# geobacter-rs/rav1e

Hardware: AMD Instinct MI355X
Metric: encoded frames/sec + Mpixels/sec, 4K 8-bit speed=10, 1/2/4/8 GPU vs host CPU (higher is better)
Workload: dtype u8

## Files before the change

include/rav1e_hip.h:

```cpp
#ifndef RAV1E_HIP_H
#define RAV1E_HIP_H

#include <stddef.h>
#include <stdint.h>

#ifdef __cplusplus
extern "C" {
#endif

#define RV_OK 0
#define RV_EINVAL (-1)
#define RV_EHIP (-2)
#define RV_ENOTSUP (-3)

typedef enum rv_cpu_feature_level {
  RV_CPU_NATIVE = 0,
  RV_CPU_SSE2 = 1,
  RV_CPU_SSSE3 = 2,
  RV_CPU_AVX2 = 3,
  RV_CPU_HIP = 4,
  RV_CPU_LEVELS = 5
} rv_cpu_feature_level;

int rv_cpu_feature_level_default(void);
// ... 248 lines not shown
                        uint32_t *d_offsets, uint32_t *d_tokens, uint32_t token_cap,
                        uint32_t *d_status, void *stream);
int rv_ec_cand_rates(const rv_ec_cand *d_cands, int n, const rv_ec_mode_job *d_mode_jobs,
                     int n_mode_jobs, const rv_ec_job *d_tx_jobs, int n_tx_jobs,
                     rv_ec_mode_params params, int n_tiles, const int32_t *d_tile_dims, int xdec,
                     int ydec, int map_w4, int map_h4, const uint8_t *d_coef_map, int map_w8,
                     int map_h8, const uint32_t *d_mode_map, void *d_scratch, uint32_t *d_offsets,
                     uint32_t *d_tokens, uint32_t token_cap, const uint16_t *d_cdfs_all, int n_cdfs,
                     const int32_t *d_group_cdf, const uint32_t *d_init, uint32_t *d_rate,
                     uint32_t *d_status, void *stream);

int rv_q_lookup(int ac, int qindex, int bit_depth);

typedef struct rv_mv {
  int16_t row, col;
} rv_mv;
typedef struct rv_fs_job {
  int32_t po_x, po_y;
  int32_t x_lo, x_hi, y_lo, y_hi;
  rv_mv pmv[2];
  uint32_t lambda;
  int32_t reserved;
} rv_fs_job;
typedef struct rv_fs_result {
  rv_mv best_mv;
  uint32_t reserved;
  uint64_t cost;
} rv_fs_result;

typedef struct rv_mv_blk {
  int8_t ref[2];
  uint8_t n4_w, n4_h, newmv, pad[3];
  rv_mv mv[2];
} rv_mv_blk;
typedef struct rv_mv_cand {
  rv_mv this_mv, comp_mv;
  uint32_t weight;
} rv_mv_cand;
typedef struct rv_mvref_tile {
  int32_t cols, rows, mi_x, mi_y;
} rv_mvref_tile;
typedef struct rv_mvref_geom {
  int32_t n_tiles, grid_w, grid_h, frame_cols, frame_rows;
  uint32_t sign_bias;
} rv_mvref_geom;
typedef struct rv_mvref_query {
  int32_t tile, bx, by, bw4, bh4, ref[2], reserved;
} rv_mvref_query;
typedef struct rv_mvref_result {
  int32_t mode_context, n;
  rv_mv_cand stack[9];
} rv_mvref_result;
size_t rv_mvref_paint_scratch_bytes(rv_mvref_geom geom);
int rv_mvref_grid_paint(const rv_ec_mode_job *d_jobs, int n, rv_mvref_geom geom,
                        const rv_mvref_tile *d_tiles, rv_mv_blk *d_grid, void *d_scratch,
                        uint32_t *d_status, void *stream);
int rv_find_mvrefs_batch(const rv_mvref_query *d_queries, int n, rv_mvref_geom geom,
                         const rv_mvref_tile *d_tiles, const rv_mv_blk *d_grid,
                         rv_mvref_result *d_results, uint32_t *d_status, void *stream);
int rv_ec_mode_fill_stacks(rv_ec_mode_job *d_jobs, int n, rv_mvref_geom geom,
                           const rv_mvref_tile *d_tiles, const rv_mv_blk *d_grid,
                           rv_mvref_result *d_stacks, uint32_t *d_status, void *stream);

size_t rv_propagate_importances_scratch(int w_imp, int h_imp);
int rv_propagate_importances(const rv_plane *org, const rv_plane *ref, const rv_mv *d_mvs,
                             const uint32_t *d_intra_costs, const float *d_importances,
                             int n_unique, float *d_ref_importances, void *d_scratch,
                             size_t scratch_bytes, void *stream);
int rv_full_search_batch(const rv_plane *org, const rv_plane *ref,
                         const rv_fs_job *d_jobs, int n, int blk_w,
                         int blk_h, int step, int allow_hp,
                         rv_fs_result *d_out, void *stream);

int rv_plane_box_sums(const rv_plane *p, uint32_t *d_box, void *stream);

int rv_full_search_sea_batch(const rv_plane *org, const rv_plane *ref,
                             const uint32_t *d_ref_box, const rv_fs_job *d_jobs,
                             int n, int allow_hp, rv_fs_result *d_out,
                             void *stream);

#define RV_DS_MAX_PRED 17
#define RV_MAX_REFS 8
typedef struct rv_ds_job {
  int32_t po_x, po_y;
  int32_t mvx_min, mvx_max;
  int32_t mvy_min, mvy_max;
  rv_mv pmv[2];
  uint32_t lambda;
  int32_t n_pred;
  rv_mv pred[RV_DS_MAX_PRED];
} rv_ds_job;
int rv_diamond_search_batch(const rv_plane *org, const rv_plane *ref,
                            const rv_ds_job *d_jobs, int n, int blk_w,
                            int blk_h, int subpixel, int use_satd,
                            int allow_hp, int bit_depth,
                            rv_fs_result *d_out, void *stream);

int rv_telescopic_subpel_batch(const rv_plane *org, const rv_plane *ref,
                               const rv_ds_job *d_jobs,
                               const rv_fs_result *d_start, int n, int blk_w,
                               int blk_h, int use_satd, int allow_hp,
                               int bit_depth, rv_fs_result *d_out,
                               void *stream);

typedef struct rv_replay_cfg {
  int32_t width, height;
  int32_t xdec, ydec;
  int32_t bit_depth;
  int32_t tile_x0, tile_y0;
  int32_t tile_w, tile_h;
  int32_t n_refs;
  int32_t tile_w_sb, tile_h_sb;
  int32_t n_inputs;
  int32_t flags;
} rv_replay_cfg;
#define RV_REPLAY_EXHAUSTIVE_FS 4
#define RV_REPLAY_SPEED6 8
#define RV_REPLAY_DEBLOCK 16
#define RV_REPLAY_CDEF 32
#define RV_REPLAY_NO_INTRA 64
#define RV_REPLAY_ENTROPY 128
#define RV_REPLAY_MVREF_STANDIN 256
#define RV_REPLAY_LRF 512
typedef struct rv_replay_frame_info {
  int32_t display;
  int32_t me_range_scale;
  int32_t level;
  int32_t is_key;
  int32_t ref_display[2];
  int32_t compound;
} rv_replay_frame_info;
typedef struct rv_replay_level_params {
  int32_t base_q_idx;
  int32_t dc_delta_q[3];
  int32_t ac_delta_q[3];
  int32_t cdef_strengths;
  double lambda, me_lambda;
  double dist_scale[3];
} rv_replay_level_params;
typedef struct rv_replay rv_replay;
rv_replay *rv_replay_create(const rv_replay_cfg *cfg, void *stream);
void rv_replay_destroy(rv_replay *r);
rv_replay *rv_replay_create_twin(rv_replay *primary, void *stream);
int rv_replay_seek(rv_replay *r, long n);
void *rv_replay_stream(rv_replay *r);
int rv_replay_set_level_params(rv_replay *r, int level, const rv_replay_level_params *p);
int rv_replay_synth_inputs(rv_replay *r, int t0);
int rv_replay_set_input(rv_replay *r, int idx, const void *host_yuv);
int rv_replay_get_input(rv_replay *r, int idx, void *host_yuv);
int rv_replay_get_recon(rv_replay *r, int display, void *host_yuv);
int rv_replay_set_importances(rv_replay *r, const float *host, int n);
int rv_replay_set_imp_window(rv_replay *r, int window, long limit);
int rv_replay_set_inputs_ready(rv_replay *r, long displays);
typedef struct rv_la_hub rv_la_hub;
rv_la_hub *rv_la_hub_create(int n_groups);
void rv_la_hub_destroy(rv_la_hub *hub);
int rv_replay_set_la_exchange(rv_replay *r, void *comm, rv_la_hub *hub);
int rv_replay_get_importances(rv_replay *r, float *host, int n);
int rv_replay_frame(rv_replay *r, rv_replay_frame_info *info);
int rv_replay_set_groups(rv_replay *r, int n_groups, const int32_t *rects, int my_group,
                         void *comm);
int rv_replay_exchange_buffers(rv_replay *r, void **send, void **recv, size_t *bytes_per_group);
int rv_replay_import(rv_replay *r);
int rv_comm_unique_id(uint8_t *out, int cap);
void *rv_comm_create(const uint8_t *id, int nranks, int rank);
void rv_comm_destroy(void *comm);
int rv_replay_results(rv_replay *r, uint64_t *host_out, int cap);
int rv_replay_entropy_stats(rv_replay *r, uint64_t *out, int cap);
int rv_replay_set_timing(rv_replay *r, int stride, int block);
int rv_replay_stage_times(rv_replay *r, float *ms_out, int cap);
int rv_replay_stage_times_sum(rv_replay *r, int last_frames, float *ms_out,
                              int cap);
int rv_replay_set_kernel_probe(rv_replay *r, int on);
int rv_round_ring_slots(uint32_t q, int32_t *out, int cap);
int rv_replay_lrf_units(rv_replay *r, int plane, int8_t *out, int cap);
int rv_replay_la_refs(long m, int R, int32_t *out);
int rv_replay_kernel_probe(rv_replay *r, double *out, int cap);
int rv_ds_phase_dump(void);
int rv_rdo_phase_dump(void);
int rv_replay_counters(rv_replay *r, uint64_t *out, int cap);

int rv_replay_dpb_slots(void);


void rv_shims_release(void);
void rv_shims_shutdown(void);

#define RV_DIST_SIZES(X) \
  X(4, 4) X(4, 8) X(8, 4) X(8, 8) X(8, 16) X(16, 8) X(16, 16) X(16, 32) \
  X(32, 16) X(32, 32) X(32, 64) X(64, 32) X(64, 64) X(64, 128) X(128, 64) \
  X(128, 128) X(4, 16) X(16, 4) X(8, 32) X(32, 8) X(16, 64) X(64, 16)

#define RV_DECL_DIST(W, H)                                                   \
  uint32_t rav1e_sad##W##x##H##_hip(const uint8_t *src, ptrdiff_t src_stride, \
                                    const uint8_t *dst, ptrdiff_t dst_stride); \
  uint32_t rav1e_sad##W##x##H##_hbd_hip(const uint16_t *src,                  \
                                        ptrdiff_t src_stride,                 \
                                        const uint16_t *dst,                  \
                                        ptrdiff_t dst_stride);                \
  uint32_t rav1e_satd_##W##x##H##_hip(const uint8_t *src,                     \
                                      ptrdiff_t src_stride,                   \
                                      const uint8_t *dst,                     \
                                      ptrdiff_t dst_stride);                  \
  uint32_t rav1e_satd_##W##x##H##_hbd_hip(const uint16_t *src,                \
                                          ptrdiff_t src_stride,               \
                                          const uint16_t *dst,                \
                                          ptrdiff_t dst_stride);
RV_DIST_SIZES(RV_DECL_DIST)
#undef RV_DECL_DIST

#define RV_FILTER_PAIRS(X)                                                  \
  X(regular, regular, 0, 0) X(smooth, regular, 1, 0)                       \
  X(sharp, regular, 2, 0) X(bilinear, regular, 3, 0)                       \
  X(regular, smooth, 0, 1) X(smooth, smooth, 1, 1) X(sharp, smooth, 2, 1)  \
  X(bilinear, smooth, 3, 1) X(regular, sharp, 0, 2) X(smooth, sharp, 1, 2) \
  X(sharp, sharp, 2, 2) X(bilinear, sharp, 3, 2)                           \
  X(regular, bilinear, 0, 3) X(smooth, bilinear, 1, 3)                     \
  X(sharp, bilinear, 2, 3) X(bilinear, bilinear, 3, 3)

#define RV_DECL_MC(NX, NY, MX, MY)                                            \
  void rav1e_put_8tap_##NX##_##NY##_hip(                                      \
      uint8_t *dst, ptrdiff_t dst_stride, const uint8_t *src,                 \
      ptrdiff_t src_stride, int32_t w, int32_t h, int32_t mx, int32_t my);    \
  void rav1e_put_8tap_##NX##_##NY##_16bpc_hip(                                \
      uint16_t *dst, ptrdiff_t dst_stride, const uint16_t *src,               \
      ptrdiff_t src_stride, int32_t w, int32_t h, int32_t mx, int32_t my,     \
      int32_t bit_depth);                                                     \
  void rav1e_prep_8tap_##NX##_##NY##_hip(int16_t *tmp, const uint8_t *src,    \
                                         ptrdiff_t src_stride, int32_t w,     \
                                         int32_t h, int32_t mx, int32_t my);  \
  void rav1e_prep_8tap_##NX##_##NY##_16bpc_hip(                               \
      int16_t *tmp, const uint16_t *src, ptrdiff_t src_stride, int32_t w,     \
      int32_t h, int32_t mx, int32_t my, int32_t bit_depth);
RV_FILTER_PAIRS(RV_DECL_MC)
#undef RV_DECL_MC

void rav1e_avg_hip(uint8_t *dst, ptrdiff_t dst_stride, const int16_t *tmp1,
                   const int16_t *tmp2, int32_t w, int32_t h);
void rav1e_avg_16bpc_hip(uint16_t *dst, ptrdiff_t dst_stride,
                         const int16_t *tmp1, const int16_t *tmp2, int32_t w,
                         int32_t h, int32_t bit_depth);

int rav1e_fwd_txfm_hip(const int16_t *residual, int32_t *coeffs,
                       int32_t tx_size, int32_t tx_type, int32_t bit_depth);
int rav1e_inv_txfm_add_hip(const int32_t *coeffs, void *dst,
                           ptrdiff_t dst_stride, int32_t tx_size,
                           int32_t tx_type, int32_t bit_depth);

typedef uint32_t (*rv_dist_fn)(const void *src, ptrdiff_t src_stride,
                               const void *dst, ptrdiff_t dst_stride);
rv_dist_fn rv_sad_fn(int cpu_level, int bsize, int hbd);
rv_dist_fn rv_satd_fn(int cpu_level, int bsize, int hbd);
typedef void (*rv_put_fn)(void *dst, ptrdiff_t dst_stride, const void *src,
                          ptrdiff_t src_stride, int32_t w, int32_t h,
                          int32_t mx, int32_t my);
rv_put_fn rv_put_fn_get(int cpu_level, int mode_x, int mode_y);

#ifdef __cplusplus
}
#endif
#endif
```

rav1e_amd/__init__.py:

```python
from __future__ import annotations

import ctypes as C
import enum
import os

import numpy as np

_ROOT = os.path.dirname(os.path.abspath(__file__))
LIB_PATH = os.environ.get("RAV1E_HIP_LIB") or os.path.join(_ROOT, "lib", "librav1e_hip.so")
HEADER_PATH = os.path.join(os.path.dirname(_ROOT), "include", "rav1e_hip.h")

RV_OK, RV_EINVAL, RV_EHIP, RV_ENOTSUP = 0, -1, -2, -3


class Rav1eHipError(RuntimeError):
    pass


class RvPlane(C.Structure):
    _fields_ = [("data", C.c_void_p), ("stride", C.c_int32),
                ("alloc_height", C.c_int32), ("width", C.c_int32),
                ("height", C.c_int32), ("xorigin", C.c_int32),
                ("yorigin", C.c_int32), ("xdec", C.c_int32),
                ("ydec", C.c_int32), ("hbd", C.c_int32),
# ... 113 lines not shown
    TX_64X64 = 4
    TX_4X8 = 5
    TX_8X4 = 6
    TX_8X16 = 7
    TX_16X8 = 8
    TX_16X32 = 9
    TX_32X16 = 10
    TX_32X64 = 11
    TX_64X32 = 12
    TX_4X16 = 13
    TX_16X4 = 14
    TX_8X32 = 15
    TX_32X8 = 16
    TX_16X64 = 17
    TX_64X16 = 18

    def width(self) -> int:
        return int(self.name.split("_")[1].split("X")[0])

    def height(self) -> int:
        return int(self.name.split("X")[-1])


class TxType(enum.IntEnum):
    DCT_DCT = 0
    ADST_DCT = 1
    DCT_ADST = 2
    ADST_ADST = 3
    FLIPADST_DCT = 4
    DCT_FLIPADST = 5
    FLIPADST_FLIPADST = 6
    ADST_FLIPADST = 7
    FLIPADST_ADST = 8
    IDTX = 9
    V_DCT = 10
    H_DCT = 11
    V_ADST = 12
    H_ADST = 13
    V_FLIPADST = 14
    H_FLIPADST = 15


class FilterMode(enum.IntEnum):
    REGULAR = 0
    SMOOTH = 1
    SHARP = 2
    BILINEAR = 3


_lib = None


class RvEcModeParams(C.Structure):
    _fields_ = [(n, C.c_int32) for n in ("frame_type", "reference_mode", "force_integer_mv",
                                         "allow_high_precision_mv", "seg_enabled",
                                         "last_active_segid")]


class RvMvrefGeom(C.Structure):
    _fields_ = [(n, C.c_int32) for n in ("n_tiles", "grid_w", "grid_h", "frame_cols",
                                         "frame_rows")] + [("sign_bias", C.c_uint32)]


def _declare(L):
    vp, i32, sz = C.c_void_p, C.c_int, C.c_size_t
    P = C.POINTER(RvPlane)
    sig = {
        "rv_cpu_feature_level_default": (i32, []),
        "rv_cpu_feature_level_index": (i32, [i32]),
        "rv_device_count": (i32, []),
        "rv_set_device": (i32, [i32]),
        "rv_last_error": (C.c_char_p, []),
        "rv_version": (C.c_char_p, []),
        "rv_malloc": (vp, [sz]),
        "rv_free": (None, [vp]),
        "rv_host_alloc": (vp, [sz]),
        "rv_host_free": (None, [vp]),
        "rv_memcpy_h2d": (i32, [vp, vp, sz, vp]),
        "rv_memcpy_d2h": (i32, [vp, vp, sz, vp]),
        "rv_memcpy_d2d": (i32, [vp, vp, sz, vp]),
        "rv_memset": (i32, [vp, i32, sz, vp]),
        "rv_stream_create": (vp, []),
        "rv_stream_create_priority": (vp, [i32]),
        "rv_stream_destroy": (i32, [vp]),
        "rv_stream_sync": (i32, [vp]),
        "rv_device_sync": (i32, []),
        "rv_trace_marker": (i32, [vp]),
        "rv_event_create": (vp, []),
        "rv_event_destroy": (i32, [vp]),
        "rv_event_record": (i32, [vp, vp]),
        "rv_event_sync": (i32, [vp]),
        "rv_stream_wait_event": (i32, [vp, vp]),
        "rv_event_elapsed_ms": (C.c_float, [vp, vp]),
        "rv_plane_geometry": (sz, [P, i32, i32, i32, i32, i32, i32, i32]),
        "rv_plane_pad": (i32, [P, vp]),
        "rv_plane_downsample": (i32, [P, P, vp]),
        "rv_sad_batch": (i32, [P, P, vp, i32, i32, i32, vp, vp]),
        "rv_satd_batch": (i32, [P, P, vp, i32, i32, i32, vp, vp]),
        "rv_sse_batch": (i32, [P, P, vp, i32, i32, i32, vp, vp]),
        "rv_lookahead_intra_costs": (i32, [P, i32, vp, vp]),
        "rv_propagate_importances_scratch": (sz, [i32, i32]),
        "rv_propagate_importances": (i32, [P, P, vp, vp, vp, i32, vp, vp, sz, vp]),
        "rv_cdef_moments_batch": (i32, [P, P, vp, i32, i32, i32, vp, vp]),
        "rv_put_8tap_batch": (i32, [P, P, vp, i32, i32, i32, i32, i32, i32, vp]),
        "rv_predict_intra_batch": (i32, [P, vp, vp, i32, i32, i32, vp]),
        "rv_cfl_luma_ac_batch": (i32, [P, vp, i32, i32, i32, i32, vp, vp]),
        "rv_predict_cfl_batch": (i32, [P, vp, vp, vp, vp, i32, i32, i32, vp]),
        "rv_cfl_alpha_search_batch": (i32, [P, P, vp, i32, i32, i32, vp, vp, vp]),
        "rv_frame_delta_batch": (i32, [P, i32, i32, vp, i32, vp, vp]),
        "rv_deblock_plane": (i32, [P, i32, i32, i32, vp, vp, i32, vp, i32, vp]),
        "rv_deblock_fast_level": (i32, [i32, i32, i32]),
        "rv_deblock_sse": (i32, [P, P, i32, i32, vp, vp, i32, vp, vp, i32, vp]),
        "rv_deblock_frame": (i32, [P, i32, i32, vp, vp, i32, vp, i32, vp]),
        "rv_cdef_find_dirs": (i32, [P, i32, i32, vp, i32, vp, vp, i32, vp]),
        "rv_lrf_stripe_filter": (i32, [P, P] + [i32] * 10 + [vp, vp]),
        "rv_y4m_parse_header": (i32, [C.c_char_p, vp]),
        "rv_y4m_open": (vp, [C.c_char_p]),
        "rv_y4m_get_info": (i32, [vp, vp]),
        "rv_y4m_frame_bytes": (sz, [vp]),
        "rv_y4m_read_frame": (i32, [vp, vp]),
        "rv_y4m_close": (None, [vp]),
        "rv_ivf_create": (vp, [C.c_char_p, i32, i32, i32, i32]),
        "rv_ivf_write_frame": (i32, [vp, C.c_uint64, vp, sz]),
        "rv_ivf_close": (i32, [vp]),
        "rv_cdef_filter_plane": (i32, [P, P, i32, i32, i32, vp, i32, vp, vp, vp, vp, vp, i32, i32,
                                       vp]),
        "rv_prep_8tap_batch": (i32, [vp, P, vp, i32, i32, i32, i32, i32, i32, vp]),
        "rv_mc_avg_batch": (i32, [P, vp, vp, vp, i32, i32, i32, i32, vp]),
        "rv_mc_dist_batch": (i32, [P, P, vp, i32, i32, i32, i32, i32, i32, i32, vp, vp]),
        "rv_fwd_txfm_batch": (i32, [vp, vp, i32, i32, i32, i32, vp]),
        "rv_diff_fwd_txfm_batch": (i32, [P, P, vp, i32, i32, i32, i32, vp, vp]),
        "rv_inv_txfm_add_batch": (i32, [vp, P, vp, i32, i32, i32, i32, vp]),
        "rv_quantize_batch": (i32, [vp, i32, i32, i32, i32, i32, i32, i32, i32, i32, vp, vp, vp,
                                    vp]),
        "rv_dequantize_batch": (i32, [vp, i32, i32, i32, i32, i32, i32, vp, vp]),
        "rv_estimate_rate_batch": (i32, [vp, i32, i32, i32, vp, vp]),
        "rv_full_search_batch": (i32, [P, P, vp, i32, i32, i32, i32, i32, vp, vp]),
        "rv_full_search_sea_batch": (i32, [P, P, vp, vp, i32, i32, vp, vp]),
        "rv_plane_box_sums": (i32, [P, vp, vp]),
        "rv_replay_create": (vp, [C.POINTER(RvReplayCfg), vp]),
        "rv_replay_create_twin": (vp, [vp, vp]),
        "rv_replay_seek": (i32, [vp, C.c_long]),
        "rv_replay_stream": (vp, [vp]),
        "rv_replay_destroy": (None, [vp]),
        "rv_q_lookup": (i32, [i32, i32, i32]),
        "rv_replay_synth_inputs": (i32, [vp, i32]),
        "rv_replay_set_level_params": (i32, [vp, i32, C.POINTER(RvReplayLevelParams)]),
        "rv_replay_set_input": (i32, [vp, i32, vp]),
        "rv_replay_get_input": (i32, [vp, i32, vp]),
        "rv_replay_get_recon": (i32, [vp, i32, vp]),
        "rv_replay_set_importances": (i32, [vp, vp, i32]),
        "rv_replay_set_imp_window": (i32, [vp, i32, C.c_long]),
        "rv_replay_set_inputs_ready": (i32, [vp, C.c_long]),
        "rv_replay_get_importances": (i32, [vp, vp, i32]),
        "rv_replay_frame": (i32, [vp, C.POINTER(RvReplayFrameInfo)]),
        "rv_replay_set_groups": (i32, [vp, i32, vp, i32, vp]),
        "rv_replay_exchange_buffers": (i32, [vp, C.POINTER(C.c_void_p), C.POINTER(C.c_void_p),
                                             C.POINTER(C.c_size_t)]),
        "rv_replay_import": (i32, [vp]),
        "rv_comm_unique_id": (i32, [vp, i32]),
        "rv_comm_create": (vp, [vp, i32, i32]),
        "rv_comm_destroy": (None, [vp]),
        "rv_replay_results": (i32, [vp, vp, i32]),
        "rv_replay_entropy_stats": (i32, [vp, vp, i32]),
        "rv_replay_stage_times": (i32, [vp, vp, i32]),
        "rv_replay_stage_times_sum": (i32, [vp, i32, vp, i32]),
        "rv_replay_counters": (i32, [vp, vp, i32]),
        "rv_replay_dpb_slots": (i32, []),
        "rv_replay_set_kernel_probe": (i32, [vp, i32]),
        "rv_replay_kernel_probe": (i32, [vp, vp, i32]),
        "rv_round_ring_slots": (i32, [C.c_uint32, vp, i32]),
        "rv_replay_lrf_units": (i32, [vp, i32, vp, i32]),
        "rv_replay_la_refs": (i32, [C.c_long, i32, vp]),
        "rv_la_hub_create": (vp, [i32]),
        "rv_la_hub_destroy": (None, [vp]),
        "rv_replay_set_la_exchange": (i32, [vp, vp, vp]),
        "rv_replay_set_timing": (i32, [vp, i32, i32]),
        "rv_diamond_search_batch": (i32, [P, P, vp, i32, i32, i32, i32, i32, i32, i32, vp, vp]),
        "rv_telescopic_subpel_batch": (i32, [P, P, vp, vp, i32, i32, i32, i32, i32, i32, vp, vp]),
        "rv_tx_dist_batch": (i32, [vp, i32, vp, i32, i32, vp, vp]),
        "rav1e_fwd_txfm_hip": (i32, [vp, vp, i32, i32, i32]),
        "rav1e_inv_txfm_add_hip": (i32, [vp, vp, C.c_ssize_t, i32, i32, i32]),
        "rv_ec_scratch_bytes": (C.c_size_t, [i32]),
        "rv_ec_tokenize": (i32, [vp, i32, i32, i32, i32, i32, i32, vp, vp, vp, vp, C.c_uint32, vp,
                                 vp]),
        "rv_ec_code_tokens": (C.c_long, [vp, C.c_size_t, vp, vp, C.c_size_t]),
        "rv_ec_count_tokens": (C.c_long, [vp, C.c_size_t, vp, vp]),
        "rv_ec_rate_batch": (i32, [vp, vp, vp, i32, vp, i32, vp, vp, vp, vp, vp]),
        "rv_ec_cdf_total": (i32, []),
        "rv_ec_default_cdf": (i32, [i32, vp]),
        "rv_ec_reset_counts": (None, [vp]),
        "rv_ec_mode_scratch_bytes": (C.c_size_t, [i32]),
        "rv_ec_mode_tokenize": (i32, [vp, i32, RvEcModeParams, i32, vp, i32, i32, vp, vp, vp, vp,
                                      C.c_uint32, vp, vp]),
        "rv_ec_code_stream": (C.c_long, [vp, C.c_size_t, vp, vp, C.c_size_t]),
        "rv_ec_count_stream": (C.c_long, [vp, C.c_size_t, vp, vp]),
        "rv_ec_cdf_total_all": (i32, []),
        "rv_ec_default_cdf_all": (i32, [i32, vp]),
        "rv_ec_reset_counts_all": (None, [vp]),
        "rv_ec_partition_gather": (i32, [vp, i32]),
        "rv_ec_rate_stream_batch": (i32, [vp, vp, vp, i32, vp, i32, vp, vp, vp, vp, vp]),
        "rv_ec_rate_stream_batch_waves": (i32, [vp, vp, vp, i32, vp, i32, vp, vp, vp, vp, i32, vp]),
        "rv_ec_cand_scratch_bytes": (C.c_size_t, [i32, i32]),
        "rv_ec_cand_tokenize": (i32, [vp, i32, vp, i32, vp, i32, RvEcModeParams, i32, vp, i32, i32,
                                      i32, i32, vp, i32, i32, vp, vp, vp, vp, C.c_uint32, vp, vp]),
        "rv_ec_cand_rates": (i32, [vp, i32, vp, i32, vp, i32, RvEcModeParams, i32, vp, i32, i32,
                                   i32, i32, vp, i32, i32, vp, vp, vp, vp, C.c_uint32, vp, i32, vp,
                                   vp, vp, vp, vp]),
        "rv_mvref_paint_scratch_bytes": (C.c_size_t, [RvMvrefGeom]),
        "rv_mvref_grid_paint": (i32, [vp, i32, RvMvrefGeom, vp, vp, vp, vp, vp]),
        "rv_find_mvrefs_batch": (i32, [vp, i32, RvMvrefGeom, vp, vp, vp, vp, vp]),
        "rv_ec_mode_fill_stacks": (i32, [vp, i32, RvMvrefGeom, vp, vp, vp, vp, vp]),
        "rv_sad_fn": (vp, [i32, i32, i32]),
        "rv_satd_fn": (vp, [i32, i32, i32]),
        "rv_put_fn_get": (vp, [i32, i32, i32]),
    }
    for name, (res, args) in sig.items():
        f = getattr(L, name)
        f.restype = res
        f.argtypes = args


def lib():
    global _lib
    if _lib is None:
        if not os.path.exists(LIB_PATH):
            raise Rav1eHipError(
                f"{LIB_PATH} missing: run `python -c 'import __graft_entry__ as g; g.build()'`")
        L = C.CDLL(LIB_PATH, mode=C.RTLD_GLOBAL)
        _declare(L)
        _lib = L
    return _lib


def _check(rc, what):
    if rc != RV_OK:
        raise Rav1eHipError(f"{what} failed ({rc}): {lib().rv_last_error().decode()}")


def require_device(device: int = 0):
    L = lib()
    if L.rv_device_count() <= device:
        raise Rav1eHipError("no HIP device visible: the HIP level needs a gfx950 GPU")
    _check(L.rv_set_device(device), "rv_set_device")


class DeviceBuffer:

    def __init__(self, nbytes: int):
        self.nbytes = int(nbytes)
        self.ptr = lib().rv_malloc(max(1, self.nbytes))
        if not self.ptr:
            raise Rav1eHipError(f"rv_malloc({nbytes}): {lib().rv_last_error().decode()}")

    @classmethod
    def from_array(cls, a: np.ndarray) -> "DeviceBuffer":
        a = np.ascontiguousarray(a)
        b = cls(a.nbytes)
        b.upload(a)
        return b

    def upload(self, a: np.ndarray, stream=None):
        a = np.ascontiguousarray(a)
        assert a.nbytes <= self.nbytes
        if a.nbytes:
            _check(lib().rv_memcpy_h2d(self.ptr, a.ctypes.data, a.nbytes, stream), "rv_memcpy_h2d")

    def download(self, dtype, count=None, stream=None) -> np.ndarray:
        dt = np.dtype(dtype)
        n = self.nbytes // dt.itemsize if count is None else int(count)
        out = np.empty(n, dtype=dt)
        if out.nbytes:
            _check(lib().rv_memcpy_d2h(out.ctypes.data, self.ptr, out.nbytes, stream),
                   "rv_memcpy_d2h")
        return out

    def zero(self, stream=None):
        _check(lib().rv_memset(self.ptr, 0, self.nbytes, stream), "rv_memset")
        _check(lib().rv_stream_sync(stream), "rv_stream_sync")

    def free(self):
        if self.ptr:
            lib().rv_free(self.ptr)
            self.ptr = None

    def __del__(self):
        try:
            self.free()
        except Exception:
            pass


class DevicePlane:

    def __init__(self, width, height, xdec=0, ydec=0, xpad=0, ypad=0, hbd=False,
                 bit_depth=None):
        self.desc = RvPlane()
        nbytes = lib().rv_plane_geometry(C.byref(self.desc), width, height, xdec, ydec,
                                         xpad, ypad, 1 if hbd else 0)
        if bit_depth is not None:
            self.desc.bit_depth = int(bit_depth)
        self.buf = DeviceBuffer(nbytes)
        self.desc.data = self.buf.ptr
        self.dtype = np.uint16 if hbd else np.uint8

    @classmethod
# ... 1737 lines not shown
```

rav1e_amd/csrc/rv_epzs.h:

```cpp
#pragma once

#include "rv_chain.h"

namespace rv {

struct EpzsGeo {
  int tx0, ty0, tw, th, tws, ths, W, H, w_in_b, h_in_b;
};

__device__ inline void epzs_tile(const EpzsGeo &g, int fx, int fy, int &t0x, int &t0y, int &mi_w,
                                 int &mi_h) {
  t0x = fx - fx % g.tws;
  t0y = fy - fy % g.ths;
  const int vw = g.W - t0x * 64 < g.tws * 64 ? g.W - t0x * 64 : g.tws * 64;
  const int vh = g.H - t0y * 64 < g.ths * 64 ? g.H - t0y * 64 : g.ths * 64;
  mi_w = vw >> 2;
  mi_h = vh >> 2;
}

__device__ inline void epzs_adjust_bo(int mi_w, int mi_h, int &bx, int &by, int bw, int bh) {
  const int x = bx < mi_w - bw / 4 ? bx : mi_w - bw / 4;
  const int y = by < mi_h - bh / 4 ? by : mi_h - bh / 4;
  bx = x > 0 ? x : 0;
  by = y > 0 ? y : 0;
}

__device__ inline rv_mv epzs_qfull(rv_mv m) {
  return rv_mv{(int16_t)((m.row / 8) * 8), (int16_t)((m.col / 8) * 8)};
}
__device__ inline bool epzs_zero(rv_mv m) { return m.row == 0 && m.col == 0; }

template <int NCM, typename Rd>
__device__ inline bool epzs_update(rv_ds_job *j, int shr, const EpzsGeo &g, int tx4, int ty4,
                                   int mi_w, int bx, int by, const rv_mv (&cm)[NCM], int ncm,
                                   Rd rd, const rv_mv *prev, int pr) {
  static_assert(NCM >= 1 && 1 + NCM + 4 + 5 <= RV_DS_MAX_PRED, "slots");
  constexpr int NS = 1 + NCM + 4 + 5;
  const bool hl = bx > 0, ht = by > 0, htr = ht && bx < mi_w - 1;
  const rv_mv z{0, 0};
  const rv_mv l = hl ? rd(tx4 + bx - 1, ty4 + by) : z;
  const rv_mv t = ht ? rd(tx4 + bx, ty4 + by - 1) : z;
  const rv_mv tr = htr ? rd(tx4 + bx + 1, ty4 + by - 1) : z;
  rv_mv c[NS];
  uint32_t valid = 1;
  c[0] = z;
#pragma unroll
  for (int i = 0; i < NCM; i++) {
    c[1 + i] = epzs_qfull(cm[i]);
    valid |= (uint32_t)(i < ncm) << (1 + i);
  }
  c[NCM + 1] = l;
  c[NCM + 2] = t;
  c[NCM + 3] = tr;
  valid |= (uint32_t)(hl && !epzs_zero(l)) << (NCM + 1);
  valid |= (uint32_t)(ht && !epzs_zero(t)) << (NCM + 2);
  valid |= (uint32_t)(htr && !epzs_zero(tr)) << (NCM + 3);
  const int nm = (int)hl + (int)ht + (int)htr;
  {
    const int16_t sr = (int16_t)((int16_t)(l.row + t.row) + tr.row);
    const int16_t sc = (int16_t)((int16_t)(l.col + t.col) + tr.col);
    const int d = nm ? nm : 1;
    c[NCM + 4] = epzs_qfull(rv_mv{(int16_t)(sr / d), (int16_t)(sc / d)});
    valid |= (uint32_t)(nm && !epzs_zero(c[NCM + 4])) << (NCM + 4);
  }
  if (prev) {
    const int fx = tx4 + bx, fy = ty4 + by, w8 = g.w_in_b >> 1;
    auto pv = [&](int x, int y) { return prev[((y >> 1) * w8 + (x >> 1)) * pr]; };
    c[NCM + 5] = fx > 0 ? pv(fx - 1, fy) : z;
    c[NCM + 6] = fy > 0 ? pv(fx, fy - 1) : z;
    c[NCM + 7] = fx < g.w_in_b - 1 ? pv(fx + 1, fy) : z;
    c[NCM + 8] = fy < g.h_in_b - 1 ? pv(fx, fy + 1) : z;
    c[NCM + 9] = pv(fx, fy);
#pragma unroll
    for (int i = NCM + 5; i < NS; i++) valid |= (uint32_t)!epzs_zero(c[i]) << i;
  } else {
#pragma unroll
    for (int i = NCM + 5; i < NS; i++) c[i] = z;
  }
  auto tf = [&](rv_mv m) { return shr ? rv_mv{(int16_t)(m.row >> 1), (int16_t)(m.col >> 1)} : m; };
  rv_mv nw[NS];
#pragma unroll
  for (int p = 0; p < NS; p++) nw[p] = z;
#pragma unroll
  for (int i = 0; i < NS; i++) {
    const bool v = (valid >> i) & 1;
    const int pos = __popc(valid & ((1u << i) - 1));
    const rv_mv ti = tf(c[i]);
#pragma unroll
    for (int p = 0; p <= i; p++)
      if (v && pos == p) nw[p] = ti;
  }
  const int n = __popc(valid);
  rv_mv old[NS];
#pragma unroll
  for (int p = 0; p < NS; p++) old[p] = j->pred[p];
  const int old_n = j->n_pred;
  bool same = old_n == n;
#pragma unroll
  for (int p = 0; p < NS; p++) same &= (p >= n) | mv_eq(old[p], nw[p]);
  if (same) return false;
#pragma unroll
  for (int p = 0; p < NS; p++)
    if (p < n) j->pred[p] = nw[p];
  j->n_pred = n;
  return true;
}

struct RoundPub {
  int32_t *cnt, *next;
  uint32_t *ticket;
  unsigned long long *host;
  uint32_t seq;
};
__device__ inline void round_publish(const RoundPub &p) {
  if (!p.host) return;
  __syncthreads();
  if (threadIdx.x != 0) return;
  __threadfence();
  const uint32_t t = atomicAdd(p.ticket, 1u);
  if (t != gridDim.x - 1) return;
  __threadfence();
  const int c = atomicAdd(p.cnt, 0) + atomicAdd(p.cnt + 1, 0);
  p.next[0] = p.next[1] = 0;
  *p.ticket = 0;
  __threadfence();
  __hip_atomic_store(p.host, ((unsigned long long)p.seq << 32) | (uint32_t)c, __ATOMIC_RELAXED,
                     __HIP_MEMORY_SCOPE_SYSTEM);
}

}
```

rav1e_amd/csrc/rv_me.h:

```cpp
#pragma once
#include "rv_chain.h"
#include "rv_device.h"

int rv_full_search_multi(const rv_plane *org, const rv_plane *refs, int n_refs,
                         const rv_fs_job *d_jobs, int n_per_ref, int blk_w, int blk_h,
                         int step, int allow_hp, rv_fs_result *d_out, const rv::ChainNext *next,
                         const uint32_t *const *box, void *stream);
int rv_diamond_search_multi(const rv_plane *org, const rv_plane *refs, int n_refs,
                            const rv_ds_job *d_jobs, int n_per_ref, int blk_w, int blk_h,
                            int subpixel, int use_satd, int allow_hp, int bit_depth,
                            rv_fs_result *d_out, uint32_t *d_evals, const rv::ChainNext *next,
                            void *stream, const uint8_t *active = nullptr,
                            const int32_t *alist = nullptr, const int32_t *acount = nullptr,
                            int lper = 1, const uint8_t *dirty = nullptr, int list_grid = 0,
                            uint32_t *eval_acc = nullptr, unsigned long long *t01 = nullptr);
int rv_diamond_f2_f3(const rv_plane *org_h, const rv_plane *refs_h, const rv_ds_job *jobs_h,
                     rv_fs_result *out_h, const uint8_t *dirty_h, const rv_plane *org,
                     const rv_plane *refs, const rv_ds_job *jobs, rv_fs_result *out,
                     const uint8_t *dirty, const rv::ChainNext *next, int n_refs, int n_per_ref,
                     int bit_depth, const int32_t *alist, const int32_t *acount, int list_grid,
                     void *stream, const rv_ds_job *jobs_sub = nullptr,
                     rv_fs_result *out_sub = nullptr, uint32_t *eval_acc = nullptr,
                     unsigned long long *t01 = nullptr);
```

rav1e_amd/csrc/rv_me_diamond.hip:

```cpp
#include <algorithm>
#include <stdio.h>
#include <stdlib.h>
#include <string.h>

#include "rv_chain.h"
#include "rv_device.h"
#include "rv_me.h"

namespace rv {

constexpr int kDsThreads = 256;
constexpr int kDsWaves = kDsThreads / 64;

__constant__ int8_t kReg[2][16][8] = {
    {{0, 0, 0, 127, 0, 0, 0, 0}, {0, 2, -6, 126, 8, -2, 0, 0},
     {0, 2, -10, 122, 18, -4, 0, 0}, {0, 2, -12, 116, 28, -8, 2, 0},
     {0, 2, -14, 110, 38, -10, 2, 0}, {0, 2, -14, 102, 48, -12, 2, 0},
     {0, 2, -16, 94, 58, -12, 2, 0}, {0, 2, -14, 84, 66, -12, 2, 0},
     {0, 2, -14, 76, 76, -14, 2, 0}, {0, 2, -12, 66, 84, -14, 2, 0},
     {0, 2, -12, 58, 94, -16, 2, 0}, {0, 2, -12, 48, 102, -14, 2, 0},
     {0, 2, -10, 38, 110, -14, 2, 0}, {0, 2, -8, 28, 116, -12, 2, 0},
     {0, 0, -4, 18, 122, -10, 2, 0}, {0, 0, -2, 8, 126, -6, 2, 0}},
    {{0, 0, 0, 127, 0, 0, 0, 0}, {0, 0, -4, 126, 8, -2, 0, 0},
     {0, 0, -8, 122, 18, -4, 0, 0}, {0, 0, -10, 116, 28, -6, 0, 0},
     {0, 0, -12, 110, 38, -8, 0, 0}, {0, 0, -12, 102, 48, -10, 0, 0},
     {0, 0, -14, 94, 58, -10, 0, 0}, {0, 0, -12, 84, 66, -10, 0, 0},
     {0, 0, -12, 76, 76, -12, 0, 0}, {0, 0, -10, 66, 84, -12, 0, 0},
     {0, 0, -10, 58, 94, -14, 0, 0}, {0, 0, -10, 48, 102, -12, 0, 0},
     {0, 0, -8, 38, 110, -12, 0, 0}, {0, 0, -6, 28, 116, -10, 0, 0},
     {0, 0, -4, 18, 122, -8, 0, 0}, {0, 0, -2, 8, 126, -4, 0, 0}}};

__device__ __forceinline__ uint32_t ds_diff_to_rate(int16_t diff, int hp) {
  int16_t d = hp ? diff : (int16_t)(diff >> 1);
  if (d == 0) return 0;
  uint32_t a = (uint16_t)(d < 0 ? -d : d);
  return 2u * (16u - (uint32_t)(__builtin_clz(a) - 16));
}

__device__ __forceinline__ uint64_t ds_cost(uint32_t dist, rv_mv mv, const rv_ds_job &jb,
                                            int hp) {
  const uint32_t r1 = ds_diff_to_rate((int16_t)(mv.row - jb.pmv[0].row), hp) +
                      ds_diff_to_rate((int16_t)(mv.col - jb.pmv[0].col), hp);
  const uint32_t r2 = ds_diff_to_rate((int16_t)(mv.row - jb.pmv[1].row), hp) +
                      ds_diff_to_rate((int16_t)(mv.col - jb.pmv[1].col), hp);
  const uint32_t rate = r1 < r2 + 1 ? r1 : r2 + 1;
  return 256ull * dist + (uint64_t)rate * jb.lambda;
}

__device__ __forceinline__ bool ds_in_range(rv_mv mv, const rv_ds_job &jb) {
  return !(mv.col < jb.mvx_min || mv.col > jb.mvx_max || mv.row < jb.mvy_min ||
           mv.row > jb.mvy_max);
}

__device__ __forceinline__ int xcd_job(int n) {
  const int per = (int)gridDim.x >> 3;
  return ((int)blockIdx.x & 7) * per + ((int)blockIdx.x >> 3);
}

struct DsArgs {
  rv_plane org;
  rv_plane ref[RV_MAX_REFS];
  const rv_ds_job *jobs;
  rv_fs_result *out;
  int n, n_per_ref, w, h, subpel, satd, hp, bd;
  uint32_t *evals;
  uint32_t *eval_acc;
  unsigned long long *t0, *t1;
  ChainNext next;
  int tele;
  const rv_fs_result *start;
  const uint8_t *active;
  const int32_t *alist;
  const int32_t *acount;
  int lper;
  const uint8_t *dirty;
  int list_grid;
  int ph;
};

__device__ unsigned long long g_ds_ph[16];

__device__ __forceinline__ int ds_list_total(const DsArgs &a) {
  const int cnt = __builtin_amdgcn_readfirstlane(*a.acount);
  return a.lper ? cnt * a.lper * (a.n / a.n_per_ref) : cnt;
}
__device__ __forceinline__ int ds_list_job(const DsArgs &a, int ord) {
  if (!a.lper) return a.alist[ord];
  const int cnt = *a.acount, per = cnt * a.lper;
  const int r = ord / per, rem = ord - r * per, i = rem / a.lper;
  return r * a.n_per_ref + a.alist[i] * a.lper + (rem - i * a.lper);
}

constexpr int kDsListGrid = 512;

__device__ __forceinline__ void ds_write(const DsArgs &a, int job, rv_mv center,
                                         uint64_t cost) {
  rv_fs_result r;
  r.best_mv = center;
  r.reserved = 0;
  r.cost = cost;
  a.out[job] = r;
}

__device__ __forceinline__ uint4 ld16(const void *p) {
  uint4 v;
  __builtin_memcpy(&v, p, 16);
  return v;
}
template <typename Px>
__device__ __forceinline__ uint32_t sad16(uint4 a, uint4 b, uint32_t acc) {
  if constexpr (sizeof(Px) == 1) {
    acc = __builtin_amdgcn_sad_u8(a.x, b.x, acc);
    acc = __builtin_amdgcn_sad_u8(a.y, b.y, acc);
    acc = __builtin_amdgcn_sad_u8(a.z, b.z, acc);
    return __builtin_amdgcn_sad_u8(a.w, b.w, acc);
  } else {
    acc = __builtin_amdgcn_sad_u16(a.x, b.x, acc);
    acc = __builtin_amdgcn_sad_u16(a.y, b.y, acc);
    acc = __builtin_amdgcn_sad_u16(a.z, b.z, acc);
    return __builtin_amdgcn_sad_u16(a.w, b.w, acc);
  }
}

__device__ __forceinline__ uint32_t wave_sum(uint32_t v) { return group_sum<64>(v); }

template <typename Px, int W, int H>
struct FullGeo {
  static constexpr int K = W * (int)sizeof(Px) / 16;
  static constexpr int R = 64 / K;
  static constexpr int I = (H + R - 1) / R;
  static constexpr bool kPartial = (R * I != H);
};

template <typename Px, int W, int H>
struct SubGeo {
  static constexpr int G = 64 / W;
  static constexpr int RG = H / G;
  static constexpr int P = sizeof(Px) == 1 ? ((W + 8 + 15) / 16) * 16
                                           : ((2 * (W + 8) + 15) / 16) * 16;
  static constexpr int kWinDwords = (H + 7) * P / 4;
  static constexpr int kOrgDwords = RG * (int)sizeof(Px) / 4;
  static constexpr int D = 8;
  static constexpr int UP = (((W + 7 + D + 4) * (int)sizeof(Px)) + 15) / 16 * 16;
  static constexpr int kUnionDwords = (H + 7 + D) * UP / 4;
};

template <typename Px, int W, int RG, int UP, bool HF, bool VF>
__device__ __forceinline__ uint32_t sub_sad_rows(const uint32_t *win, const Px *ocol, int cx,
                                                 int grp, const int8_t *xf, const int8_t *yf,
                                                 int ib, int maxv) {
  constexpr int B = (int)sizeof(Px);
  constexpr int PD = UP / 4;
  uint32_t xp[4] = {0, 0, 0, 0};
  int xsum = 0;
  if constexpr (HF) {
    if constexpr (B == 1) {
#pragma unroll
      for (int h = 0; h < 2; h++)
        xp[h] = (uint32_t)(uint8_t)xf[4 * h] | ((uint32_t)(uint8_t)xf[4 * h + 1] << 8) |
                ((uint32_t)(uint8_t)xf[4 * h + 2] << 16) | ((uint32_t)(uint8_t)xf[4 * h + 3] << 24);
#pragma unroll
      for (int k = 0; k < 8; k++) xsum += xf[k];
    } else {
#pragma unroll
      for (int h = 0; h < 3; h++)
        xp[h] = (uint32_t)(uint16_t)(int16_t)xf[2 * h + 1] |
                ((uint32_t)(uint16_t)(int16_t)xf[2 * h + 2] << 16);
    }
  }
  uint32_t tp[3] = {0, 0, 0};
  if constexpr (VF) {
#pragma unroll
    for (int h = 0; h < 3; h++)
      tp[h] = (uint32_t)(uint16_t)(int16_t)yf[2 * h + 1] |
              ((uint32_t)(uint16_t)(int16_t)yf[2 * h + 2] << 16);
  }
  const int hbias = 128 * xsum;
  const int hround = (1 << (7 - ib)) >> 1, hsh = 7 - ib;
  const uint32_t *base = win + grp * RG * PD;
  auto hval = [&](int t) __attribute__((always_inline)) -> int32_t {
    const uint32_t *row = base + t * PD;
    if constexpr (B == 1) {
      if constexpr (!HF) {
        return (int32_t)(reinterpret_cast<const uint8_t *>(row)[cx + 3] ^ 0x80u);
      } else {
        const int d0 = cx >> 2, sh = cx & 3;
        const uint32_t w0 = row[d0], w1 = row[d0 + 1], w2 = row[d0 + 2];
        int32_t s = dot4_i8(__builtin_amdgcn_alignbyte(w1, w0, sh), xp[0], hbias + hround);
        s = dot4_i8(__builtin_amdgcn_alignbyte(w2, w1, sh), xp[1], s);
        return s >> hsh;
      }
    } else {
      if constexpr (!HF) {
        return (int32_t)reinterpret_cast<const uint16_t *>(row)[cx + 3];
      } else {
        const int c1 = cx + 1, d0 = c1 >> 1, sh = (c1 & 1) * 2;
        uint32_t w[4];
#pragma unroll
        for (int k = 0; k < 4; k++) w[k] = row[d0 + k];
        int32_t s = hround;
#pragma unroll
        for (int k = 0; k < 3; k++) s = dot2_i16(__builtin_amdgcn_alignbyte(w[k + 1], w[k], sh), xp[k], s);
        return s >> hsh;
      }
    }
  };
  auto absdiff_acc = [](uint32_t a, uint32_t b, uint32_t acc) __attribute__((always_inline)) {
    return (a > b ? a - b : b - a) + acc;
  };
  uint32_t acc = 0;
  if constexpr (!VF) {
#pragma unroll 8
    for (int r = 0; r < RG; r++) {
      int32_t v = hval(r + 3);
      if constexpr (HF) v = clamp_med3(round_shift(v, ib), 0, maxv);
      acc = absdiff_acc((uint32_t)ocol[r * W], (uint32_t)v, acc);
    }
  } else {
    const int vshift = HF ? 7 + ib : 7;
    const int vround = (1 << vshift) >> 1;
    auto pack = [](int32_t lo, int32_t hi) __attribute__((always_inline)) {
      return __builtin_amdgcn_perm((uint32_t)hi, (uint32_t)lo, 0x05040100u);
    };
    uint32_t pr[8];
    int32_t prev = hval(1);
#pragma unroll
    for (int t = 2; t < 6; t++) {
      const int32_t m = hval(t);
      pr[t - 1] = pack(prev, m);
      prev = m;
// ... 609 lines not shown
      if (center_cost <= best) {
        if (radius == radius_end) break;
        radius /= 2;
      } else {
        center = best_mv;
        center_cost = best;
      }
    }
  }
  if (threadIdx.x == 0) {
    if (a.evals) a.evals[job] = evals;
    ds_write(a, job, center, center_cost);
    chain_emit(a.next, job, a.n_per_ref, a.n / a.n_per_ref, center);
  }
}

template <typename Px, int W, int H>
__global__ __launch_bounds__(64) void ds_wave_kernel(DsArgs a) {
  using F = FullGeo<Px, W, H>;
  constexpr int B = (int)sizeof(Px);
  const int job = xcd_job(a.n);
  if (job >= a.n) return;
  if (a.active && !a.active[job % a.n_per_ref]) return;
  const int lane = threadIdx.x;
  const rv_ds_job *jp = a.jobs + job;
  const rv_ds_job jb = *jp;
  const rv_plane &ref = a.ref[job / a.n_per_ref];
  const int frow = lane / F::K, fchunk = lane % F::K;
  uint32_t org[4 * F::I];
  {
    const uint8_t *o = (const uint8_t *)plane_ptr<Px>(a.org, jb.po_x, jb.po_y);
    const int64_t os = (int64_t)a.org.stride * B;
#pragma unroll
    for (int i = 0; i < F::I; i++) {
      const int r = i * F::R + frow;
      uint4 v = make_uint4(0, 0, 0, 0);
      if (!F::kPartial || r < H) v = ld16(o + r * os + fchunk * 16);
      org[4 * i + 0] = v.x;
      org[4 * i + 1] = v.y;
      org[4 * i + 2] = v.z;
      org[4 * i + 3] = v.w;
    }
  }
  const int64_t rs = (int64_t)ref.stride * B;
  uint32_t evals = 0;
  auto round4 = [&](const rv_mv *cands, int n, int skip, uint64_t *cost)
      __attribute__((always_inline)) {
    bool ok[kDsWaves];
    const uint8_t *rp[kDsWaves];
#pragma unroll
    for (int k = 0; k < kDsWaves; k++) {
      ok[k] = k < n && k != skip && ds_in_range(cands[k], jb);
      rp[k] = (const uint8_t *)plane_ptr<Px>(ref, jb.po_x + (ok[k] ? cands[k].col / 8 : 0),
                                             jb.po_y + (ok[k] ? cands[k].row / 8 : 0));
      evals += ok[k];
    }
    uint32_t acc[kDsWaves] = {0, 0, 0, 0};
#pragma unroll
    for (int i = 0; i < F::I; i++) {
      const int rr = i * F::R + frow;
      if (!F::kPartial || rr < H) {
        uint4 v[kDsWaves];
#pragma unroll
        for (int k = 0; k < kDsWaves; k++)
          v[k] = ok[k] ? ld16(rp[k] + rr * rs + fchunk * 16) : make_uint4(0, 0, 0, 0);
        const uint4 o = make_uint4(org[4 * i], org[4 * i + 1], org[4 * i + 2], org[4 * i + 3]);
#pragma unroll
        for (int k = 0; k < kDsWaves; k++) acc[k] = sad16<Px>(o, v[k], acc[k]);
      }
    }
#pragma unroll
    for (int k = 0; k < kDsWaves; k++)
      cost[k] = ok[k] ? ds_cost(wave_sum(acc[k]), cands[k], jb, a.hp) : ~0ull;
  };

  rv_mv center{0, 0};
  uint64_t center_cost = ~0ull;
  const int np = jb.n_pred < RV_DS_MAX_PRED ? jb.n_pred : RV_DS_MAX_PRED;
  int16_t radius = 16;
  const int16_t radius_end = 8;
  int p0 = 0;
  int back = -1;
  for (int iter = 0; iter < 4096 + RV_DS_MAX_PRED; iter++) {
    const bool pred_phase = p0 < np;
    rv_mv c4[kDsWaves];
    int n;
    if (pred_phase) {
      n = np - p0 < kDsWaves ? np - p0 : kDsWaves;
#pragma unroll
      for (int k = 0; k < kDsWaves; k++) c4[k] = jp->pred[p0 + (k < n ? k : 0)];
    } else {
      n = kDsWaves;
      c4[0] = rv_mv{(int16_t)(center.row + radius), center.col};
      c4[1] = rv_mv{center.row, (int16_t)(center.col + radius)};
      c4[2] = rv_mv{(int16_t)(center.row - radius), center.col};
      c4[3] = rv_mv{center.row, (int16_t)(center.col - radius)};
    }
    uint64_t c[kDsWaves];
    round4(c4, n, pred_phase ? -1 : back, c);
    uint64_t best = ~0ull;
    int bp = 0;
#pragma unroll
    for (int k = 0; k < kDsWaves; k++)
      if (k < n && c[k] < best) {
        best = c[k];
        bp = k;
      }
    rv_mv bmv = c4[0];
#pragma unroll
    for (int k = 1; k < kDsWaves; k++)
      if (bp == k) bmv = c4[k];
    if (pred_phase) {
      if (best < center_cost) {
        center = bmv;
        center_cost = best;
      }
      p0 += kDsWaves;
    } else if (center_cost <= best) {
      if (radius == radius_end) break;
      radius /= 2;
      back = -1;
    } else {
      back = center_cost != ~0ull ? (bp + 2) & 3 : -1;
      center = bmv;
      center_cost = best;
    }
  }
  if (lane == 0) {
    if (a.evals) a.evals[job] = evals;
    ds_write(a, job, center, center_cost);
    chain_emit(a.next, job, a.n_per_ref, a.n / a.n_per_ref, center);
  }
}

typedef short rv_s16x2 __attribute__((ext_vector_type(2)));
__device__ __forceinline__ int32_t sdot2(uint32_t a, uint32_t b, int32_t c) {
  return __builtin_amdgcn_sdot2(__builtin_bit_cast(rv_s16x2, a), __builtin_bit_cast(rv_s16x2, b),
                                c, false);
}
__device__ __forceinline__ uint32_t pk16(int lo, int hi) {
  return (uint32_t)(uint16_t)lo | ((uint32_t)(uint16_t)hi << 16);
}

template <int N, bool SADONLY>
struct GrpGeo {
  static constexpr int C = N == 8 || (SADONLY && N == 16) ? 4 : 16;
  static constexpr int L = 4 * C;
  static constexpr int RPL = N == 8 ? 2 : (N == 16 && C == 16) ? 2 : 8;
  static constexpr int LPC = 8 / RPL;
  static constexpr int NC = N / 8;
  static constexpr int CPL = NC * NC * LPC / C;
};

template <typename Px, int N, bool SUB, bool SATD>
__device__ __forceinline__ void ds_grp_body(const DsArgs &a, const int ord, const int nord) {
  using G = GrpGeo<N, !SUB && !SATD>;
  static_assert(G::CPL >= 1 && G::C % G::LPC == 0, "lane layout");
  const int lane = threadIdx.x & 63;
  const int gl = lane % G::L, k = gl / G::C, c = gl % G::C;
  const int gbase = lane - gl;
  const int oid = ord < nord ? ord : nord - 1;
  const int job = a.alist ? ds_list_job(a, oid) : oid;
  const bool live = ord < nord && !(a.dirty && !a.dirty[job]);
  if (__ballot(live) == 0) return;
  const int jid = job;
  const rv_ds_job *jp = a.jobs + jid;
  const rv_ds_job jb = *jp;
  const rv_plane &ref = a.ref[jid / a.n_per_ref];
  const int ib = a.bd == 12 ? 2 : 4, maxv = (1 << a.bd) - 1;
  const int lic = c % G::LPC;

  auto dist = [&](rv_mv mv, bool ok) -> uint32_t {
    int cf = 0, rf = 0, sx = 0, sy = 0;
    if (SUB) {
      const int xs = 3 + ref.xdec, ys = 3 + ref.ydec;
      const int roff = (int)mv.row >> ys, coff = (int)mv.col >> xs;
      rf = ((int)mv.row - (roff << ys)) << (4 - ys);
      cf = ((int)mv.col - (coff << xs)) << (4 - xs);
      sx = clampi(jb.po_x + coff - 3, -ref.xorigin, ref.width);
      sy = clampi(jb.po_y + roff - 3, -ref.yorigin, ref.height);
    } else {
      sx = jb.po_x + (ok ? mv.col / 8 : 0);
      sy = jb.po_y + (ok ? mv.row / 8 : 0);
    }
    uint32_t xp[7];
    int32_t fy[8];
    if (SUB) {
      int32_t fx[8];
      const int8_t *xf = kReg[0][cf];
      const int8_t *yf = kReg[0][rf];
#pragma unroll
      for (int u = 0; u < 8; u++) {
        fx[u] = cf ? (int32_t)xf[u] : (u == 3 ? 128 : 0);
        fy[u] = rf ? (int32_t)yf[u] : (u == 3 ? 128 : 0);
      }
      xp[0] = pk16(fx[1], fx[2]);
      xp[1] = pk16(fx[3], fx[4]);
      xp[2] = pk16(fx[5], fx[6]);
      xp[3] = pk16(fx[0], fx[1]);
      xp[4] = pk16(fx[2], fx[3]);
      xp[5] = pk16(fx[4], fx[5]);
      xp[6] = pk16(fx[6], fx[7]);
    }
    const int32_t hround = (1 << (7 - ib)) >> 1, vround = (1 << (7 + ib)) >> 1;
    uint32_t acc = 0;
#pragma unroll 1
    for (int j = 0; j < G::CPL; j++) {
      const int q = c / G::LPC + j * (G::C / G::LPC);
      const int x0 = (q % G::NC) * 8, y0 = (q / G::NC) * 8 + lic * G::RPL;
      int32_t d[G::RPL][8];
      if (SUB) {
        int32_t v[G::RPL][8];
#pragma unroll
        for (int i = 0; i < G::RPL; i++)
#pragma unroll
          for (int t = 0; t < 8; t++) v[i][t] = vround;
#pragma unroll
        for (int m = 1; m < G::RPL + 6; m++) {
          const Px *w = plane_ptr<Px>(ref, sx + x0, sy + y0 + m);
          uint32_t pp[7];
          if constexpr (sizeof(Px) == 1) {
            const uint4 lv = ld16(w);
            const uint32_t wd[4] = {lv.x, lv.y, lv.z, lv.w};
#pragma unroll
            for (int jj = 0; jj < 7; jj++)
              pp[jj] = __builtin_amdgcn_perm(0u, wd[jj >> 1], jj & 1 ? 0x0c030c02u : 0x0c010c00u);
          } else {
            const uint4 v0 = ld16(w), v1 = ld16(w + 8);
            const uint32_t wd[7] = {v0.x, v0.y, v0.z, v0.w, v1.x, v1.y, v1.z};
#pragma unroll
            for (int jj = 0; jj < 7; jj++) pp[jj] = wd[jj];
          }
          int32_t mid[8];
#pragma unroll
          for (int t = 0; t < 8; t++) {
            int32_t hs = hround;
            if (t & 1) {
#pragma unroll
              for (int u = 0; u < 3; u++) hs = sdot2(pp[(t + 1) / 2 + u], xp[u], hs);
            } else {
#pragma unroll
              for (int u = 0; u < 4; u++) hs = sdot2(pp[t / 2 + u], xp[3 + u], hs);
            }
            mid[t] = hs >> (7 - ib);
          }
#pragma unroll
          for (int i = 0; i < G::RPL; i++) {
            const int kk = m - i;
            if (kk >= 1 && kk < 7) {
#pragma unroll
              for (int t = 0; t < 8; t++) v[i][t] += __mul24(fy[kk], mid[t]);
            }
          }
        }
#pragma unroll
        for (int i = 0; i < G::RPL; i++) {
          const Px *o = plane_ptr<Px>(a.org, jb.po_x + x0, jb.po_y + y0 + i);
#pragma unroll
          for (int t = 0; t < 8; t++)
            d[i][t] = (int32_t)o[t] - clampi(v[i][t] >> (7 + ib), 0, maxv);
        }
      } else if (ok) {
        if (!SATD) {
#pragma unroll
          for (int i = 0; i < G::RPL; i++) {
            const Px *o = plane_ptr<Px>(a.org, jb.po_x + x0, jb.po_y + y0 + i);
            const Px *r = plane_ptr<Px>(ref, sx + x0, sy + y0 + i);
            if constexpr (sizeof(Px) == 1) {
              uint2 ov, rv;
              __builtin_memcpy(&ov, o, 8);
              __builtin_memcpy(&rv, r, 8);
              acc = __builtin_amdgcn_sad_u8(ov.x, rv.x, acc);
              acc = __builtin_amdgcn_sad_u8(ov.y, rv.y, acc);
            } else {
              acc = sad16<Px>(ld16(o), ld16(r), acc);
            }
#pragma unroll
            for (int t = 0; t < 8; t++) d[i][t] = 0;
          }
        } else {
#pragma unroll
          for (int i = 0; i < G::RPL; i++) {
            const Px *o = plane_ptr<Px>(a.org, jb.po_x + x0, jb.po_y + y0 + i);
            const Px *r = plane_ptr<Px>(ref, sx + x0, sy + y0 + i);
#pragma unroll
            for (int t = 0; t < 8; t++) d[i][t] = (int32_t)o[t] - (int32_t)r[t];
          }
        }
      } else {
#pragma unroll
        for (int i = 0; i < G::RPL; i++)
#pragma unroll
          for (int t = 0; t < 8; t++) d[i][t] = 0;
      }
      if (SATD) {
#pragma unroll
        for (int i = 0; i < G::RPL; i++) ds_had<8>(&d[i][0], 1);
#pragma unroll
        for (int b = 1; b < G::RPL; b <<= 1)
#pragma unroll
          for (int i = 0; i < G::RPL; i++)
            if (!(i & b))
#pragma unroll
              for (int t = 0; t < 8; t++) {
                const int32_t x = d[i][t], y = d[i + b][t];
                d[i][t] = x + y;
                d[i + b][t] = x - y;
              }
#pragma unroll
        for (int b = 1; b < G::LPC; b <<= 1) {
          const bool up = (lic & b) != 0;
#pragma unroll
          for (int i = 0; i < G::RPL; i++)
#pragma unroll
            for (int t = 0; t < 8; t++) {
              const int32_t p = __shfl_xor(d[i][t], b, 64);
              d[i][t] = up ? p - d[i][t] : d[i][t] + p;
            }
        }
      }
#pragma unroll
      for (int i = 0; i < G::RPL; i++)
#pragma unroll
        for (int t = 0; t < 8; t++) acc += (uint32_t)(d[i][t] < 0 ? -d[i][t] : d[i][t]);
    }
#pragma unroll
    for (int m = G::C / 2; m; m >>= 1) acc += __shfl_xor(acc, m, 64);
    return SATD ? (acc + 4) >> 3 : acc;
  };

  uint32_t evals = 0;
  auto round4 = [&](const rv_mv *cands, int n, int skip, uint64_t *cost)
      __attribute__((always_inline)) {
    bool ok[4];
#pragma unroll
    for (int kk = 0; kk < 4; kk++) {
      ok[kk] = kk < n && kk != skip && ds_in_range(cands[kk], jb);
      evals += ok[kk];
    }
    rv_mv mine = cands[0];
    bool okm = ok[0];
#pragma unroll
    for (int kk = 1; kk < 4; kk++)
      if (k == kk) {
        mine = cands[kk];
        okm = ok[kk];
      }
    const uint32_t dv = dist(mine, okm);
    const uint64_t cm = okm ? ds_cost(dv, mine, jb, a.hp) : ~0ull;
    const uint32_t lo = (uint32_t)cm, hi = (uint32_t)(cm >> 32);
#pragma unroll
    for (int kk = 0; kk < 4; kk++) {
      const uint32_t l = __shfl(lo, gbase + kk * G::C, 64), h = __shfl(hi, gbase + kk * G::C, 64);
      cost[kk] = ((uint64_t)h << 32) | l;
    }
  };

  rv_mv center{0, 0};
  uint64_t center_cost = ~0ull;
  const int np = jb.n_pred < RV_DS_MAX_PRED ? jb.n_pred : RV_DS_MAX_PRED;
  int16_t radius = SUB ? 4 : 16;
  const int16_t radius_end = SUB ? (a.hp ? 1 : 2) : 8;
  int p0 = 0, back = -1;
  for (int iter = 0; iter < 4096 + RV_DS_MAX_PRED; iter++) {
    const bool pred_phase = p0 < np;
    rv_mv c4[4];
    int n;
    if (pred_phase) {
      n = np - p0 < 4 ? np - p0 : 4;
#pragma unroll
      for (int kk = 0; kk < 4; kk++) c4[kk] = jp->pred[p0 + (kk < n ? kk : 0)];
    } else {
      n = 4;
      c4[0] = rv_mv{(int16_t)(center.row + radius), center.col};
      c4[1] = rv_mv{center.row, (int16_t)(center.col + radius)};
      c4[2] = rv_mv{(int16_t)(center.row - radius), center.col};
      c4[3] = rv_mv{center.row, (int16_t)(center.col - radius)};
    }
    uint64_t cst[4];
    round4(c4, n, pred_phase ? -1 : back, cst);
    uint64_t best = ~0ull;
    int bp = 0;
#pragma unroll
    for (int kk = 0; kk < 4; kk++)
      if (kk < n && cst[kk] < best) {
        best = cst[kk];
        bp = kk;
      }
    rv_mv bmv = c4[0];
#pragma unroll
    for (int kk = 1; kk < 4; kk++)
      if (bp == kk) bmv = c4[kk];
    if (pred_phase) {
      if (best < center_cost) {
        center = bmv;
        center_cost = best;
      }
      p0 += 4;
    } else if (center_cost <= best) {
      if (radius == radius_end) break;
      radius /= 2;
      back = -1;
    } else {
      back = center_cost != ~0ull ? (bp + 2) & 3 : -1;
      center = bmv;
      center_cost = best;
    }
  }
  if (gl == 0 && live) {
    if (a.evals) a.evals[job] = evals;
    ds_write(a, job, center, center_cost);
    chain_emit(a.next, job, a.n_per_ref, a.n / a.n_per_ref, center);
  }
}

template <typename Px, int N, bool SUB, bool SATD>
__global__ __launch_bounds__(256) void ds_grp_kernel(DsArgs a) {
  using G = GrpGeo<N, !SUB && !SATD>;
  constexpr int JPW = 64 / G::L;
  const int lane = threadIdx.x & 63;
  const int w0 = ((int)blockIdx.x * 4 + (int)(threadIdx.x >> 6)) * JPW;
  const int nord = a.alist ? ds_list_total(a) : a.n;
  const int step = (int)gridDim.x * 4 * JPW;
  for (int o = w0; o < nord; o += step) {
    ds_grp_body<Px, N, SUB, SATD>(a, o + lane / G::L, nord);
    if (!a.alist) break;
  }
}
template <typename Px>
__device__ __forceinline__ void ds_grp16_pool(DsArgs a, int b, int gsz) {
  using G = GrpGeo<16, true>;
  constexpr int JPW = 64 / G::L;
  const int lane = threadIdx.x & 63;
  const int nord = ds_list_total(a);
  for (int o = (b * 4 + (int)(threadIdx.x >> 6)) * JPW; o < nord; o += gsz * 4 * JPW)
    ds_grp_body<Px, 16, false, false>(a, o + lane / G::L, nord);
}
template <typename Px>
__device__ __forceinline__ void ds_fast64_pool(DsArgs a, DsArgs sa, bool fuse, int b, int gsz) {
  const int total = ds_list_total(a);
  for (int i = b; i < total; i += gsz) {
    const int job = __builtin_amdgcn_readfirstlane(ds_list_job(a, i));
    if (a.dirty && !a.dirty[job]) continue;
    const rv_mv best = ds_fast_body<Px, 64, 64, false>(a, job);
    __syncthreads();
    if (fuse) {
      ds_fast_body<Px, 64, 64, true>(sa, job, true, best);
      __syncthreads();
    }
  }
}
template <typename Px>
__global__ __launch_bounds__(256) void ds_f2_f3_kernel(
    DsArgs f2, DsArgs f3, DsArgs f3s, int g2, int fuse, unsigned long long *t01) {
  if (t01 && threadIdx.x == 0) atomicMin(t01, (unsigned long long)wall_clock64());
  if ((int)blockIdx.x < g2)
    ds_grp16_pool<Px>(f2, blockIdx.x, g2);
  else
    ds_fast64_pool<Px>(f3, f3s, fuse != 0, (int)blockIdx.x - g2, (int)gridDim.x - g2);
  if (t01) {
    __syncthreads();
    if (threadIdx.x == 0) atomicMax(t01 + 1, (unsigned long long)wall_clock64());
  }
}

template <typename Px>
bool try_grp(const DsArgs &a, hipStream_t s) {
  if (a.tele || a.w != a.h || a.active) return false;
  const int n = a.w;
  const bool small = n == 8 || n == 16;
  if (!(small || (a.satd && (n == 32 || n == 64)))) return false;
  const int jpw = 64 / (n == 8 || (n == 16 && !a.subpel && !a.satd) ? 16 : 64);
  unsigned grid = (unsigned)((a.n + 4 * jpw - 1) / (4 * jpw));
  if (a.alist && grid > (unsigned)(a.list_grid ? a.list_grid : kDsListGrid))
    grid = (unsigned)(a.list_grid ? a.list_grid : kDsListGrid);
#define RV_GRP(N)                                                                     \
  if (n == N) {                                                                       \
    if (a.subpel) {                                                                   \
      if (a.satd) ds_grp_kernel<Px, N, true, true><<<grid, 256, 0, s>>>(a);           \
      else ds_grp_kernel<Px, N, true, false><<<grid, 256, 0, s>>>(a);                 \
    } else {                                                                          \
      if (a.satd) ds_grp_kernel<Px, N, false, true><<<grid, 256, 0, s>>>(a);          \
      else ds_grp_kernel<Px, N, false, false><<<grid, 256, 0, s>>>(a);                \
    }                                                                                 \
    return true;                                                                      \
  }
  RV_GRP(8)
  RV_GRP(16)
  RV_GRP(32)
  RV_GRP(64)
#undef RV_GRP
  return false;
}

template <typename Px, int W, int H, bool SUB>
void launch_fast(DsArgs a, hipStream_t s) {
  static const bool phases = getenv("RAV1E_HIP_DS_PHASES") && getenv("RAV1E_HIP_DS_PHASES")[0] == '1';
  a.ph = phases && SUB && a.alist ? 1 : 0;
  const unsigned grid = a.alist ? (unsigned)std::min(a.n, a.list_grid ? a.list_grid : kDsListGrid)
                                 : (unsigned)((a.n + 7) / 8 * 8);
  if (!SUB && !a.tele && W * H <= 32 * 32 && !a.alist)
    ds_wave_kernel<Px, W, H><<<grid, 64, 0, s>>>(a);
  else
    ds_fast_kernel<Px, W, H, SUB><<<grid, kDsThreads, 0, s>>>(a);
}

template <typename Px>
bool try_fast(const DsArgs &a, hipStream_t s) {
  if (a.satd) return false;
#define RV_DS_CASE(W, H)                                        \
  if (a.w == W && a.h == H) {                                   \
    if (a.subpel)                                               \
      launch_fast<Px, W, H, true>(a, s);                        \
    else                                                        \
      launch_fast<Px, W, H, false>(a, s);                       \
    return true;                                                \
  }
  RV_DS_CASE(64, 64)
  RV_DS_CASE(32, 32)
  RV_DS_CASE(64, 32)
  RV_DS_CASE(32, 64)
  RV_DS_CASE(16, 32)
  RV_DS_CASE(16, 64)
#undef RV_DS_CASE
  return false;
}

}

using namespace rv;

extern "C" int rv_ds_phase_dump(void) {
  unsigned long long h[16];
  if (hipDeviceSynchronize() != hipSuccess || hipMemcpyFromSymbol(h, HIP_SYMBOL(g_ds_ph), sizeof(h)) != hipSuccess)
    return rv_set_error(RV_EHIP, "rv_ds_phase_dump");
  const double us = 0.01;
  const double j = h[5] ? (double)h[5] : 1.0, w = h[8] ? (double)h[8] : 1.0;
  fprintf(stderr,
          "[ds phases] jobs %llu: setup %.2f us, stage+filter+SAD %.2f us, exchange %.2f us, "
          "job %.2f us per job; %.2f iterations, %.2f stagings per job; workgroups %llu: %.2f us each\n",
          h[5], h[0] * us / j, h[1] * us / j, h[2] * us / j, h[3] * us / j, h[4] / j, h[6] / j, h[8],
          h[7] * us / w);
  memset(h, 0, sizeof(h));
  return hipMemcpyToSymbol(HIP_SYMBOL(g_ds_ph), h, sizeof(h)) == hipSuccess ? RV_OK : rv_set_error(RV_EHIP, "rv_ds_phase_dump");
}

static int ds_dispatch(DsArgs &a, void *stream);

int rv_diamond_search_multi(const rv_plane *org, const rv_plane *refs, int n_refs,
                            const rv_ds_job *d_jobs, int n_per_ref, int blk_w, int blk_h,
                            int subpixel, int use_satd, int allow_hp, int bit_depth,
                            rv_fs_result *d_out, uint32_t *d_evals, const ChainNext *next,
                            void *stream, const uint8_t *active, const int32_t *alist,
                            const int32_t *acount, int lper, const uint8_t *dirty,
                            int list_grid, uint32_t *eval_acc, unsigned long long *t01) {
  auto p2 = [](int v) { return v >= 4 && v <= 128 && (v & (v - 1)) == 0; };
  if (!org || !refs || n_refs < 1 || n_refs > RV_MAX_REFS || n_per_ref < 0 || !p2(blk_w) ||
      !p2(blk_h) || (bit_depth != 8 && bit_depth != 10 && bit_depth != 12) ||
      (!org->hbd && bit_depth != 8))
    return rv_set_error(RV_EINVAL, "rv_diamond_search_batch: bad arguments");
  for (int k = 0; k < n_refs; k++)
    if (refs[k].hbd != org->hbd)
      return rv_set_error(RV_EINVAL, "rv_diamond_search_batch: pixel type mismatch");
  const int n = n_refs * n_per_ref;
  if (n == 0) return RV_OK;
  DsArgs a;
  memset(&a, 0, sizeof(a));
  a.org = *org;
  for (int k = 0; k < n_refs; k++) a.ref[k] = refs[k];
  a.jobs = d_jobs;
  a.out = d_out;
  a.n = n;
  a.n_per_ref = n_per_ref;
  a.w = blk_w;
  a.h = blk_h;
  a.subpel = subpixel ? 1 : 0;
  a.satd = use_satd ? 1 : 0;
  a.hp = allow_hp ? 1 : 0;
  a.bd = bit_depth;
  a.evals = d_evals;
  a.active = active;
  a.alist = alist;
  a.acount = acount;
  a.lper = lper;
  a.dirty = alist ? dirty : nullptr;
  a.list_grid = list_grid;
  a.eval_acc = eval_acc;
  if (t01) {
    a.t0 = t01;
    a.t1 = t01 + 1;
  }
  if (alist && (!acount || lper < 0 || use_satd ||
                !((blk_w == 64 && blk_h == 64) || (blk_w == 16 && blk_h == 16 && !subpixel))))
    return rv_set_error(RV_EINVAL,
                        "rv_diamond_search_multi: list-driven launches: 64x64, or 16x16 full-pel SAD");
  if (next) a.next = *next;
  return ds_dispatch(a, stream);
}

static void ds_fill(DsArgs &a, const rv_plane *org, const rv_plane *refs, int n_refs,
                    const rv_ds_job *d_jobs, int n_per_ref, int blk, rv_fs_result *d_out,
                    int bit_depth, const int32_t *alist, const int32_t *acount, int lper,
                    const uint8_t *dirty) {
  memset(&a, 0, sizeof(a));
  a.org = *org;
  for (int k = 0; k < n_refs; k++) a.ref[k] = refs[k];
  a.jobs = d_jobs;
  a.out = d_out;
  a.n = n_refs * n_per_ref;
  a.n_per_ref = n_per_ref;
  a.w = a.h = blk;
  a.bd = bit_depth;
  a.alist = alist;
  a.acount = acount;
  a.lper = lper;
  a.dirty = dirty;
}

int rv_diamond_f2_f3(const rv_plane *org_h, const rv_plane *refs_h, const rv_ds_job *jobs_h,
                     rv_fs_result *out_h, const uint8_t *dirty_h, const rv_plane *org,
                     const rv_plane *refs, const rv_ds_job *jobs, rv_fs_result *out,
                     const uint8_t *dirty, const ChainNext *next, int n_refs, int n_per_ref,
                     int bit_depth, const int32_t *alist, const int32_t *acount, int list_grid,
                     void *stream, const rv_ds_job *jobs_sub, rv_fs_result *out_sub,
                     uint32_t *eval_acc, unsigned long long *t01) {
  if (!org_h || !refs_h || !org || !refs || n_refs < 1 || n_refs > RV_MAX_REFS || n_per_ref <= 0 ||
      !alist || !acount || org->hbd != org_h->hbd)
    return rv_set_error(RV_EINVAL, "rv_diamond_f2_f3: bad arguments");
  DsArgs f2, f3;
  ds_fill(f2, org_h, refs_h, n_refs, jobs_h, n_per_ref * 4, 16, out_h, bit_depth, alist, acount, 4,
          dirty_h);
  ds_fill(f3, org, refs, n_refs, jobs, n_per_ref, 64, out, bit_depth, alist, acount, 1, dirty);
  if (next) f3.next = *next;
  DsArgs f3s;
  ds_fill(f3s, org, refs, n_refs, jobs_sub ? jobs_sub : jobs, n_per_ref, 64, out_sub ? out_sub : out,
          bit_depth, alist, acount, 1, dirty);
  f3s.subpel = 1;
  static const bool phases = getenv("RAV1E_HIP_DS_PHASES") && getenv("RAV1E_HIP_DS_PHASES")[0] == '1';
  f3s.ph = phases ? 1 : 0;
  const int fuse = jobs_sub && out_sub ? 1 : 0;
  if (fuse) f3s.eval_acc = eval_acc;
  unsigned long long *ts = fuse ? t01 : nullptr;
  const int pool = list_grid ? list_grid : kDsListGrid;
  const int g2 = std::min(pool, (f2.n + 15) / 16), g3 = std::min(f3.n, pool);
  hipStream_t s = rv_resolve_stream(stream);
  if (org->hbd)
    ds_f2_f3_kernel<uint16_t><<<g2 + g3, 256, 0, s>>>(f2, f3, f3s, g2, fuse, ts);
  else
    ds_f2_f3_kernel<uint8_t><<<g2 + g3, 256, 0, s>>>(f2, f3, f3s, g2, fuse, ts);
  RV_HIP_CHECK_LAUNCH();
  return RV_OK;
}

static int ds_dispatch(DsArgs &a, void *stream) {
  const int n = a.n, blk_w = a.w, blk_h = a.h, subpixel = a.subpel;
  const rv_plane *org = &a.org;
  hipStream_t s = rv_resolve_stream(stream);
  const bool fast = (org->hbd ? try_grp<uint16_t>(a, s) : try_grp<uint8_t>(a, s)) ||
                    (org->hbd ? try_fast<uint16_t>(a, s) : try_fast<uint8_t>(a, s));
  if (!fast) {
    const size_t lds = subpixel ? (size_t)((blk_w + 7) * (blk_h + 7) + (blk_h + 7) * blk_w +
                                           blk_w * blk_h) * sizeof(int16_t)
                                : 0;
    if (org->hbd)
      diamond_kernel<uint16_t><<<n, kDsThreads, lds, s>>>(a);
    else
      diamond_kernel<uint8_t><<<n, kDsThreads, lds, s>>>(a);
  }
  RV_HIP_CHECK_LAUNCH();
  return RV_OK;
}

extern "C" int rv_diamond_search_batch(const rv_plane *org, const rv_plane *ref,
                                       const rv_ds_job *d_jobs, int n, int blk_w,
                                       int blk_h, int subpixel, int use_satd,
                                       int allow_hp, int bit_depth,
                                       rv_fs_result *d_out, void *stream) {
  if (!ref) return rv_set_error(RV_EINVAL, "rv_diamond_search_batch: null ref");
  return rv_diamond_search_multi(org, ref, 1, d_jobs, n, blk_w, blk_h, subpixel, use_satd,
                                 allow_hp, bit_depth, d_out, nullptr, nullptr, stream, nullptr,
                                 nullptr, nullptr, 0, nullptr, 0, nullptr, nullptr);
}

extern "C" int rv_telescopic_subpel_batch(const rv_plane *org, const rv_plane *ref,
                                          const rv_ds_job *d_jobs, const rv_fs_result *d_start,
                                          int n, int blk_w, int blk_h, int use_satd,
                                          int allow_hp, int bit_depth, rv_fs_result *d_out,
                                          void *stream) {
  auto p2 = [](int v) { return v >= 4 && v <= 128 && (v & (v - 1)) == 0; };
  if (!org || !ref || !d_start || n < 0 || !p2(blk_w) || !p2(blk_h) || ref->hbd != org->hbd ||
      (bit_depth != 8 && bit_depth != 10 && bit_depth != 12) || (!org->hbd && bit_depth != 8))
    return rv_set_error(RV_EINVAL, "rv_telescopic_subpel_batch: bad arguments");
  if (n == 0) return RV_OK;
  DsArgs a;
  memset(&a, 0, sizeof(a));
  a.org = *org;
  a.ref[0] = *ref;
  a.jobs = d_jobs;
  a.out = d_out;
  a.n = n;
  a.n_per_ref = n;
  a.w = blk_w;
  a.h = blk_h;
  a.subpel = 1;
  a.satd = use_satd ? 1 : 0;
  a.hp = allow_hp ? 1 : 0;
  a.bd = bit_depth;
  a.tele = 1;
  a.start = d_start;
  return ds_dispatch(a, stream);
}
```

rav1e_amd/csrc/rv_replay.h:

```cpp
#pragma once
#include <string.h>

#include <chrono>
#include <condition_variable>
#include <algorithm>
#include <deque>
#include <mutex>
#include <thread>
#include <vector>

#include "rv_cdef.h"
#include "rv_chain.h"
#include "rv_deblock.h"
#include "rv_device.h"
#include "rv_ec.h"
#include "rv_frame.h"
#include "rv_intra.h"
#include "rv_intra_pass.h"
#include "rv_me.h"
#include "rv_mvref.h"
#include "rv_owned.h"
#include "rv_impwin.h"
#include "rv_lrf.h"
#include "rv_rdo.h"
#include <string>

#if __has_include(<rccl/rccl.h>)
#include <rccl/rccl.h>
#define RV_HAVE_RCCL 1
#else
#define RV_HAVE_RCCL 0
#endif

#define RV_R(expr)                  \
  do {                              \
    int e_ = (expr);                \
    if (e_ != RV_OK) return e_;     \
  } while (0)
#define RV_H(expr)                                            \
  do {                                                        \
    hipError_t e_ = (expr);                                   \
    if (e_ != hipSuccess) return rv_set_hip_error(e_, #expr); \
  } while (0)

namespace rv {

constexpr int kSb = 64;
constexpr int kSlots = 24;
constexpr int kWordsPerRef = 2 + 8 + 2 + 2 + 32 + 8;
constexpr int kRoundGrid = 256;
constexpr int kMaxGroups = 8;

struct Geo {
  int W, H, xdec, ydec, bd, hbd;
  int w_in_b, h_in_b;
  int tx0, ty0, tw, th;
  int tws, ths;
  int nsb, R, M, C;
  int cw, ch;
  int w_imp, h_imp;
  int vis_w, vis_h;
};

__host__ __device__ inline int div_trunc8(int v) { return v / 8; }

__host__ __device__ inline void mv_range(const Geo &g, int bx, int by, int bw, int bh, int r[4]) {
  const int border_w = 128 + bw * 8, border_h = 128 + bh * 8;
  r[0] = -bx * 32 - border_w;
  r[1] = (g.w_in_b - bx - bw / 4) * 32 + border_w;
  r[2] = -by * 32 - border_h;
  r[3] = (g.h_in_b - by - bh / 4) * 32 + border_h;
}
__host__ __device__ inline void sb_tile(const Geo &g, int sx, int sy, int &t0x, int &t0y,
                                        int &mi_w, int &mi_h) {
  const int fx = g.tx0 + sx, fy = g.ty0 + sy;
  t0x = fx - fx % g.tws;
  t0y = fy - fy % g.ths;
  const int vw = g.W - t0x * kSb < g.tws * kSb ? g.W - t0x * kSb : g.tws * kSb;
  const int vh = g.H - t0y * kSb < g.ths * kSb ? g.H - t0y * kSb : g.ths * kSb;
  mi_w = vw >> 2;
  mi_h = vh >> 2;
}
__host__ __device__ inline void adjust_bo(int mi_w, int mi_h, int &bx, int &by, int bw, int bh) {
  int x = bx < mi_w - bw / 4 ? bx : mi_w - bw / 4;
  int y = by < mi_h - bh / 4 ? by : mi_h - bh / 4;
  bx = x > 0 ? x : 0;
  by = y > 0 ? y : 0;
}
__host__ __device__ inline uint32_t pack_mv(rv_mv m) {
  return ((uint32_t)(uint16_t)m.row << 16) | (uint16_t)m.col;
}
__device__ inline void block_atomic_add(uint64_t s, unsigned long long *out) {
  __shared__ uint64_t red[4];
  s = group_sum<64>(s);
  if ((threadIdx.x & 63) == 0) red[threadIdx.x >> 6] = s;
  __syncthreads();
  if (threadIdx.x == 0) {
    uint64_t t = 0;
    for (int i = 0; i < (int)(blockDim.x >> 6); i++) t += red[i];
    if (t) atomicAdd(out, (unsigned long long)t);
  }
}

constexpr int kLevels = 4;

struct CandKey {
  uint32_t tag, mv0, mv1;
};

struct XRect {
  int64_t off;
  int plane, x0, y0, w, h;
};

enum StageEv {
  kEvStart = 0,
  kEvF0,
  kEvF1,
  kEvF2,
  kEvFL,
  kEvF3Full,
  kEvF3Sub,
  kEvF4Single,
  kEvF4Comp,
  kEvArgmin,
  kEvCommit,
  kEvIntra,
  kEvF5,
  kEvF7,
  kEvLaBegin,
  kEvLaEnd,
  kEvEdgeBegin,
  kEvEdgeEnd,
  kEvF8Begin,
  kEvF8End,
  kEvCount
};

}

using namespace rv;

struct RvSlot {
  rv_plane y, u, v;
  rv_mv *fmv = nullptr;
};
struct RvInput {
  rv_plane y, u, v;
  rv_plane hres, qres;
  uint32_t *qres_box = nullptr;
};

struct EcHost {
  std::thread th;
  std::mutex mu;
  std::condition_variable cv;
  struct Item {
    int slot, level, qctx;
  };
  std::deque<Item> q;
  bool stop = false;
  long queued = 0, done = 0;
  int ntiles = 1;
  uint32_t *tok_h[2] = {nullptr, nullptr}, *stat_h[2] = {nullptr, nullptr};
  hipEvent_t ev[2] = {nullptr, nullptr};
  bool busy[2] = {false, false};
  std::vector<uint16_t> chain[3];
  uint64_t stat[5] = {0, 0, 0, 0, 0};
  int err = 0;

  void code(const Item &it);
  void run();
  void drain();
};

struct RoundRing {
  static constexpr int kCnt = 64, kPub = 64;
  int32_t *cnt = nullptr;
  uint32_t *ticket = nullptr;
  unsigned long long *h_pub = nullptr, *d_pub = nullptr;
  uint32_t seq = 0;
  int last_count = -1;
  int32_t *slot(uint32_t q) const { return cnt + 2 * (q % kCnt); }
  RoundPub pub(uint32_t q, bool publish = true) const {
    return RoundPub{slot(q), slot(q + 1), ticket, publish ? d_pub + q % kPub : nullptr, q};
  }
};

struct LaRefs {
  int n, disp[kImpMaxRefs], order[kImpMaxRefs];
};

struct LaOut {
  rv_fs_result *coarse = nullptr, *half_l = nullptr, *look = nullptr;
};

constexpr int kEngineWaitS = 60;

struct rv_la_hub {
  static constexpr int kRing = 4;
  int n = 0;
  std::mutex mu;
  std::condition_variable cv;
  std::vector<long> posted;
  std::vector<uint8_t *> buf[kRing];
  std::vector<hipEvent_t> ev[kRing];
};

struct RvLaEngine {
  static constexpr int kLaSlack = 28;
  int W = 0, RW = 0, dev = 0;
  long limit = 0;
  Owned own;
  hipStream_t las = nullptr;
  RoundRing rr;
  int32_t *la_list = nullptr;
  void *scratch = nullptr;
  size_t scratch_bytes = 0;
  struct Entry {
    LaOut o;
    ImpFrame f;
    long m = -1;
    long used_by = -1;
    rv_replay_frame_info fi{};
    LaRefs lr{};
    hipEvent_t ev_imp = nullptr, ev_used = nullptr;
    hipEvent_t ev_data = nullptr, ev_xchg = nullptr;
  };
  std::vector<Entry> ring;
  std::vector<long> pyr_display;
  std::thread th;
  std::mutex mu;
  std::condition_variable cv;
  long requested = 0;
  long inputs_ready = 0;
  long imp_ready = 0;
  long imp_next = 1;
  bool stop = false;
  int err = 0;
  std::string msg;
  long la_round_sum = 0, la_reeval = 0, la_frames = 0;
  void *comm = nullptr;
  uint8_t *psend = nullptr, *precv = nullptr;
  size_t pbytes = 0;
  long data_ready = 0, xchg_done = 0, xchg_next = 1;
  rv_la_hub *hub = nullptr;
  int hub_k = -1;
  Entry &at(long m) { return ring[(size_t)(m % RW)]; }
};

struct rv_replay {
  rv_replay_cfg cfg{};
  Geo g{};
  int RA = 1;
  CandGeo cg{};
  Owned own;
  hipStream_t stream = nullptr;
  template <class T>
  T *dev(size_t n, Fill fill = Fill::None) { return own.dev<T>(n, fill, stream); }
  hipEvent_t ev_ielig = nullptr;
  bool overlap = false;
  bool own_stream = false;
  bool sea = false;
  struct Level {
    bool set = false;
    int qidx = 0;
    QCtx ql{}, qu{}, qv{};
    QCtx qil{}, qiu{}, qiv{};
    QCtx qs[kLevels][3] = {};
    double lambda = 0.0, me_lambda = 0.0, ds[3] = {0.0, 0.0, 0.0};
  } lv[3] = {};
  struct PLevel {
    int B = 0, n = 0, gw = 0, gh = 0, bc = 0, bch = 0, txl = 0, txc = 0;
    CandGeo cg{};
    rv_ds_job *jobs_full[3] = {nullptr, nullptr, nullptr}, *jobs_sub[3] = {nullptr, nullptr, nullptr};
    rv_fs_result *full = nullptr, *sub = nullptr;
    uint64_t *l_out = nullptr, *c_out = nullptr;
    RdoWinner *win = nullptr;
    int32_t *cand_list = nullptr, *cand_count = nullptr;
    int32_t *l_lev = nullptr, *c_lev = nullptr;
    int32_t *leaf = nullptr;
    size_t woff = 0;
  } pl[kLevels] = {};
  bool s6 = false;
  bool lvl = false;
  int ex0 = 0, ey0 = 0, ew = 0, eh = 0;
  bool lv_used[kLevels] = {false, false, false, false};
  bool lv_me[kLevels] = {false, false, false, false};
  hipStream_t edge[kLevels] = {nullptr, nullptr, nullptr, nullptr};
  hipEvent_t ev_efork = nullptr, ev_l1me = nullptr, ev_epart = nullptr;
  hipEvent_t ev_ejoin[kLevels] = {nullptr, nullptr, nullptr, nullptr};
  hipEvent_t ev_ecommit[kLevels] = {nullptr, nullptr, nullptr, nullptr};
  bool deblock = false;
  uint8_t *mi_lg = nullptr, *mi_skip = nullptr;
  int mi_stride = 0, mi_cols = 0, mi_rows = 0;
  uint8_t db_level[3] = {0, 0, 0};
  int64_t *db_tally = nullptr;
  uint8_t *db_dlev = nullptr;
  bool cdef = false;
  bool lrf = false;
  uint64_t *lrf_err = nullptr;
  int8_t *lrf_xqd = nullptr, *lrf_units = nullptr;
  int lrf_fix_passes = 1 << 30;
  RvInput lrf_out{};
  RvInput cdef_pre{};
  uint8_t *cdef_dir = nullptr, *cdef_idx = nullptr;
  int32_t *cdef_var = nullptr;
  uint8_t cdef_str[3][2] = {};
  int32_t *leaf_count = nullptr;
  bool entropy = false;
  EcFrameBufs ecb{};
  EcHost *ech = nullptr;
  long ec_frames = 0;
  bool intra = false;
  uint8_t *i_elig = nullptr, *i_was = nullptr, *i_win = nullptr, *i_modes = nullptr;
  int32_t *i_mark = nullptr, *i_list[2] = {nullptr, nullptr}, *i_commit = nullptr,
          *i_revert = nullptr;
  int32_t *i_cnt = nullptr;
  int32_t *h_cnt = nullptr;
  void *i_edges = nullptr;
  uint64_t *i_lout = nullptr, *i_cout = nullptr;
  uint32_t *i_stats = nullptr;
  bool exact = false;
  MvStack *stk = nullptr;
  BlkDec *dec_lv[3] = {nullptr, nullptr, nullptr};
  uint8_t *mv_active = nullptr;
  static constexpr int kRoundsAhead = 2;
  RoundRing rr;
  int32_t *mv_list = nullptr;
  bool edge_tr = false;
  long mv_round_sum = 0, mv_reeval = 0, mv_run_sum = 0;
  long mv_frames = 0;
  size_t nwords = 0, wpart = 0;
  bool jobs_built = false;
  std::mutex jobs_mu;
  std::vector<RvSlot> slots;
  std::vector<RvInput> inputs;
  rv_fs_job *fs_jobs[3] = {nullptr, nullptr, nullptr};
  rv_fs_result *coarse = nullptr, *half = nullptr, *full = nullptr, *sub = nullptr, *look = nullptr;
  rv_fs_result *half_l = nullptr;
  rv_ds_job *jobs_half[3] = {}, *jobs_full[3] = {}, *jobs_sub[3] = {}, *jobs_look[3] = {};
  rv_ds_job *jobs_half_l[3] = {nullptr, nullptr, nullptr};
  int32_t *la_list = nullptr;
  long la_round_sum = 0, la_reeval = 0;
  long la_frames = 0;
  RvLaEngine *eng = nullptr;
  bool eng_owned = false;
  const float *imp_last = nullptr;
  int32_t *src_half = nullptr, *src_full = nullptr, *src_look = nullptr;
  uint64_t *l_out = nullptr, *c_out = nullptr;
  RdoWinner *win = nullptr;
  int32_t *cand_list = nullptr, *cand_count = nullptr;
  RdoArgs *f4_args = nullptr;
  CandKey *cand_key = nullptr;
  uint8_t *f3dirty = nullptr;
  uint8_t *f2dirty = nullptr;
  uint32_t *cand_evals = nullptr;
  int32_t *l_lev = nullptr, *c_lev = nullptr;
  uint64_t *words = nullptr;
  unsigned long long *tail = nullptr;
  float *imp = nullptr;
  int n_imp = 0, imp_bx = 0, imp_by = 0, ntx_c = 0;
  long coded = 0;
  rv_replay_frame_info last{};
  int n_groups = 1, my_group = 0;
  int32_t grects[4 * kMaxGroups] = {};
  size_t xbytes = 0;
  uint8_t *xsend = nullptr, *xrecv = nullptr;
  void *comm = nullptr;
  static constexpr int kRing = 64;
  hipEvent_t evs[kRing][kEvCount] = {};
  int timing_stride = 1, timing_block = 1;
  long timed = 0;
  uint32_t *ds_evals = nullptr;
  static constexpr int kProbes = 2, kKpCnt = 4;
  bool kprobe = false;
  static constexpr int kKp = 512;
  std::vector<hipEvent_t> kp_ev[kProbes];
  long kp_n[kProbes] = {0, 0}, kp_done[kProbes] = {0, 0}, kp_base[kProbes] = {0, 0};
  long kp_init[kProbes] = {0, 0};
  static constexpr int kKpInit = 256;
  double kp_ms[kProbes] = {0.0, 0.0}, kp_dev_ms[kProbes] = {0.0, 0.0};
  uint32_t *kp_cnt[kProbes] = {nullptr, nullptr};
  unsigned long long *kp_ts[kProbes] = {nullptr, nullptr};
  double kp_tick_ms = 0.0;
};

template <typename Check, typename Eval>
int run_rounds(RoundRing &rr, hipStream_t xs, int budget, Check &&check, Eval &&eval,
               long *nrounds, long *nre, bool *changed, const char *what, long frame, int level) {
  static const bool mv_trace = getenv("RAV1E_HIP_MV_TRACE") != nullptr;
  if (changed) *changed = false;
  rr.last_count = -1;
  const uint32_t first = rr.seq++;
  RV_R(check(first));
  int queued = 0;
  for (int seen = 0;; seen++) {
    while (queued < budget && queued < seen + rv_replay::kRoundsAhead) {
      RV_R(eval(first + (uint32_t)queued));
      RV_R(check(rr.seq++));
      queued++;
    }
    const uint32_t q = first + (uint32_t)seen;
    volatile unsigned long long *pub = rr.h_pub + q % RoundRing::kPub;
    const auto t0 = std::chrono::steady_clock::now();
    unsigned long long v;
    for (long spin = 0;; spin++) {
      v = *pub;
      if ((uint32_t)(v >> 32) == q) break;
      if ((spin & 1023) == 1023) {
        const hipError_t he = hipStreamQuery(xs);
        if (he != hipSuccess && he != hipErrorNotReady)
          return rv_set_error(RV_EHIP, "rv_replay_frame: a round failed");
        if (std::chrono::steady_clock::now() - t0 > std::chrono::seconds(30))
          return rv_set_error(RV_EHIP, "rv_replay_frame: a round's count never arrived");
        std::this_thread::yield();
      }
    }
    const int c = (int)(uint32_t)v;
    rr.last_count = c;
    if (mv_trace) fprintf(stderr, "%s frame %ld level %d check %d: %d\n", what, frame, level, seen, c);
    if (c == 0) return RV_OK;
    if (seen >= budget)
      return rv_set_error(RV_EHIP, "rv_replay_frame: rounds beyond the chain's dependency "
                                   "depth (internal error)");
    *nre += c;
    (*nrounds)++;
    if (changed) *changed = true;
  }
}

namespace rv {

inline bool groups_active(const rv_replay *r) { return r->n_groups >= 2 || r->comm; }

hipError_t kp_harvest(rv_replay *r, int p, long upto);
size_t plane_bytes(const rv_plane &p);
void round_ring_alloc(Owned &dev, Owned &host, RoundRing &q, hipStream_t st);
int ensure_jobs(rv_replay *r);
int group_rects(const rv_replay *r, int k, XRect out[9], int *n);
int xcopy(rv_replay *r, const RvSlot &s, const XRect *rects, int n, int to_plane, uint8_t *buf);
int lrf_decide_slot(rv_replay *r, const RvSlot &s, const RvInput &in, int lv, const LrfGeo &lg,
                    const int32_t *rect);
int filter_slot(rv_replay *r, const RvSlot &s, const RvInput &in, int lv);
void frame_info(long n, int R, rv_replay_frame_info *f);
LaRefs la_refs_of(long m, int R);

int lookahead_frame(rv_replay *r, RoundRing &rr, hipStream_t xs, const rv_replay_frame_info &fi,
                    const LaRefs &lr, long frame, const LaOut &o, int32_t *la_list, bool pyramid,
                    long *nrounds, long *nre, hipEvent_t *e);
void la_engine_destroy(rv_replay *r);
int la_encode_exchange(rv_replay *r, long n, hipStream_t st);
int la_engine_take(rv_replay *r, long n, hipStream_t st, const float **imp);
int la_engine_release(rv_replay *r, long n, hipStream_t st);

}
```

rav1e_amd/csrc/rv_replay.hip:

```cpp
#include "rv_replay.h"

namespace rv {

__global__ void coeff_checksum(const int32_t *packed, int64_t total, int per_block,
                               unsigned long long *out) {
  uint64_t s = 0;
  for (int64_t i = (int64_t)blockIdx.x * blockDim.x + threadIdx.x; i < total;
       i += (int64_t)gridDim.x * blockDim.x)
    s += (uint64_t)(int64_t)packed[i] * (uint64_t)(i % per_block + 1);
  block_atomic_add(s, out);
}

template <typename Px>
__global__ void sum_rect(rv_plane p, int x0, int y0, int w, int h, unsigned long long *out) {
  uint64_t s = 0;
  for (int64_t i = (int64_t)blockIdx.x * blockDim.x + threadIdx.x; i < (int64_t)w * h;
       i += (int64_t)gridDim.x * blockDim.x) {
    const int y = (int)(i / w), x = (int)(i - (int64_t)y * w);
    s += *plane_ptr<Px>(p, x0 + x, y0 + y);
  }
  block_atomic_add(s, out);
}

struct XArgs {
// ... 613 lines not shown
            if (inside && !pin) r->lv_used[l] = true;
          }
      }
    }
    if (x1 >= 0) {
      r->lvl = true;
      r->ex0 = x0;
      r->ey0 = y0;
      r->ew = x1 - x0 + 1;
      r->eh = y1 - y0 + 1;
    }
  }
  if (!r->lvl) return RV_OK;
  r->lv_me[1] = r->lv_used[1] || r->lv_used[2] || r->lv_used[3];
  r->lv_me[2] = r->lv_used[2];
  r->lv_me[3] = r->lv_used[3];
  rv_replay::PLevel &P0 = r->pl[0];
  P0.B = kSb;
  P0.n = g.nsb;
  P0.gw = g.tw;
  P0.gh = g.th;
  for (int l = 1; l < kLevels; l++) {
    rv_replay::PLevel &P = r->pl[l];
    const int k = 1 << l;
    P.B = kSb >> l;
    P.gw = r->ew * k;
    P.gh = r->eh * k;
    P.n = P.gw * P.gh;
    P.bc = P.B >> g.xdec;
    P.bch = P.B >> g.ydec;
    P.txl = 4 - l;
    P.txc = P.bc == 32 ? 3 : P.bc == 16 ? 2 : P.bc == 8 ? 1 : 0;
    P.cg = CandGeo{P.n, P.gw, P.gh, (g.tx0 + r->ex0) * k, (g.ty0 + r->ey0) * k, g.tws * k,
                   g.ths * k, g.R, g.M, 0};
    P.woff = r->nwords;
    r->nwords += (size_t)P.n * (4 * g.R + 4);
  }
  r->wpart = r->nwords;
  r->nwords += (size_t)g.nsb;
  return RV_OK;
}

static int configure_stages(rv_replay *r) {
  const Geo &g = r->g;
  const uint32_t flags = r->cfg.flags;
  r->intra = !r->s6 && !(flags & RV_REPLAY_NO_INTRA) && g.xdec == 1 && g.ydec == 1;
  r->exact = !r->s6 && !(flags & RV_REPLAY_MVREF_STANDIN);
  for (int sb = 0; sb < g.nsb && r->exact && r->lvl; sb++) {
    const int fsx = g.tx0 + sb % g.tw, fsy = g.ty0 + sb / g.tw;
    const int t0x = fsx - fsx % g.tws;
    const int cols = std::min(g.tws * 16, g.w_in_b - t0x * 16);
    if ((fsx + 1) * 64 <= g.W && (fsy + 1) * 64 <= g.H && fsy % g.ths != 0 &&
        (fsx - t0x) * 16 + 16 < cols && (fsx + 2) * 64 > g.W)
      r->edge_tr = true;
  }
  if (flags & RV_REPLAY_CDEF) {
    if (!(flags & RV_REPLAY_DEBLOCK) || (g.W & 7) || (g.H & 7))
      return rv_set_error(RV_EINVAL, "rv_replay_create: RV_REPLAY_CDEF needs RV_REPLAY_DEBLOCK and a "
                                     "frame size that is a multiple of 8");
    r->cdef = true;
  }
  if (flags & RV_REPLAY_LRF) {
    LrfGeo lg;
    if (!r->cdef || g.xdec != g.ydec ||
        lrf_geometry(g.W, g.H, g.xdec, g.ydec, g.bd, 100, g.tws, g.ths, &lg) != RV_OK)
      return rv_set_error(RV_EINVAL, "rv_replay_create: RV_REPLAY_LRF needs RV_REPLAY_CDEF, 4:2:0 or 4:4:4 "
                                     "(rav1e's enable_restoration is off in 4:2:2) and units of one superblock");
    r->lrf = true;
    const char *fe = getenv("RAV1E_LRF_FIX"), *fp = getenv("RAV1E_LRF_FIX_PASSES");
    r->lrf_fix_passes = (fe && fe[0] == '0') ? 0 : fp ? std::max(atoi(fp), 1) : 1 << 30;
  }
  r->entropy = (flags & RV_REPLAY_ENTROPY) != 0;
  if (r->entropy && g.xdec != g.ydec)
    return rv_set_error(RV_EINVAL, "rv_replay_create: RV_REPLAY_ENTROPY needs xdec == ydec");
  r->deblock = (flags & RV_REPLAY_DEBLOCK) != 0;
  if (r->deblock || r->entropy) {
    r->mi_cols = (g.W + 3) / 4;
    r->mi_rows = (g.H + 3) / 4;
    r->mi_stride = (r->mi_cols + 15) / 16 * 16;
  }
  if (r->entropy) {
    EcFrameBufs &b = r->ecb;
    b.ntiles = ((g.tw + g.tws - 1) / g.tws) * ((g.th + g.ths - 1) / g.ths);
    b.max_jobs = ec_max_jobs(g.nsb, b.ntiles);
    b.map_w4 = g.tws * 16;
    b.map_h4 = g.ths * 16;
    b.cap = (uint32_t)((size_t)g.nsb * (1024 + 2 * r->ntx_c * 1024) + (size_t)b.max_jobs * 4);
  }
  const char *e = getenv("RAV1E_HIP_REPLAY_SERIAL");
  r->overlap = !(e && e[0] == '1');
  return RV_OK;
}

static int replay_configure(const rv_replay_cfg *cfg, rv_replay *r) {
  if (!cfg || cfg->width <= 0 || cfg->height <= 0 || (cfg->width & 7) || (cfg->height & 7) ||
      (cfg->bit_depth != 8 && cfg->bit_depth != 10 && cfg->bit_depth != 12) || cfg->xdec < 0 ||
      cfg->xdec > 1 || cfg->ydec < 0 || cfg->ydec > 1 || cfg->n_refs < 1 || cfg->n_refs > 2 ||
      cfg->n_inputs < 1 || cfg->tile_w_sb < 0 || cfg->tile_h_sb < 0)
    return rv_set_error(RV_EINVAL, "rv_replay_create: bad config");
  r->cfg = *cfg;
  Geo &g = r->g;
  g.W = cfg->width;
  g.H = cfg->height;
  g.xdec = cfg->xdec;
  g.ydec = cfg->ydec;
  g.bd = cfg->bit_depth;
  g.hbd = cfg->bit_depth > 8;
  g.w_in_b = 2 * ((g.W + 7) >> 3);
  g.h_in_b = 2 * ((g.H + 7) >> 3);
  const int sbc = (g.W + kSb - 1) / kSb, sbr = (g.H + kSb - 1) / kSb;
  g.tx0 = cfg->tile_x0;
  g.ty0 = cfg->tile_y0;
  g.tw = cfg->tile_w > 0 ? cfg->tile_w : sbc - g.tx0;
  g.th = cfg->tile_h > 0 ? cfg->tile_h : sbr - g.ty0;
  g.tws = cfg->tile_w_sb > 0 ? cfg->tile_w_sb : sbc;
  g.ths = cfg->tile_h_sb > 0 ? cfg->tile_h_sb : sbr;
  if (g.tx0 < 0 || g.ty0 < 0 || g.tw <= 0 || g.th <= 0 || g.tx0 + g.tw > sbc ||
      g.ty0 + g.th > sbr || g.tx0 % g.tws || g.ty0 % g.ths ||
      ((g.tx0 + g.tw) % g.tws && g.tx0 + g.tw != sbc) ||
      ((g.ty0 + g.th) % g.ths && g.ty0 + g.th != sbr))
    return rv_set_error(RV_EINVAL,
                        "rv_replay_create: the tile group is not a rectangle of whole tiles");
  g.vis_w = (g.W - g.tx0 * kSb) < g.tw * kSb ? g.W - g.tx0 * kSb : g.tw * kSb;
  g.vis_h = (g.H - g.ty0 * kSb) < g.th * kSb ? g.H - g.ty0 * kSb : g.th * kSb;
  g.nsb = g.tw * g.th;
  g.R = cfg->n_refs;
  r->RA = g.R == 2 ? kImpMaxRefs : g.R;
  g.M = kCandModes;
  g.C = g.R * g.M + (g.R == 2 ? kCompModes : 0);
  g.cw = kSb >> g.xdec;
  g.ch = kSb >> g.ydec;
  g.w_imp = g.w_in_b / 2;
  g.h_imp = g.h_in_b / 2;
  r->cg = CandGeo{g.nsb, g.tw, g.th, g.tx0, g.ty0, g.tws, g.ths, g.R, g.M, 0};
  r->sea = g.bd <= 10 && (cfg->flags & RV_REPLAY_EXHAUSTIVE_FS) == 0;
  r->ntx_c = (g.cw / 32) * (g.ch / 32);
  r->imp_bx = g.vis_w / 8;
  r->imp_by = g.vis_h / 8;
  r->n_imp = r->imp_bx * r->imp_by;
  const int32_t me[4] = {g.tx0, g.ty0, g.tw, g.th};
  memcpy(r->grects, me, sizeof(me));
  RV_R(configure_levels(r));
  return configure_stages(r);
}

static void alloc_dpb(rv_replay *r, const rv_replay *share) {
  r->slots = share ? share->slots : std::vector<RvSlot>(kSlots);
  r->inputs = share ? share->inputs : std::vector<RvInput>(r->cfg.n_inputs);
  if (share) return;
  for (auto &s : r->slots) alloc_slot(r, s);
  for (auto &in : r->inputs) alloc_input(r, in, true);
}

static void alloc_superblocks(rv_replay *r) {
  const Geo &g = r->g;
  const size_t nsb = (size_t)g.nsb, nr = nsb * g.R, nc = nsb * g.C;
  r->coarse = r->dev<rv_fs_result>(nr);
  r->half = r->dev<rv_fs_result>(nr * 4);
  r->look = r->dev<rv_fs_result>(nr * 16, Fill::Zero);
  r->half_l = r->dev<rv_fs_result>(nr * 4, Fill::Zero);
  r->la_list = r->dev<int32_t>(nr * 20);
  r->full = r->dev<rv_fs_result>(nr);
  r->sub = r->dev<rv_fs_result>(nr);
  r->ds_evals = r->dev<uint32_t>((size_t)rv_replay::kRing * 2 * nr, Fill::Zero);
  r->l_out = r->dev<uint64_t>(nc * 3);
  r->c_out = r->dev<uint64_t>(nc * r->ntx_c * 3 * 2);
  r->win = r->dev<RdoWinner>(nsb);
  r->cand_list = r->dev<int32_t>(nc);
  r->cand_key = r->dev<CandKey>(nsb * (g.R * g.M + kCompModes), Fill::Zero);
  r->f3dirty = r->dev<uint8_t>(nsb * g.R);
  r->f2dirty = r->dev<uint8_t>(nsb * g.R * 4);
  r->cand_count = r->dev<int32_t>(2, Fill::Zero);
  r->f4_args = r->dev<RdoArgs>(4);
  r->cand_evals = r->dev<uint32_t>((size_t)rv_replay::kRing * 2 * kLevels, Fill::Zero);
  r->l_lev = r->dev<int32_t>(nsb * 1024, Fill::Zero);
  r->c_lev = r->dev<int32_t>(nsb * r->ntx_c * 1024 * 2, Fill::Zero);
  r->words = r->dev<uint64_t>(r->nwords, Fill::Zero);
  r->tail = r->dev<unsigned long long>(5, Fill::Zero);
}

static void alloc_levels(rv_replay *r) {
  if (!r->lvl) return;
  size_t nleaf = (size_t)r->g.nsb;
  for (int l = 1; l < kLevels; l++) {
    rv_replay::PLevel &P = r->pl[l];
    const size_t n = (size_t)P.n, nr = n * r->g.R, nc = n * r->g.C;
    P.full = r->dev<rv_fs_result>(nr);
    P.sub = r->dev<rv_fs_result>(nr);
    P.l_out = r->dev<uint64_t>(nc * 3);
    P.c_out = r->dev<uint64_t>(nc * 3 * 2);
    P.win = r->dev<RdoWinner>(n);
    P.cand_list = r->dev<int32_t>(nc);
    P.cand_count = r->dev<int32_t>(2, Fill::Zero);
    P.l_lev = r->dev<int32_t>(n * P.B * P.B, Fill::Zero);
    P.c_lev = r->dev<int32_t>(n * P.bc * P.bch * 2, Fill::Zero);
    nleaf += n;
  }
  int32_t *lf = r->dev<int32_t>(nleaf);
  r->leaf_count = r->dev<int32_t>(kLevels, Fill::Zero);
  for (int l = 0; l < kLevels && lf; l++) {
    r->pl[l].leaf = lf;
    lf += r->pl[l].n;
  }
}

static void alloc_intra(rv_replay *r) {
  r->i_stats = r->dev<uint32_t>((size_t)rv_replay::kRing * 3, Fill::Zero);
  if (!r->intra) return;
  const size_t n = (size_t)r->g.nsb;
  r->i_elig = r->dev<uint8_t>(n);
  r->i_was = r->dev<uint8_t>(n, Fill::Zero);
  r->i_win = r->dev<uint8_t>(2 * n, Fill::Zero);
  r->i_modes = r->dev<uint8_t>(4 * n);
  for (int32_t **list : {&r->i_mark, &r->i_list[0], &r->i_list[1], &r->i_commit, &r->i_revert})
    *list = r->dev<int32_t>(n);
  r->i_cnt = r->dev<int32_t>(4);
  r->i_edges = r->dev<uint8_t>(n * 3 * kIntraEdge * (r->g.hbd ? 2 : 1));
  r->i_lout = r->dev<uint64_t>(n * 3 * 3);
  r->i_cout = r->dev<uint64_t>(n * 6 * 3 * 2);
  r->h_cnt = r->own.pinned<int32_t>(4, hipHostMallocDefault);
  r->ev_ielig = r->own.event(hipEventDisableTiming);
}

static void alloc_mvref(rv_replay *r) {
  round_ring_alloc(r->own, r->own, r->rr, r->stream);
  if (!r->exact) return;
  const size_t n = (size_t)r->g.nsb;
  r->stk = r->dev<MvStack>(n);
  for (int l = 0; l < 3; l++) r->dec_lv[l] = r->dev<BlkDec>(n, Fill::Zero);
  r->mv_active = r->dev<uint8_t>(n);
  r->mv_list = r->dev<int32_t>(2 * n);
}

static void alloc_filters(rv_replay *r) {
  const Geo &g = r->g;
  const size_t n8 = (size_t)(g.W / 8) * (g.H / 8), n64 = (size_t)((g.W + 63) / 64) * ((g.H + 63) / 64);
  if (r->cdef) {
    r->cdef_dir = r->dev<uint8_t>(n8);
    r->cdef_var = r->dev<int32_t>(n8);
    r->cdef_idx = r->dev<uint8_t>(n64, Fill::Zero);
    alloc_input(r, r->cdef_pre, false);
  }
  if (r->lrf) {
    r->lrf_err = r->dev<uint64_t>(3 * n64 * 17);
    r->lrf_xqd = r->dev<int8_t>(3 * n64 * 32);
    r->lrf_units = r->dev<int8_t>(3 * n64 * 3);
    alloc_input(r, r->lrf_out, false);
  }
  if (!r->deblock && !r->entropy) return;
  const size_t mb = (size_t)r->mi_stride * (r->mi_rows + 16);
  r->mi_lg = r->dev<uint8_t>(mb, Byte(4));
  r->mi_skip = r->dev<uint8_t>(mb, Fill::Zero);
  if (r->s6 && r->deblock) {
    r->db_tally = r->dev<int64_t>(3 * 130);
    r->db_dlev = r->dev<uint8_t>(4);
  }
}

static void alloc_sync(rv_replay *r) {
  for (int f = 0; f < rv_replay::kRing; f++)
    for (int i = 0; i < kEvCount; i++) r->evs[f][i] = r->own.event(hipEventDisableSystemFence);
  if (!r->overlap || !r->lvl || r->s6) return;
  for (hipEvent_t *ev : {&r->ev_efork, &r->ev_l1me, &r->ev_epart})
    *ev = r->own.event(hipEventDisableTiming);
  const hipStream_t es = r->own.stream();
  for (int l = 1; l < kLevels; l++) {
    r->edge[l] = es;
    r->ev_ejoin[l] = r->own.event(hipEventDisableTiming);
    r->ev_ecommit[l] = r->own.event(hipEventDisableTiming);
  }
}

static void alloc_entropy(rv_replay *r) {
  if (!r->entropy) return;
  EcFrameBufs &b = r->ecb;
  b.jobs = r->dev<rv_ec_job>((size_t)b.max_jobs);
  b.sb_off = r->dev<uint32_t>((size_t)r->g.nsb + 1);
  b.map = r->dev<uint8_t>((size_t)b.ntiles * 3 * b.map_w4 * b.map_h4);
  b.scratch = r->dev<uint8_t>(rv_ec_scratch_bytes(b.max_jobs));
  b.offsets = r->dev<uint32_t>((size_t)b.max_jobs + 1);
  b.dstat = r->dev<uint32_t>(4);
  EcHost *eh = r->ech = new EcHost();
  eh->ntiles = b.ntiles;
  for (int k = 0; k < 2; k++) {
    eh->tok_h[k] = r->own.pinned<uint32_t>(b.cap, hipHostMallocMapped | hipHostMallocCoherent);
    eh->stat_h[k] = r->own.pinned<uint32_t>((size_t)b.ntiles + 8, hipHostMallocMapped | hipHostMallocCoherent);
    eh->ev[k] = r->own.event(hipEventBlockingSync | hipEventDisableTiming);
  }
  if (!r->own.failed) eh->th = std::thread([eh] { eh->run(); });
}

}

extern "C" {

void rv_replay_destroy(rv_replay *r) {
  if (!r) return;
  la_engine_destroy(r);
  if (r->stream) (void)hipStreamSynchronize(r->stream);
  if (r->ech) {
    {
      std::lock_guard<std::mutex> lk(r->ech->mu);
      r->ech->stop = true;
    }
    r->ech->cv.notify_all();
    if (r->ech->th.joinable()) r->ech->th.join();
    delete r->ech;
  }
  if (r->edge[1]) (void)hipStreamSynchronize(r->edge[1]);
  r->own.release();
  delete r;
}

static rv_replay *create_impl(const rv_replay_cfg *cfg, void *stream, const rv_replay *share) {
// ... 531 lines not shown
```

rav1e_amd/csrc/rv_replay_frame.hip:

```cpp
#include "rv_replay.h"

namespace rv {

struct CandCost {
  double rs, rn;
  uint64_t ds, dn;
  int live;
};
__device__ inline CandCost cand_cost(const CandGeo &cg, double lambda, double ds_u, double ds_v,
                                     const rv_fs_result *sub, const uint64_t *lout,
                                     const uint64_t *uout, const uint64_t *vout, int ntx_c, int sb,
                                     int c) {
  CandCost k{0.0, 0.0, 0, 0, 0};
  const int ns = cg.R * cg.M;
  rv_mv mv;
  if (c < ns ? !cand_live(cg, sub, sb, c, &mv) : !comp_live(cg, sub, sb, c - ns)) return k;
  k.live = 1;
  const int64_t o = (int64_t)c * cg.nsb + sb;
  uint64_t su = 0, sv = 0, nu = 0, nv = 0;
  uint32_t rate = (uint32_t)lout[o * 3 + 2];
  for (int j = 0; j < ntx_c; j++) {
    const int64_t t = (o * ntx_c + j) * 3;
    su += uout[t];
    sv += vout[t];
// ... 533 lines not shown
  ~SideJoin() {
    for (int l = 1; l < kLevels; l++)
      if (armed && r->edge[l]) (void)hipStreamSynchronize(r->edge[l]);
  }
};

struct HostTrace {
  using hclock = std::chrono::steady_clock;
  hclock::time_point h0 = hclock::now(), take = h0, r0 = h0, mv = h0, intra = h0;
  static hclock::time_point now() { return hclock::now(); }
  void report(long frame, int lv) const {
    static const bool host_trace = getenv("RAV1E_HIP_HOST_TRACE") != nullptr;
    if (!host_trace) return;
    auto us = [](hclock::time_point a, hclock::time_point b) {
      return (long)std::chrono::duration_cast<std::chrono::microseconds>(b - a).count();
    };
    static thread_local hclock::time_point prev_end = h0;
    const auto h1 = hclock::now();
    fprintf(stderr, "host frame %ld level %d: since-last-exit %ld take %ld r0 %ld mv %ld intra %ld tail %ld us\n",
            frame, lv, us(prev_end, h0), us(h0, take), us(take, r0), us(r0, mv), us(mv, intra),
            us(intra, h1));
    prev_end = h1;
  }
};

struct KProbe {
  rv_replay *r;
  bool on;
  uint32_t *acc(int p) const { return on ? r->kp_cnt[p] : nullptr; }
  int open(hipStream_t xs, int p = 0) const {
    if (!on) return RV_OK;
    if (r->kp_n[p] >= r->kp_init[p]) {
      constexpr long K = rv_replay::kKp, C = rv_replay::kKpInit;
      static_assert(C <= K, "the initialised slots fit the ring");
      const long need = r->kp_n[p] + C - K;
      if (r->kp_done[p] < need) RV_H(kp_harvest(r, p, need));
      static const std::vector<unsigned long long> init = [] {
        std::vector<unsigned long long> v(2 * (size_t)C, 0ull);
        for (long i = 0; i < C; i++) v[2 * (size_t)i] = ~0ull;
        return v;
      }();
      const long s0 = r->kp_n[p] % K, first = std::min(C, K - s0);
      RV_H(hipMemcpyAsync(r->kp_ts[p] + 2 * s0, init.data(), 2 * sizeof(unsigned long long) * first,
                          hipMemcpyHostToDevice, xs));
      if (C > first)
        RV_H(hipMemcpyAsync(r->kp_ts[p], init.data(), 2 * sizeof(unsigned long long) * (C - first),
                            hipMemcpyHostToDevice, xs));
      r->kp_init[p] = r->kp_n[p] + C;
    }
    RV_H(hipEventRecord(r->kp_ev[p][2 * (size_t)(r->kp_n[p] % rv_replay::kKp)], xs));
    return RV_OK;
  }
  unsigned long long *ts(int p = 0) const {
    return on ? r->kp_ts[p] + 2 * (size_t)(r->kp_n[p] % rv_replay::kKp) : nullptr;
  }
  int close(hipStream_t xs, int p = 0) const {
    if (!on) return RV_OK;
    RV_H(hipEventRecord(r->kp_ev[p][2 * (size_t)(r->kp_n[p] % rv_replay::kKp) + 1], xs));
    r->kp_n[p]++;
    return RV_OK;
  }
};

struct FrameRun {
  rv_replay *const r;
  const Geo &g;
  const rv_replay_frame_info &fi;
  HostTrace &tr;
  const int lv;
  const rv_replay::Level &L;
  hipStream_t const st;
  const RvInput &cur;
  const RvSlot &S;
  CandGeo cg;
  const RvSlot *ref[RV_MAX_REFS];
  rv_plane refs_y[RV_MAX_REFS], refs_h[RV_MAX_REFS], refs_o[RV_MAX_REFS];
  const int nr;
  const long ncoded;
  const int slot;
  uint32_t *ev_full, *ev_sub;
  ChainNext to_sub;
  const EpzsGeo eg;
  const LvPlace place;
  const bool tm;
  hipEvent_t *e;
  const KProbe kp;
  const float *imp = nullptr;
  const uint8_t *const act;
  const int nsingle, ntx_c;
  const int64_t nct;
  const bool f4_list;
  RdoArgs f4h[4], la, ca;
  RdoArgs ll[kLevels], lc6[kLevels];
  MvrefArgs ma;
  uint32_t q_first = 0;
  int mv_runs = 0;
  const int budget;

  static LvPlace placement(const rv_replay *r) {
    if (!r->lvl) return LvPlace::kNone;
    if (!r->s6 && r->edge[1]) return LvPlace::kEdge;
    return r->exact ? LvPlace::kEarly : LvPlace::kRound0;
  }

  FrameRun(rv_replay *r_, const rv_replay_frame_info &fi_, HostTrace &tr_)
      : r(r_), g(r_->g), fi(fi_), tr(tr_), lv(fi_.level), L(r_->lv[fi_.level]), st(r_->stream),
        cur(r_->inputs[fi_.display % r_->inputs.size()]), S(r_->slots[fi_.display % kSlots]),
        cg(r_->cg), nr(r_->g.nsb), ncoded(r_->coded - 1),
        slot((int)((r_->coded - 1) % rv_replay::kRing)),
        to_sub{kChainFullToSub, r_->jobs_sub[fi_.level]},
        eg{g.tx0, g.ty0, g.tw, g.th, g.tws, g.ths, g.W, g.H, g.w_in_b, g.h_in_b},
        place(placement(r_)),
        tm(r_->timing_stride > 0 && (ncoded / r_->timing_block) % r_->timing_stride == 0),
        e(r_->evs[r_->timed % rv_replay::kRing]), kp{r_, tm && r_->kprobe && !r_->s6},
        act(r_->exact ? r_->mv_active : nullptr), nsingle(g.nsb * g.R * g.M), ntx_c(r_->ntx_c),
        nct((int64_t)g.nsb * g.C * r_->ntx_c), f4_list(g.bd != 12),
        budget(g.tws + 2 * g.ths - 2) {
    cg.comp = fi.compound ? kCompModes : 0;
    cg.stk = r->exact ? r->stk : nullptr;
    for (int k = 0; k < g.R; k++) {
      ref[k] = &r->slots[fi.ref_display[k] % kSlots];
      refs_y[k] = ref[k]->y;
      const RvInput &ri = r->inputs[fi.ref_display[k] % r->inputs.size()];
      refs_h[k] = ri.hres;
      refs_o[k] = ri.y;
    }
    ev_full = r->ds_evals + (size_t)slot * 2 * nr * g.R;
    ev_sub = ev_full + (size_t)nr * g.R;
    if (tm) r->timed++;
    memset(&ma, 0, sizeof(ma));
  }

  int ev(StageEv i, hipStream_t xs) const {
    if (tm) RV_H(hipEventRecord(e[i], xs));
    return RV_OK;
  }
  int ev(StageEv i) const { return ev(i, st); }
  Levels searched(int only) const { return Levels{r->lv_me, only}; }
  Levels used(int only = 0) const { return Levels{r->lv_used, only}; }
  int32_t *slot_cnt(uint32_t q) const { return r->rr.slot(q); }
  int32_t *mvl(uint32_t q) const { return r->mv_list + (size_t)(q & 1) * g.nsb; }

  int take_lookahead() {
    imp = r->imp;
    if (r->eng) {
      RV_R(la_encode_exchange(r, r->coded, st));
      RV_R(la_engine_take(r, r->coded, st, &imp));
      for (StageEv i : {kEvF0, kEvF1, kEvF2, kEvLaBegin, kEvLaEnd}) RV_R(ev(i));
    } else {
      LaRefs er;
      memset(&er, 0, sizeof(er));
      er.n = g.R;
      for (int k = 0; k < g.R; k++) er.disp[k] = fi.ref_display[k], er.order[k] = k;
      RV_R(lookahead_frame(r, r->rr, st, fi, er, ncoded, LaOut{r->coarse, r->half_l, r->look}, r->la_list,
                           true, &r->la_round_sum, &r->la_reeval, tm ? e : nullptr));
      r->la_frames++;
    }
    r->imp_last = imp;
    tr.take = HostTrace::now();
    return RV_OK;
  }

  void level_args(int l, RdoArgs a, RdoArgs c) {
    const rv_replay::PLevel &P = r->pl[l];
    CandGeo cgl = P.cg;
    cgl.comp = cg.comp;
    const int ns = P.n * g.R * g.M;
    a.p[0].levels = P.l_lev;
    a.p[0].out = P.l_out;
    a.p[0].q = L.qs[l][0];
    a.g = cgl;
    a.sub = P.sub;
    a.win = P.win;
    a.n_tx = ns;
    a.list = P.cand_list;
    a.count = P.cand_count;
    a.ntx_per_cand = 1;
    a.bsize = P.B;
    a.mb_w = a.mb_h = P.B;
    a.q_tx_index = P.txl * 16;
    a.tx_size = P.txl;
    for (int q = 0; q < 2; q++) {
      c.p[q].levels = P.c_lev + (size_t)q * P.n * P.bc * P.bch;
      c.p[q].out = P.c_out + (size_t)q * P.n * g.C * 3;
      c.p[q].q = L.qs[l][1 + q];
    }
    c.g = cgl;
    c.sub = P.sub;
    c.win = P.win;
    c.n_tx = ns;
    c.list = P.cand_list;
    c.count = P.cand_count;
    c.ntx_per_cand = 1;
    c.bsize = P.B;
    c.mb_w = P.bc;
    c.mb_h = P.bch;
    c.sub_w = (P.bc < 8 ? P.bc : 8) >> g.xdec;
    c.sub_h = (P.bch < 8 ? P.bch : 8) >> g.ydec;
    c.q_tx_index = P.txc * 16;
    c.tx_size = P.txc;
    ll[l] = a;
    lc6[l] = c;
  }

  void build_args() {
    memset(&la, 0, sizeof(la));
    la.p[0].org = cur.y;
    for (int k = 0; k < g.R; k++) la.p[0].ref[k] = ref[k]->y;
    la.p[0].dst = S.y;
    la.p[0].levels = r->l_lev;
    la.p[0].out = r->l_out;
    la.g = cg;
    la.sub = r->sub;
    la.win = r->win;
    la.imp = imp;
    la.w_in_b = g.w_in_b;
    la.h_in_b = g.h_in_b;
    la.w_imp = g.w_imp;
    la.n_tx = nsingle;
    la.list = r->cand_list;
    la.count = r->cand_count;
    la.ntx_per_cand = 1;
    la.bd = g.bd;
    la.bsize = kSb;
    la.mb_w = la.mb_h = kSb;
    la.sub_w = la.sub_h = 8;
    la.p[0].q = L.ql;
    la.q_tx_index = 4 * 16 + 0;
    la.tx_size = 4;
    la.qindex = L.qidx;
    ca = la;
    const rv_plane cur_c[2] = {cur.u, cur.v}, s_c[2] = {S.u, S.v};
    for (int p = 0; p < 2; p++) {
      ca.p[p].org = cur_c[p];
      for (int k = 0; k < g.R; k++) ca.p[p].ref[k] = p ? ref[k]->v : ref[k]->u;
      ca.p[p].dst = s_c[p];
      ca.p[p].levels = r->c_lev + (size_t)p * g.nsb * ntx_c * 1024;
      ca.p[p].out = r->c_out + (size_t)p * nct * 3;
      ca.p[p].q = p ? L.qv : L.qu;
    }
    ca.n_tx = nsingle * ntx_c;
    ca.ntx_per_cand = ntx_c;
    ca.mb_w = g.cw;
    ca.mb_h = g.ch;
    ca.xdec = g.xdec;
    ca.ydec = g.ydec;
    ca.sub_w = (g.cw < 8 ? g.cw : 8) >> g.xdec;
    ca.sub_h = (g.ch < 8 ? g.ch : 8) >> g.ydec;
    ca.q_tx_index = 3 * 16 + 0;
    ca.tx_size = 3;
    f4h[0] = f4h[2] = la;
    f4h[1] = f4h[3] = ca;
    f4h[2].list = f4h[3].list = r->cand_list + nsingle;
    f4h[2].count = f4h[3].count = r->cand_count + 1;
    f4h[2].cand_base = f4h[3].cand_base = 0;
    f4h[2].n_tx = g.nsb * cg.comp;
    f4h[3].n_tx = g.nsb * cg.comp * ntx_c;
    if (place != LvPlace::kNone)
      for (int l : used()) level_args(l, la, ca);
    la.commit = ca.commit = 1;
    la.list = ca.list = r->lvl ? r->pl[0].leaf : nullptr;
    la.count = ca.count = r->lvl ? r->leaf_count : nullptr;
    la.n_tx = g.nsb;
    ca.n_tx = g.nsb * ntx_c;
    la.ntx_per_cand = 1;
  }

  int lv_me(hipStream_t es, int only = 0) {
    for (int l : searched(only)) {
      rv_replay::PLevel &P = r->pl[l];
      if (l == 1)
        seed_level_kernel<<<(P.n * g.R + 255) / 256, 256, 0, es>>>(
            P.jobs_full[lv], P.n, P.gw, g.R, r->half_l, g.nsb, 0, 0, r->ex0, r->ey0, g.tw);
      else
        seed_level_kernel<<<(P.n * g.R + 255) / 256, 256, 0, es>>>(
            P.jobs_full[lv], P.n, P.gw, g.R, r->pl[1].sub, r->pl[1].n, r->pl[1].gw, 1 << (l - 1),
            0, 0, 0);
      ChainNext to_s{kChainFullToSub, P.jobs_sub[lv]};
      RV_R(rv_diamond_search_multi(&cur.y, refs_y, g.R, P.jobs_full[lv], P.n, P.B, P.B, 0, 0, 0,
                                   g.bd, P.full, nullptr, &to_s, es));
      RV_R(rv_diamond_search_multi(&cur.y, refs_y, g.R, P.jobs_sub[lv], P.n, P.B, P.B, 1,
                                   r->s6 ? 1 : 0, 0, g.bd, P.sub, nullptr, nullptr, es));
    }
    return RV_OK;
  }
  void lv_lists(hipStream_t es, bool comp, int only = 0) {
    for (int l : used(only)) {
      rv_replay::PLevel &P = r->pl[l];
      const int ns = P.n * g.R * g.M;
      if (!comp) {
        cand_list_kernel<<<(ns + 255) / 256, 256, 0, es>>>(P.cg, P.sub, ns, P.cand_list,
                                                            P.cand_count);
      } else {
        CandGeo cgl = P.cg;
        cgl.comp = cg.comp;
        comp_list_kernel<<<(P.n * cg.comp + 255) / 256, 256, 0, es>>>(
            cgl, P.sub, ns, P.cand_list + ns, P.cand_count + 1);
      }
    }
  }
  int lv_rdo(hipStream_t es, int only = 0) {
    for (int l : used(only))
      RV_R(rv_rdo_blocks2(ll[l], lc6[l], r->pl[l].B, r->pl[l].bc, g.hbd, es, 0));
    return RV_OK;
  }
  int lv_rdo_comp(hipStream_t es, int only = 0) {
    for (int l : used(only)) {
// ... 504 lines not shown
```

rav1e_amd/csrc/rv_replay_la.hip:

```cpp
#include "rv_replay.h"

namespace rv {

struct LaArgs {
  Geo g;
  EpzsGeo eg;
  rv_ds_job *jh, *jl;
  const int32_t *sl;
  const rv_fs_result *coarse, *half_l, *look;
  int32_t *list_h, *list_l;
  int init;
  int what;
  int nref;
  RoundPub pub;
};

__device__ inline rv_mv la_coarse4(const LaArgs &a, int k, int sb) {
  const rv_mv c = a.coarse[(size_t)k * a.g.nsb + sb].best_mv;
  return rv_mv{(int16_t)(c.row * 4), (int16_t)(c.col * 4)};
}

__global__ __launch_bounds__(256) void la_check_kernel(LaArgs a) {
  const Geo &g = a.g;
  const int nh = (a.what & 1) ? a.nref * g.nsb * 4 : 0, nl = (a.what & 2) ? a.nref * g.nsb * 16 : 0;
  const int i = blockIdx.x * 256 + threadIdx.x;
  bool mh = false, ml = false;
  int job = 0;
  if (i < nh) {
    job = i;
    const int k = i / (g.nsb * 4), sb = (i / 4) % g.nsb, q = i % 4;
    const int sx = sb % g.tw, sy = sb / g.tw;
    int t0x, t0y, mi_w, mi_h;
    sb_tile(g, sx, sy, t0x, t0y, mi_w, mi_h);
    const int fsx = g.tx0 + sx, fsy = g.ty0 + sy, tsx = fsx - t0x, tsy = fsy - t0y;
    const int tsw = (mi_w + 15) / 16, tsh = (mi_h + 15) / 16;
    const bool hh = (q & 1) ? tsx < tsw - 1 : tsx > 0, hv = (q >> 1) ? tsy < tsh - 1 : tsy > 0;
    const rv_mv ch = hh ? la_coarse4(a, k, (q & 1) ? sb + 1 : sb - 1) : rv_mv{0, 0};
    const rv_mv cv = hv ? la_coarse4(a, k, (q >> 1) ? sb + g.tw : sb - g.tw) : rv_mv{0, 0};
    const rv_mv cm[3] = {la_coarse4(a, k, sb), hh ? ch : cv, cv};
    const int nc = 1 + (int)hh + (int)hv;
    int bx = tsx * 16 + (q & 1) * 8, by = tsy * 16 + (q >> 1) * 8;
    adjust_bo(mi_w, mi_h, bx, by, 32, 32);
    auto rd = [&](int X4, int Y4) {
      const int SX = X4 >> 4, SY = Y4 >> 4;
      if (SX == fsx && SY == fsy) return rv_mv{0, 0};
      const int gsb = (SY - g.ty0) * g.tw + (SX - g.tx0);
      const rv_mv h =
          a.half_l[((size_t)k * g.nsb + gsb) * 4 + ((Y4 >> 3) & 1) * 2 + ((X4 >> 3) & 1)].best_mv;
      return rv_mv{(int16_t)(h.row * 2), (int16_t)(h.col * 2)};
    };
    mh = epzs_update(a.jh + i, 1, a.eg, t0x * 16, t0y * 16, mi_w, bx, by, cm, nc, rd, nullptr, 1) &&
         !a.init;
  } else if (i - nh < nl) {
    const int j = i - nh;
    job = j;
    const int k = j / (g.nsb * 16), sb = (j / 16) % g.nsb, b = j % 16;
    const int sx = sb % g.tw, sy = sb / g.tw;
    int t0x, t0y, mi_w, mi_h;
    sb_tile(g, sx, sy, t0x, t0y, mi_w, mi_h);
    const int tsx = g.tx0 + sx - t0x, tsy = g.ty0 + sy - t0y;
    rv_mv cm[6];
    int nc = 0;
    bool more = true;
#pragma unroll
    for (int p = 1; p < 7; p++) {
      const int v = more ? a.sl[8 * j + p] : -1;
      more = more && v >= 0;
      const rv_mv m = !more ? rv_mv{0, 0}
                            : (v & 1) ? a.half_l[v >> 1].best_mv : a.coarse[v >> 1].best_mv;
      const int sc = (v & 1) ? 2 : 4;
      cm[p - 1] = rv_mv{(int16_t)(m.row * sc), (int16_t)(m.col * sc)};
      nc += more ? 1 : 0;
    }
    int bx = tsx * 16 + (b % 4) * 4, by = tsy * 16 + (b / 4) * 4;
    adjust_bo(mi_w, mi_h, bx, by, 16, 16);
    auto rd = [&](int X4, int Y4) {
      const int gsb = ((Y4 >> 4) - g.ty0) * g.tw + ((X4 >> 4) - g.tx0);
      return a.look[((size_t)k * g.nsb + gsb) * 16 + ((Y4 & 15) >> 2) * 4 + ((X4 & 15) >> 2)]
          .best_mv;
    };
    ml = epzs_update(a.jl + j, 0, a.eg, t0x * 16, t0y * 16, mi_w, bx, by, cm, nc, rd, nullptr, 1) &&
         !a.init;
  }
  const int lane = threadIdx.x & 63;
  const uint64_t below = (1ull << lane) - 1;
  const uint64_t bh = __ballot(mh), bl = __ballot(ml);
  int b0 = 0, b1 = 0;
  if (lane == 0) {
    if (bh) b0 = atomicAdd(a.pub.cnt, (int)__popcll(bh));
    if (bl) b1 = atomicAdd(a.pub.cnt + 1, (int)__popcll(bl));
  }
  b0 = __shfl(b0, 0, 64);
  b1 = __shfl(b1, 0, 64);
  if (mh) a.list_h[b0 + __popcll(bh & below)] = job;
  if (ml) a.list_l[b1 + __popcll(bl & below)] = job;
  round_publish(a.pub);
}

int lookahead_frame(rv_replay *r, RoundRing &rr, hipStream_t xs,
                    const rv_replay_frame_info &fi, const LaRefs &lr, long frame,
                    const LaOut &o, int32_t *la_list, bool pyramid, long *nrounds,
                    long *nre, hipEvent_t *e) {
  const Geo &g = r->g;
  const int lv = fi.level, nr = g.nsb, RL = lr.n;
  const RvInput &cur = r->inputs[fi.display % r->inputs.size()];
  rv_plane refs_h[kImpMaxRefs], refs_q[kImpMaxRefs], refs_o[kImpMaxRefs];
  const uint32_t *box[kImpMaxRefs];
  for (int k = 0; k < RL; k++) {
    const RvInput &ri = r->inputs[lr.disp[k] % r->inputs.size()];
    refs_h[k] = ri.hres;
    refs_q[k] = ri.qres;
    refs_o[k] = ri.y;
    box[k] = ri.qres_box;
  }
  auto ev = [&](StageEv i) -> int {
    if (e) RV_H(hipEventRecord(e[i], xs));
    return RV_OK;
  };
  if (pyramid) {
    RV_R(rv_plane_pyramid(&cur.y, &cur.hres, &cur.qres, xs));
    if (r->sea) RV_R(rv_plane_box_sums(&cur.qres, cur.qres_box, xs));
  }
  RV_R(ev(kEvF0));
  RV_R(rv_full_search_multi(&cur.qres, refs_q, RL, r->fs_jobs[lv], nr, 16, 16, 1, 0, o.coarse,
                            nullptr, r->sea ? box : nullptr, xs));
  RV_R(ev(kEvF1));
  LaArgs la_a;
  memset(&la_a, 0, sizeof(la_a));
  la_a.g = g;
  la_a.eg = EpzsGeo{g.tx0, g.ty0, g.tw, g.th, g.tws, g.ths, g.W, g.H, g.w_in_b, g.h_in_b};
  la_a.jh = r->jobs_half_l[lv];
  la_a.jl = r->jobs_look[lv];
  la_a.sl = r->src_look;
  la_a.coarse = o.coarse;
  la_a.half_l = o.half_l;
  la_a.look = o.look;
  const int nh = nr * RL * 4, nl = nr * RL * 16;
  la_a.nref = RL;
  la_a.list_h = la_list;
  la_a.list_l = la_list + nh;
  auto la_launch = [&](int what, uint32_t q, bool init) -> int {
    la_a.what = what;
    la_a.init = init ? 1 : 0;
    la_a.pub = rr.pub(q, !init);
    const int n = ((what & 1) ? nh : 0) + ((what & 2) ? nl : 0);
    la_check_kernel<<<(n + 255) / 256, 256, 0, xs>>>(la_a);
    RV_H(hipGetLastError());
    return RV_OK;
  };
  auto f2l = [&](const int32_t *list, const int32_t *cnt) {
    return rv_diamond_search_multi(&cur.hres, refs_h, RL, r->jobs_half_l[lv], nr * 4, 16, 16, 0,
                                   0, 0, g.bd, o.half_l, nullptr, nullptr, xs, nullptr, list, cnt,
                                   0);
  };
  auto fl = [&](const int32_t *list, const int32_t *cnt) {
    return rv_diamond_search_multi(&cur.y, refs_o, RL, r->jobs_look[lv], nr * 16, 16, 16, 0, 0, 0,
                                   g.bd, o.look, nullptr, nullptr, xs, nullptr, list, cnt, 0);
  };
  RV_R(la_launch(1, 0, true));
  RV_R(f2l(nullptr, nullptr));
  RV_R(ev(kEvF2));
  RV_R(ev(kEvLaBegin));
  RV_R(la_launch(2, 0, true));
  RV_R(fl(nullptr, nullptr));
  (*nrounds)++;
  RV_R(run_rounds(
      rr, xs, 5 * (g.tws + g.ths), [&](uint32_t q) { return la_launch(3, q, false); },
      [&](uint32_t q) -> int {
        RV_R(f2l(la_list, rr.slot(q)));
        return fl(la_list + nh, rr.slot(q) + 1);
      },
      nrounds, nre, nullptr, "lookahead", frame, lv));
  RV_R(ev(kEvLaEnd));
  return RV_OK;
}

static long coded_of_display(long d) {
  if (d == 0) return 0;
  static const int jof[4] = {0, 2, 1, 3}, off[4] = {4, 2, 1, 3};
  const int j = jof[d % 4];
  return 4 * ((d - off[j]) / 4) + j + 1;
}

static int la_exchange(rv_replay *r, long m, RvLaEngine::Entry &e, int R, hipStream_t xs) {
  RvLaEngine &E = *r->eng;
  const Geo &g = r->g;
  const int ng = r->n_groups;
  if (ng <= 1 && !E.comm) {
    if (g.tx0 || g.ty0 || g.vis_w != g.W || g.vis_h != g.H)
      return rv_set_error(RV_EINVAL, "rv_replay_frame: a tile group's window needs the other groups "
                                     "(rv_replay_set_groups + rv_replay_set_la_exchange)");
    return RV_OK;
  }
  auto rect = [&](int j) { return r->grects + 4 * j; };
  (void)R;
  if (E.comm) {
    RV_H(hipEventRecord(e.ev_data, xs));
    std::unique_lock<std::mutex> lk(E.mu);
    E.data_ready = m;
    E.cv.notify_all();
    if (!E.cv.wait_for(lk, std::chrono::seconds(kEngineWaitS),
                       [&] { return E.stop || E.xchg_done >= m; }))
      return rv_set_error(RV_EHIP, "la_exchange: the frame's parts were never all-gathered");
    if (E.stop) return rv_set_error(RV_EINVAL, "la_exchange: stopped");
    lk.unlock();
    RV_H(hipStreamWaitEvent(xs, e.ev_xchg, 0));
    return RV_OK;
  }
  rv_la_hub *h = E.hub;
  if (!h || h->n != ng)
    return rv_set_error(RV_EINVAL, "rv_replay_frame: a tile group's window needs an exchange "
                                   "(rv_replay_set_la_exchange)");
  const int k = E.hub_k, slot = (int)(m % rv_la_hub::kRing);
  const int32_t *me = rect(k);
  RV_R(impwin_part(e.f, R, me[0], me[1], me[2], me[3], g.w_imp, g.h_imp, h->buf[slot][k], false, xs));
  RV_H(hipEventRecord(h->ev[slot][k], xs));
  {
    std::unique_lock<std::mutex> lk(h->mu);
    h->posted[k] = m;
    h->cv.notify_all();
    if (!h->cv.wait_for(lk, std::chrono::seconds(kEngineWaitS), [&] {
          for (int j = 0; j < ng; j++)
            if (h->posted[j] < m) return false;
          return true;
        }))
      return rv_set_error(RV_EHIP, "la_exchange: a group's part never arrived");
  }
  for (int j = 0; j < ng; j++) {
    if (j == k) continue;
    RV_H(hipStreamWaitEvent(xs, h->ev[slot][j], 0));
    RV_R(impwin_part(e.f, R, rect(j)[0], rect(j)[1], rect(j)[2], rect(j)[3], g.w_imp, g.h_imp,
                     h->buf[slot][j], true, xs));
  }
  return RV_OK;
}

static int la_step(rv_replay *r, long m) {
  RvLaEngine &E = *r->eng;
  const Geo &g = r->g;
  hipStream_t xs = E.las;
  RvLaEngine::Entry &e = E.at(m);
  if (m - E.RW >= 1) RV_H(hipStreamWaitEvent(xs, e.ev_used, 0));
  rv_replay_frame_info fi;
  frame_info(m, g.R, &fi);
  const LaRefs lr = la_refs_of(m, g.R);
  long ds[1 + kImpMaxRefs];
  int nd = 0;
  ds[nd++] = fi.display;
  for (int k = 0; k < lr.n; k++) ds[nd++] = lr.disp[k];
  for (int i = 0; i < nd; i++) {
    const size_t idx = (size_t)(ds[i] % (long)r->inputs.size());
    if (E.pyr_display[idx] == ds[i]) continue;
    const RvInput &in = r->inputs[idx];
    RV_R(rv_plane_pyramid(&in.y, &in.hres, &in.qres, xs));
    if (r->sea) RV_R(rv_plane_box_sums(&in.qres, in.qres_box, xs));
    E.pyr_display[idx] = ds[i];
  }
  const size_t nr = (size_t)g.nsb * lr.n;
  if (m > 1) {
    const RvLaEngine::Entry &p = E.at(m - 1);
    RV_H(hipMemcpyAsync(e.o.half_l, p.o.half_l, nr * 4 * sizeof(rv_fs_result),
                        hipMemcpyDeviceToDevice, xs));
    RV_H(hipMemcpyAsync(e.o.look, p.o.look, nr * 16 * sizeof(rv_fs_result),
                        hipMemcpyDeviceToDevice, xs));
  }
  long la_rounds = 0, la_reeval = 0;
  RV_R(lookahead_frame(r, E.rr, xs, fi, lr, m - 1, e.o, E.la_list, false, &la_rounds, &la_reeval,
                       nullptr));
  {
    std::lock_guard<std::mutex> lk(E.mu);
    E.la_round_sum += la_rounds;
    E.la_reeval += la_reeval;
    E.la_frames++;
  }
  rv_plane refs_o[kImpMaxRefs];
  for (int k = 0; k < lr.n; k++) refs_o[k] = r->inputs[lr.disp[k] % r->inputs.size()].y;
  e.m = m;
  e.fi = fi;
  e.lr = lr;
  RV_R(impwin_group_data(r->inputs[fi.display % r->inputs.size()].y, refs_o, lr.n, g.bd, e.o.look,
                         g.tx0, g.ty0, g.tw, g.th, g.w_imp, g.h_imp, e.f, xs));
  RV_R(la_exchange(r, m, e, lr.n, xs));
  RV_R(impwin_lists(e.f, lr.n, g.w_imp, g.h_imp, E.scratch, E.scratch_bytes, xs));
  const long last_frame = E.limit > 0 ? E.limit - 1 : -1;
  const size_t ni = (size_t)g.w_imp * g.h_imp;
  while (E.imp_next <= m && (E.imp_next + E.W <= m || m == last_frame)) {
    const long n = E.imp_next, last = n + E.W < m ? n + E.W : m;
    {
      std::vector<float *> zs;
      for (long t = n; t <= last; t++) zs.push_back(E.at(t).f.imp);
      RV_R(impwin_zero(zs.data(), (int)zs.size(), (int)ni, xs));
    }
    for (long s2 = last; s2 > n; s2--) {
      const RvLaEngine::Entry &es = E.at(s2);
      const int nu = es.lr.n;
      int ks[kImpMaxRefs], np = 0;
      float *dst[kImpMaxRefs];
      for (int j = 0; j < nu; j++) {
        const int k = es.lr.order[j];
        const long t = coded_of_display(es.lr.disp[k]);
        if (t < n) continue;
        for (int i = 0; i < np; i++)
          if (dst[i] == E.at(t).f.imp)
            return rv_set_error(RV_EINVAL, "la_step: two passes into one frame");
        ks[np] = k;
        dst[np++] = E.at(t).f.imp;
      }
      if (np) RV_R(impwin_pass(es.f, ks, dst, np, nu, g.w_imp, g.h_imp, xs));
    }
    RV_R(impwin_final(E.at(n).f, g.w_imp, g.h_imp, xs));
    RV_H(hipEventRecord(E.at(n).ev_imp, xs));
    std::lock_guard<std::mutex> lk(E.mu);
    E.imp_ready = n;
    E.imp_next = n + 1;
    E.cv.notify_all();
  }
  return RV_OK;
}

static void la_thread_main(rv_replay *r) {
  RvLaEngine &E = *r->eng;
  (void)hipSetDevice(E.dev);
  for (long m = 1;; m++) {
    {
      std::unique_lock<std::mutex> lk(E.mu);
      E.cv.wait(lk, [&] {
        if (E.stop) return true;
        if (E.requested < 1 && E.inputs_ready == 0) return false;
        if (m > E.requested + E.W && 4 * ((m - 1) / 4) + 4 >= E.inputs_ready) return false;
        if (E.limit > 0 && m >= E.limit) return false;
        return m - E.RW < 1 || E.at(m).used_by == m - E.RW;
      });
      if (E.stop) return;
    }
    if (!E.las) E.las = E.own.stream();
    int rc = E.las ? RV_OK : rv_set_error(RV_EHIP, "the lookahead engine's stream");
    if (rc == RV_OK) rc = ensure_jobs(r);
    if (rc == RV_OK) rc = la_step(r, m);
    if (rc != RV_OK) {
      std::lock_guard<std::mutex> lk(E.mu);
      E.err = rc;
      E.msg = rv_last_error();
      E.cv.notify_all();
      return;
    }
  }
}

void la_engine_destroy(rv_replay *r) {
  RvLaEngine *E = r->eng;
  if (E && r->eng_owned) {
    {
      std::lock_guard<std::mutex> lk(E->mu);
      E->stop = true;
      E->cv.notify_all();
    }
    if (E->th.joinable()) E->th.join();
    if (E->las) (void)hipStreamSynchronize(E->las);
    E->own.release();
    delete E;
  }
  r->eng = nullptr;
}

int la_encode_exchange(rv_replay *r, long n, hipStream_t st) {
  RvLaEngine &E = *r->eng;
  if (!E.comm) return RV_OK;
  if (!r->eng_owned)
    return rv_set_error(RV_EINVAL, "rv_replay_frame: RCCL lookahead parts on the primary only");
#if RV_HAVE_RCCL
  const Geo &g = r->g;
  long last = n + E.W;
  if (E.limit > 0 && last > E.limit - 1) last = E.limit - 1;
  {
    std::lock_guard<std::mutex> lk(E.mu);
    if (n > E.requested) E.requested = n;
    E.cv.notify_all();
  }
  for (long m = E.xchg_next; m <= last; m++) {
    {
      std::unique_lock<std::mutex> lk(E.mu);
      if (!E.cv.wait_for(lk, std::chrono::seconds(kEngineWaitS),
                         [&] { return E.err != 0 || E.data_ready >= m; }))
        return rv_set_error(RV_EHIP, "rv_replay_frame: the lookahead engine's part never came");
      if (E.err) return rv_set_error(E.err, E.msg.c_str());
    }
    RvLaEngine::Entry &e = E.at(m);
    if (e.m != m) return rv_set_error(RV_EINVAL, "rv_replay_frame: the lookahead ring lost a frame");
    const int R = e.lr.n;
    const int32_t *me = r->grects + 4 * r->my_group;
    RV_H(hipStreamWaitEvent(st, e.ev_data, 0));
    RV_R(impwin_part(e.f, R, me[0], me[1], me[2], me[3], g.w_imp, g.h_imp, E.psend, false, st));
    if (ncclAllGather(E.psend, E.precv, E.pbytes, ncclUint8, (ncclComm_t)E.comm, st) != ncclSuccess)
      return rv_set_error(RV_EHIP, "rv_replay_frame: ncclAllGather (lookahead parts)");
    for (int j = 0; j < r->n_groups; j++) {
      if (j == r->my_group) continue;
      const int32_t *q = r->grects + 4 * j;
      RV_R(impwin_part(e.f, R, q[0], q[1], q[2], q[3], g.w_imp, g.h_imp,
                       E.precv + (size_t)j * E.pbytes, true, st));
    }
    RV_H(hipEventRecord(e.ev_xchg, st));
    std::lock_guard<std::mutex> lk(E.mu);
    E.xchg_done = m;
    E.xchg_next = m + 1;
    E.cv.notify_all();
  }
  return RV_OK;
#else
  (void)n;
  (void)st;
  return rv_set_error(RV_EINVAL, "rv_replay_frame: built without RCCL");
#endif
}

int la_engine_take(rv_replay *r, long n, hipStream_t st, const float **imp) {
  RvLaEngine &E = *r->eng;
  if (E.limit > 0 && n >= E.limit)
    return rv_set_error(RV_EINVAL, "rv_replay_frame: past the stream's limit "
                                   "(rv_replay_set_imp_window)");
  {
    std::unique_lock<std::mutex> lk(E.mu);
    if (n > E.requested) E.requested = n;
    E.cv.notify_all();
    if (!E.cv.wait_for(lk, std::chrono::seconds(kEngineWaitS),
                       [&] { return E.err != 0 || E.imp_ready >= n; }))
      return rv_set_error(RV_EHIP, "rv_replay_frame: the lookahead engine did not deliver the "
                                   "frame's importances (a frame skipped and never coded?)");
    if (E.err) return rv_set_error(E.err, E.msg.c_str());
  }
  const RvLaEngine::Entry &e = E.at(n);
  if (e.m != n) return rv_set_error(RV_EINVAL, "rv_replay_frame: the lookahead ring lost a frame");
  RV_H(hipStreamWaitEvent(st, e.ev_imp, 0));
  const size_t nr = (size_t)r->g.nsb * r->g.R;
  RV_H(hipMemcpyAsync(r->coarse, e.o.coarse, nr * sizeof(rv_fs_result), hipMemcpyDeviceToDevice, st));
  RV_H(hipMemcpyAsync(r->half_l, e.o.half_l, nr * 4 * sizeof(rv_fs_result),
                      hipMemcpyDeviceToDevice, st));
  RV_H(hipMemcpyAsync(r->look, e.o.look, nr * 16 * sizeof(rv_fs_result), hipMemcpyDeviceToDevice,
                      st));
  *imp = e.f.fin;
  return RV_OK;
}

int la_engine_release(rv_replay *r, long n, hipStream_t st) {
  RvLaEngine &E = *r->eng;
  RvLaEngine::Entry &e = E.at(n);
  RV_H(hipEventRecord(e.ev_used, st));
  std::lock_guard<std::mutex> lk(E.mu);
  e.used_by = n;
  E.cv.notify_all();
  return RV_OK;
}

}

extern "C" {

int rv_replay_set_inputs_ready(rv_replay *r, long displays) {
  if (!r || displays < 0) return rv_set_error(RV_EINVAL, "rv_replay_set_inputs_ready: bad arguments");
  if (displays > (long)r->inputs.size())
    return rv_set_error(RV_EINVAL, "rv_replay_set_inputs_ready: more displays than input slots");
  if (r->eng) {
    RV_R(ensure_jobs(r));
    std::lock_guard<std::mutex> lk(r->eng->mu);
    r->eng->inputs_ready = displays;
    r->eng->cv.notify_all();
  }
  return RV_OK;
}

int rv_replay_set_imp_window(rv_replay *r, int window, long limit) {
  if (!r || window < 0 || window > 1024 || limit < 0)
    return rv_set_error(RV_EINVAL, "rv_replay_set_imp_window: bad arguments");
  if (r->coded > 0) return rv_set_error(RV_EINVAL, "rv_replay_set_imp_window: after the first frame");
  const Geo &g = r->g;
  if (r->eng && !r->eng_owned)
    return rv_set_error(RV_EINVAL, "rv_replay_set_imp_window: on the primary instance");
  la_engine_destroy(r);
  if (!window) return RV_OK;
  RvLaEngine *E = new RvLaEngine();
  E->W = window;
  E->RW = window + 1 + RvLaEngine::kLaSlack;
  E->limit = limit;
  E->own.failed = hipGetDevice(&E->dev) != hipSuccess;
  round_ring_alloc(r->own, E->own, E->rr, r->stream);
  const int ni = g.w_imp * g.h_imp, nr = g.nsb * r->RA;
  E->la_list = r->dev<int32_t>((size_t)nr * 20);
  E->scratch_bytes = impwin_scratch_bytes(ni);
  E->scratch = r->dev<uint8_t>(E->scratch_bytes);
  E->ring.resize((size_t)E->RW);
  const size_t ob = ((size_t)nr * 21 * sizeof(rv_fs_result) + 255) / 256 * 256;
  for (auto &en : E->ring) {
    uint8_t *m = r->dev<uint8_t>(ob + impwin_frame_bytes(ni, r->RA));
    if (!m || hipMemsetAsync(m, 0, ob, r->stream) != hipSuccess) E->own.failed = true;
    if (r->own.failed || E->own.failed) break;
    for (hipEvent_t *ev : {&en.ev_imp, &en.ev_used, &en.ev_data, &en.ev_xchg})
      *ev = E->own.event(hipEventDisableTiming);
    en.o.coarse = (rv_fs_result *)m;
    en.o.half_l = en.o.coarse + nr;
    en.o.look = en.o.half_l + (size_t)nr * 4;
    impwin_frame_carve(en.f, m + ob, ni, r->RA);
  }
  E->pyr_display.assign(r->inputs.size(), -1);
  r->eng = E;
  r->eng_owned = true;
  if (r->own.failed || E->own.failed || hipStreamSynchronize(r->stream) != hipSuccess) {
    la_engine_destroy(r);
    return rv_set_error(RV_EHIP, "rv_replay_set_imp_window: allocation failed");
  }
  E->th = std::thread(la_thread_main, r);
  return RV_OK;
}

rv_la_hub *rv_la_hub_create(int n_groups) {
  if (n_groups < 2 || n_groups > kMaxGroups) {
    rv_set_error(RV_EINVAL, "rv_la_hub_create: 2 .. kMaxGroups groups");
    return nullptr;
  }
  rv_la_hub *h = new rv_la_hub();
  h->n = n_groups;
  h->posted.assign((size_t)n_groups, 0);
  for (int s = 0; s < rv_la_hub::kRing; s++) {
    h->buf[s].assign((size_t)n_groups, nullptr);
    h->ev[s].assign((size_t)n_groups, nullptr);
  }
  return h;
}
void rv_la_hub_destroy(rv_la_hub *h) { delete h; }

int rv_replay_set_la_exchange(rv_replay *r, void *comm, rv_la_hub *hub) {
  if (!r || (!comm == !hub)) return rv_set_error(RV_EINVAL, "rv_replay_set_la_exchange: comm xor hub");
  if (!r->eng || !r->eng_owned || r->coded > 0)
    return rv_set_error(RV_EINVAL, "rv_replay_set_la_exchange: a primary instance with a window, "
                                   "before the first frame");
  if (r->n_groups < 2 && !comm)
    return rv_set_error(RV_EINVAL, "rv_replay_set_la_exchange: rv_replay_set_groups first");
  RvLaEngine &E = *r->eng;
  const Geo &g = r->g;
  size_t most = 0;
  for (int j = 0; j < r->n_groups; j++) {
    int bx0, by0, bw, bh;
    impwin_group_blocks(r->grects[4 * j], r->grects[4 * j + 1], r->grects[4 * j + 2],
                        r->grects[4 * j + 3], g.w_imp, g.h_imp, bx0, by0, bw, bh);
    const size_t b = (size_t)bw * bh * kImpPartBytes;
    most = b > most ? b : most;
  }
  E.pbytes = (most + 255) / 256 * 256;
  if (comm) {
    E.psend = r->dev<uint8_t>(E.pbytes);
    E.precv = r->dev<uint8_t>(E.pbytes * (size_t)r->n_groups);
    if (!E.psend || !E.precv) return rv_set_error(RV_EHIP, "rv_replay_set_la_exchange: alloc");
    E.comm = comm;
    return RV_OK;
  }
  if (hub->n != r->n_groups)
    return rv_set_error(RV_EINVAL, "rv_replay_set_la_exchange: the hub's group count");
  const int k = r->my_group;
  std::lock_guard<std::mutex> lk(hub->mu);
  for (int s = 0; s < rv_la_hub::kRing; s++) {
    if (hub->buf[s][k]) return rv_set_error(RV_EINVAL, "rv_replay_set_la_exchange: group joined twice");
    hub->buf[s][k] = r->dev<uint8_t>(E.pbytes);
    hub->ev[s][k] = E.own.event(hipEventDisableTiming);
    if (!hub->buf[s][k] || !hub->ev[s][k])
      return rv_set_error(RV_EHIP, "rv_replay_set_la_exchange: alloc");
  }
  E.hub = hub;
  E.hub_k = k;
  return RV_OK;
}

int rv_replay_get_importances(rv_replay *r, float *host, int n) {
  if (!r || !host || n != r->g.w_imp * r->g.h_imp)
    return rv_set_error(RV_EINVAL, "rv_replay_get_importances: bad arguments");
  RV_H(hipStreamSynchronize(r->stream));
  if (!r->imp_last) {
    memset(host, 0, (size_t)n * 4);
    return RV_OK;
  }
  RV_H(hipMemcpy(host, r->imp_last, (size_t)n * 4, hipMemcpyDeviceToHost));
  return RV_OK;
}

}
```

rav1e_amd/replay.py:

```python
from __future__ import annotations

import ctypes as C

import os

import numpy as np

from . import RvReplayCfg, RvReplayFrameInfo, RvReplayLevelParams, _check, lib
from . import rate as _rate

DEFAULT_QUANTIZER = 100

RV_REPLAY_EXHAUSTIVE_FS = 4
RV_REPLAY_SPEED6 = 8
RV_REPLAY_DEBLOCK = 16
RV_REPLAY_CDEF = 32
RV_REPLAY_LRF = 512
RV_REPLAY_NO_INTRA = 64
RV_REPLAY_ENTROPY = 128
RV_REPLAY_MVREF_STANDIN = 256
N_STAGES = 16

GOP_SCALES = (4, 2, 1, 1)

# ... 118 lines not shown
def tile_groups(tiling: dict, world: int) -> list:
    cols, rows = tiling["cols"], tiling["rows"]
    tws, ths = tiling["tile_width_sb"], tiling["tile_height_sb"]
    sbc, sbr = tiling["sb_cols"], tiling["sb_rows"]
    n = cols * rows
    if world < 1 or world > n:
        raise ValueError(f"{world} ranks for {n} tiles")
    out = []
    for r in range(world):
        a, b = r * n // world, (r + 1) * n // world
        tiles = [(i % cols, i // cols) for i in range(a, b)]
        c0, c1 = min(t[0] for t in tiles), max(t[0] for t in tiles)
        r0, r1 = min(t[1] for t in tiles), max(t[1] for t in tiles)
        if len(tiles) != (c1 - c0 + 1) * (r1 - r0 + 1):
            raise ValueError(f"tiles {a}..{b - 1} of a {cols}x{rows} grid are not a rectangle")
        x0, y0 = c0 * tws, r0 * ths
        out.append((x0, y0, min((c1 + 1) * tws, sbc) - x0, min((r1 + 1) * ths, sbr) - y0))
    return out


WORDS_PER_REF = 2 + 8 + 2 + 2 + 32 + 8
W_COARSE, W_HALF, W_FULL, W_SUB, W_LOOK, W_HALF_LA = 0, 2, 10, 12, 14, 46


def sb_words_per(n_refs):
    return WORDS_PER_REF * n_refs + 4


def level_rect(width, height, tile_w_sb=0, tile_h_sb=0, tile_x0=0, tile_y0=0, speed=10, xdec=1,
               ydec=1):
    sbc, sbr = (width + 63) // 64, (height + 63) // 64
    tw = tile_w_sb or (sbc - tile_x0)
    th = tile_h_sb or (sbr - tile_y0)
    if speed == 6:
        return (0, 0, tw, th)
    if xdec != ydec:
        return None
    edge = [(x, y) for y in range(th) for x in range(tw)
            if (tile_x0 + x + 1) * 64 > width or (tile_y0 + y + 1) * 64 > height]
    if not edge:
        return None
    xs, ys = [e[0] for e in edge], [e[1] for e in edge]
    return (min(xs), min(ys), max(xs) - min(xs) + 1, max(ys) - min(ys) + 1)


def result_words(width, height, n_refs, tile_w_sb=0, tile_h_sb=0, tile_x0=0, tile_y0=0,
                 speed=10, xdec=1, ydec=1):
    sbc, sbr = (width + 63) // 64, (height + 63) // 64
    tw = tile_w_sb or (sbc - tile_x0)
    th = tile_h_sb or (sbr - tile_y0)
    n = tw * th * sb_words_per(n_refs)
    rect = level_rect(width, height, tile_w_sb, tile_h_sb, tile_x0, tile_y0, speed, xdec, ydec)
    if rect:
        n += sum(rect[2] * rect[3] * 4 ** l * (4 * n_refs + 4) for l in (1, 2, 3)) + tw * th
    return n + 5


def level_words(width, height, n_refs, words, tile_w_sb=0, tile_h_sb=0, tile_x0=0, tile_y0=0,
                speed=6, xdec=1, ydec=1):
    sbc, sbr = (width + 63) // 64, (height + 63) // 64
    tw = tile_w_sb or (sbc - tile_x0)
    th = tile_h_sb or (sbr - tile_y0)
    nsb = tw * th
    rect = level_rect(width, height, tile_w_sb, tile_h_sb, tile_x0, tile_y0, speed, xdec, ydec)
    o = nsb * sb_words_per(n_refs)
    sbw = words[:o].reshape(nsb, sb_words_per(n_refs))
    lv = []
    for l in (1, 2, 3):
        n = rect[2] * rect[3] * 4 ** l
        lv.append(words[o:o + n * (4 * n_refs + 4)].reshape(n, 4 * n_refs + 4))
        o += n * (4 * n_refs + 4)
    return sbw, lv, words[o:o + nsb], words[o + nsb:]


class HipReplay:

    def __init__(self, width, height, xdec=1, ydec=1, bit_depth=8, n_refs=2, group=None,
                 tile_size=(0, 0), n_inputs=8, stream=None, flags=0,
                 quantizer=DEFAULT_QUANTIZER, imp_window=0, imp_limit=0):
        cfg = RvReplayCfg()
        cfg.width, cfg.height, cfg.xdec, cfg.ydec = width, height, xdec, ydec
        cfg.bit_depth, cfg.n_refs, cfg.n_inputs, cfg.flags = bit_depth, n_refs, n_inputs, flags
        cfg.tile_w_sb, cfg.tile_h_sb = tile_size
        if group:
            cfg.tile_x0, cfg.tile_y0, cfg.tile_w, cfg.tile_h = group
        self.cfg = cfg
        self.geom = (width, height, xdec, ydec, bit_depth)
        self.h = lib().rv_replay_create(C.byref(cfg), stream)
        if not self.h:
            raise RuntimeError(f"rv_replay_create: {lib().rv_last_error().decode()}")
        self.speed = 6 if flags & RV_REPLAY_SPEED6 else 10
        self.n_words = result_words(width, height, n_refs, cfg.tile_w, cfg.tile_h,
                                    cfg.tile_x0, cfg.tile_y0, self.speed, xdec, ydec)
        self.levels = _rate.level_params(quantizer, bit_depth)
        for lv, d in enumerate(self.levels):
            p = RvReplayLevelParams.from_dict(d)
            _check(lib().rv_replay_set_level_params(self.h, lv, C.byref(p)),
                   "rv_replay_set_level_params")
        self.imp_window = imp_window
        if imp_window:
            _check(lib().rv_replay_set_imp_window(self.h, int(imp_window), int(imp_limit)),
                   "rv_replay_set_imp_window")
        self.imp_shape = ((height + 7) // 8, (width + 7) // 8)

    def twin(self, stream=None):
        t = HipReplay.__new__(HipReplay)
        t.cfg, t.geom, t.speed, t.n_words, t.levels = self.cfg, self.geom, self.speed, \
            self.n_words, self.levels
        t.imp_window, t.imp_shape = self.imp_window, self.imp_shape
        t.h = lib().rv_replay_create_twin(self.h, stream)
        if not t.h:
            raise RuntimeError(f"rv_replay_create_twin: {lib().rv_last_error().decode()}")
        t.primary = self
        return t

    def seek(self, n: int):
        _check(lib().rv_replay_seek(self.h, int(n)), "rv_replay_seek")

    @property
    def stream(self):
        return lib().rv_replay_stream(self.h)

    def _frame_array(self):
        w, h, xd, yd, bd = self.geom
        n = frame_bytes(w, h, xd, yd, bd) // (2 if bd > 8 else 1)
        return np.zeros(n, dtype=np.uint16 if bd > 8 else np.uint8)

    def synth_inputs(self, t0: int = 0):
        _check(lib().rv_replay_synth_inputs(self.h, t0), "rv_replay_synth_inputs")

    def set_input(self, idx: int, yuv: np.ndarray):
        yuv = np.ascontiguousarray(yuv)
        _check(lib().rv_replay_set_input(self.h, idx, yuv.ctypes.data), "rv_replay_set_input")

    def get_input(self, idx: int) -> np.ndarray:
        out = self._frame_array()
        _check(lib().rv_replay_get_input(self.h, idx, out.ctypes.data), "rv_replay_get_input")
        return out

    def lrf_units(self, plane: int) -> np.ndarray:
        n = ((self.cfg.width + 63) // 64) * ((self.cfg.height + 63) // 64)
        out = np.zeros(3 * n, np.int8)
        _check(lib().rv_replay_lrf_units(self.h, plane, out.ctypes.data, out.size), "rv_replay_lrf_units")
        return out.reshape(n, 3)

    def get_recon(self, display: int) -> np.ndarray:
        out = self._frame_array()
        _check(lib().rv_replay_get_recon(self.h, display, out.ctypes.data), "rv_replay_get_recon")
        return out

    def set_inputs_ready(self, displays: int):
        _check(lib().rv_replay_set_inputs_ready(self.h, int(displays)),
               "rv_replay_set_inputs_ready")

    def set_importances(self, imp):
        if imp is None:
            _check(lib().rv_replay_set_importances(self.h, None, 0), "rv_replay_set_importances")
            return
        imp = np.ascontiguousarray(imp, dtype=np.float32)
        _check(lib().rv_replay_set_importances(self.h, imp.ctypes.data, imp.size),
               "rv_replay_set_importances")

    def importances(self) -> np.ndarray:
        out = np.zeros(self.imp_shape, np.float32)
        _check(lib().rv_replay_get_importances(self.h, out.ctypes.data, out.size),
               "rv_replay_get_importances")
        return out

    def frame(self) -> dict:
        fi = RvReplayFrameInfo()
        _check(lib().rv_replay_frame(self.h, C.byref(fi)), "rv_replay_frame")
        return {"display": fi.display, "me_range_scale": fi.me_range_scale, "level": fi.level,
                "is_key": fi.is_key, "ref_display": list(fi.ref_display),
                "compound": fi.compound}

    def set_la_exchange(self, comm=None, hub=None):
        _check(lib().rv_replay_set_la_exchange(self.h, comm, hub.h if hub else None),
               "rv_replay_set_la_exchange")

    def set_groups(self, rects, my_group, comm=None):
        arr = np.ascontiguousarray(np.asarray(rects, dtype=np.int32).ravel())
        _check(lib().rv_replay_set_groups(self.h, len(rects), arr.ctypes.data, my_group, comm),
               "rv_replay_set_groups")

    def exchange_buffers(self):
        s, r, n = C.c_void_p(), C.c_void_p(), C.c_size_t()
        _check(lib().rv_replay_exchange_buffers(self.h, C.byref(s), C.byref(r), C.byref(n)),
               "rv_replay_exchange_buffers")
        return s.value, r.value, n.value

    def import_(self):
        _check(lib().rv_replay_import(self.h), "rv_replay_import")

    def results(self) -> np.ndarray:
        out = np.zeros(self.n_words, dtype=np.uint64)
        n = lib().rv_replay_results(self.h, out.ctypes.data, out.size)
        if n < 0:
            _check(n, "rv_replay_results")
        return out[:n]

    def entropy_stats(self):
        out = np.zeros(5, np.uint64)
        n = lib().rv_replay_entropy_stats(self.h, out.ctypes.data, 5)
        if n < 0:
            _check(n, "rv_replay_entropy_stats")
        return [int(v) for v in out]

    def set_timing(self, stride: int, block: int = 1):
        _check(lib().rv_replay_set_timing(self.h, stride, block), "rv_replay_set_timing")

    def stage_ms(self) -> np.ndarray:
        out = np.zeros(N_STAGES, dtype=np.float32)
        n = lib().rv_replay_stage_times(self.h, out.ctypes.data, N_STAGES)
        if n < 0:
            _check(n, "rv_replay_stage_times")
        return out[:n]

    def stage_ms_sum(self, last_frames: int) -> np.ndarray:
        out = np.zeros(N_STAGES, dtype=np.float32)
        n = lib().rv_replay_stage_times_sum(self.h, last_frames, out.ctypes.data, N_STAGES)
        if n < 0:
            _check(n, "rv_replay_stage_times_sum")
        return out

    def set_kernel_probe(self, on: bool = True):
        _check(lib().rv_replay_set_kernel_probe(self.h, 1 if on else 0),
               "rv_replay_set_kernel_probe")

    def kernel_probe(self) -> np.ndarray:
        out = np.zeros(12, np.float64)
        _check(lib().rv_replay_kernel_probe(self.h, out.ctypes.data, 12) - 12,
               "rv_replay_kernel_probe")
        return out

    def counters(self) -> np.ndarray:
        out = np.zeros(21, dtype=np.uint64)
        _check(lib().rv_replay_counters(self.h, out.ctypes.data, 21) - 21, "rv_replay_counters")
        return out

    def close(self):
        if self.h:
            lib().rv_replay_destroy(self.h)
            self.h = None

    def __del__(self):
        try:
            self.close()
        except Exception:
            pass


def frame_info(n: int, n_refs: int = 2) -> dict:
    if n == 0:
        return {"display": 0, "me_range_scale": 0, "level": 0, "is_key": 1,
                "ref_display": [0, 0], "compound": 0}
    g, j = (n - 1) // 4, (n - 1) % 4
    rf = ((0, -4), (0, 4), (0, 2), (2, 4))[j]
    refs = [max(0, 4 * g + rf[k]) for k in range(n_refs)] + [0] * (2 - n_refs)
    return {"display": 4 * g + (4, 2, 1, 3)[j], "me_range_scale": (4, 2, 1, 1)[j],
            "level": (0, 1, 2, 2)[j], "is_key": 0, "ref_display": refs,
            "compound": int(n_refs == 2 and j in (1, 3))}


class PairedReplay:

    def __init__(self, primary: "HipReplay", twin_levels: str = None):
        import queue
        import threading
        self.twin_levels = twin_levels or os.environ.get("RAV1E_PAIRED_TWIN", "l2b")
        if self.twin_levels not in ("l2", "l2b", "alt"):
            raise ValueError(f"PairedReplay: twin_levels {self.twin_levels!r}")
        self.p = primary
        self.t = primary.twin()
        self.n = 0
        self.q = queue.Queue()
        self.err = None
        self._thr = threading
        self.ev_p = [lib().rv_event_create() for _ in range(8)]
        self.ev_t = [lib().rv_event_create() for _ in range(8)]
        self.ready_p, self.ready_t = {}, {}
        self.worker = threading.Thread(target=self._run, daemon=True)
        self.worker.start()

    def on_primary(self, f: int) -> bool:
        g, j = f // 4, f % 4
        if j < 2:
            return True
        if j == 3:
            return False
        return self.twin_levels == "l2b" or (self.twin_levels == "alt" and g % 2 == 0)

    def _flag(self, d, g):
        if g not in d:
            d[g] = self._thr.Event()
        return d[g]

    def frame(self) -> dict:
        n = self.n
        self.n += 1
        if n == 0:
            return self.p.frame()
        g, j = (n - 1) // 4, (n - 1) % 4
        if not self.on_primary(n - 1):
            self.q.put(n)
            return frame_info(n, self.p.cfg.n_refs)
        if j == 0 and g >= 2:
# ... 344 lines not shown
```

Measured before the change: 182.6.

## Skip unchanged lookahead EPZS jobs via stamps and fuse paired diamond rounds

Lookahead rounds now write a per-job stamp whenever the diamond search updates a job. The check kernel re-runs EPZS predictor updates only for jobs whose neighbour or source jobs were stamped in the previous round. The two per-round diamond searches (half-res and full-res) are merged into one paired kernel launch, with grid sizes taken from the previous round's count. An optional verify mode counts skipped jobs whose result would have changed. The risk is that the dependency tracking misses a source and gives different results, and that the adaptive grid caps leave work unprocessed.

Result: no change. 180.8 (-0.9%).

```diff
diff --git a/include/rav1e_hip.h b/include/rav1e_hip.h
--- a/include/rav1e_hip.h
+++ b/include/rav1e_hip.h
@@ -424,6 +424,8 @@
 int rv_replay_set_importances(rv_replay *r, const float *host, int n);
 int rv_replay_set_imp_window(rv_replay *r, int window, long limit);
 int rv_replay_set_inputs_ready(rv_replay *r, long displays);
+int rv_replay_set_la_verify(rv_replay *r, int on);
+int rv_replay_la_verify_counts(rv_replay *r, uint64_t *out, int cap);
 typedef struct rv_la_hub rv_la_hub;
 rv_la_hub *rv_la_hub_create(int n_groups);
 void rv_la_hub_destroy(rv_la_hub *hub);
diff --git a/rav1e_amd/__init__.py b/rav1e_amd/__init__.py
--- a/rav1e_amd/__init__.py
+++ b/rav1e_amd/__init__.py
@@ -289,6 +289,8 @@
         "rv_replay_set_importances": (i32, [vp, vp, i32]),
         "rv_replay_set_imp_window": (i32, [vp, i32, C.c_long]),
         "rv_replay_set_inputs_ready": (i32, [vp, C.c_long]),
+        "rv_replay_set_la_verify": (i32, [vp, i32]),
+        "rv_replay_la_verify_counts": (i32, [vp, vp, i32]),
         "rv_replay_get_importances": (i32, [vp, vp, i32]),
         "rv_replay_frame": (i32, [vp, C.POINTER(RvReplayFrameInfo)]),
         "rv_replay_set_groups": (i32, [vp, i32, vp, i32, vp]),
diff --git a/rav1e_amd/csrc/rv_epzs.h b/rav1e_amd/csrc/rv_epzs.h
--- a/rav1e_amd/csrc/rv_epzs.h
+++ b/rav1e_amd/csrc/rv_epzs.h
@@ -30,17 +30,28 @@
 }
 __device__ inline bool epzs_zero(rv_mv m) { return m.row == 0 && m.col == 0; }
 
+struct EpzsUnits {
+  bool hl, ht, htr;
+  int lx, ly, tx, ty, rx, ry;
+};
+__device__ inline EpzsUnits epzs_units(int tx4, int ty4, int mi_w, int bx, int by) {
+  const bool hl = bx > 0, ht = by > 0, htr = ht && bx < mi_w - 1;
+  return EpzsUnits{hl, ht, htr, tx4 + bx - 1, ty4 + by, tx4 + bx, ty4 + by - 1, tx4 + bx + 1,
+                   ty4 + by - 1};
+}
+
 template <int NCM, typename Rd>
 __device__ inline bool epzs_update(rv_ds_job *j, int shr, const EpzsGeo &g, int tx4, int ty4,
                                    int mi_w, int bx, int by, const rv_mv (&cm)[NCM], int ncm,
                                    Rd rd, const rv_mv *prev, int pr) {
   static_assert(NCM >= 1 && 1 + NCM + 4 + 5 <= RV_DS_MAX_PRED, "slots");
   constexpr int NS = 1 + NCM + 4 + 5;
-  const bool hl = bx > 0, ht = by > 0, htr = ht && bx < mi_w - 1;
+  const EpzsUnits u = epzs_units(tx4, ty4, mi_w, bx, by);
+  const bool hl = u.hl, ht = u.ht, htr = u.htr;
   const rv_mv z{0, 0};
-  const rv_mv l = hl ? rd(tx4 + bx - 1, ty4 + by) : z;
-  const rv_mv t = ht ? rd(tx4 + bx, ty4 + by - 1) : z;
-  const rv_mv tr = htr ? rd(tx4 + bx + 1, ty4 + by - 1) : z;
+  const rv_mv l = hl ? rd(u.lx, u.ly) : z;
+  const rv_mv t = ht ? rd(u.tx, u.ty) : z;
+  const rv_mv tr = htr ? rd(u.rx, u.ry) : z;
   rv_mv c[NS];
   uint32_t valid = 1;
   c[0] = z;
diff --git a/rav1e_amd/csrc/rv_me.h b/rav1e_amd/csrc/rv_me.h
--- a/rav1e_amd/csrc/rv_me.h
+++ b/rav1e_amd/csrc/rv_me.h
@@ -22,3 +22,9 @@
                      void *stream, const rv_ds_job *jobs_sub = nullptr,
                      rv_fs_result *out_sub = nullptr, uint32_t *eval_acc = nullptr,
                      unsigned long long *t01 = nullptr);
+int rv_diamond_la_pair(const rv_plane *org_h, const rv_plane *refs_h, const rv_ds_job *jobs_h,
+                       rv_fs_result *out_h, const int32_t *list_h, const int32_t *count_h,
+                       uint32_t *stamp_h, int g_h, const rv_plane *org, const rv_plane *refs,
+                       const rv_ds_job *jobs, rv_fs_result *out, const int32_t *list_l,
+                       const int32_t *count_l, uint32_t *stamp_l, int g_l, int n_refs,
+                       int n_per_ref, int bit_depth, uint32_t stamp_v, void *stream);
diff --git a/rav1e_amd/csrc/rv_me_diamond.hip b/rav1e_amd/csrc/rv_me_diamond.hip
--- a/rav1e_amd/csrc/rv_me_diamond.hip
+++ b/rav1e_amd/csrc/rv_me_diamond.hip
@@ -76,6 +76,8 @@
   const uint8_t *dirty;
   int list_grid;
   int ph;
+  uint32_t *stamp;
+  uint32_t stamp_v;
 };
 
 __device__ unsigned long long g_ds_ph[16];
@@ -991,7 +993,7 @@
   static constexpr int CPL = NC * NC * LPC / C;
 };
 
-template <typename Px, int N, bool SUB, bool SATD>
+template <typename Px, int N, bool SUB, bool SATD, bool STAMP = false>
 __device__ __forceinline__ void ds_grp_body(const DsArgs &a, const int ord, const int nord) {
   using G = GrpGeo<N, !SUB && !SATD>;
   static_assert(G::CPL >= 1 && G::C % G::LPC == 0, "lane layout");
@@ -1249,6 +1251,7 @@
   if (gl == 0 && live) {
     if (a.evals) a.evals[job] = evals;
     ds_write(a, job, center, center_cost);
+    if constexpr (STAMP) a.stamp[job] = a.stamp_v;
     chain_emit(a.next, job, a.n_per_ref, a.n / a.n_per_ref, center);
   }
 }
@@ -1266,14 +1269,14 @@
     if (!a.alist) break;
   }
 }
-template <typename Px>
+template <typename Px, bool STAMP = false>
 __device__ __forceinline__ void ds_grp16_pool(DsArgs a, int b, int gsz) {
   using G = GrpGeo<16, true>;
   constexpr int JPW = 64 / G::L;
   const int lane = threadIdx.x & 63;
   const int nord = ds_list_total(a);
   for (int o = (b * 4 + (int)(threadIdx.x >> 6)) * JPW; o < nord; o += gsz * 4 * JPW)
-    ds_grp_body<Px, 16, false, false>(a, o + lane / G::L, nord);
+    ds_grp_body<Px, 16, false, false, STAMP>(a, o + lane / G::L, nord);
 }
 template <typename Px>
 __device__ __forceinline__ void ds_fast64_pool(DsArgs a, DsArgs sa, bool fuse, int b, int gsz) {
@@ -1301,6 +1304,14 @@
     __syncthreads();
     if (threadIdx.x == 0) atomicMax(t01 + 1, (unsigned long long)wall_clock64());
   }
+}
+
+template <typename Px>
+__global__ __launch_bounds__(256) void ds_la_pair_kernel(DsArgs f2l, DsArgs fl, int g2) {
+  if ((int)blockIdx.x < g2)
+    ds_grp16_pool<Px, true>(f2l, blockIdx.x, g2);
+  else
+    ds_grp16_pool<Px, true>(fl, (int)blockIdx.x - g2, (int)gridDim.x - g2);
 }
 
 template <typename Px>
@@ -1491,6 +1502,33 @@
   return RV_OK;
 }
 
+int rv_diamond_la_pair(const rv_plane *org_h, const rv_plane *refs_h, const rv_ds_job *jobs_h,
+                       rv_fs_result *out_h, const int32_t *list_h, const int32_t *count_h,
+                       uint32_t *stamp_h, int g_h, const rv_plane *org, const rv_plane *refs,
+                       const rv_ds_job *jobs, rv_fs_result *out, const int32_t *list_l,
+                       const int32_t *count_l, uint32_t *stamp_l, int g_l, int n_refs,
+                       int n_per_ref, int bit_depth, uint32_t stamp_v, void *stream) {
+  if (!org_h || !refs_h || !org || !refs || n_refs < 1 || n_refs > RV_MAX_REFS || n_per_ref <= 0 ||
+      !jobs_h || !out_h || !list_h || !count_h || !stamp_h || !jobs || !out || !list_l ||
+      !count_l || !stamp_l || g_h < 1 || g_l < 1 || org->hbd != org_h->hbd)
+    return rv_set_error(RV_EINVAL, "rv_diamond_la_pair: bad arguments");
+  DsArgs f2l, fl;
+  ds_fill(f2l, org_h, refs_h, n_refs, jobs_h, n_per_ref * 4, 16, out_h, bit_depth, list_h, count_h,
+          0, nullptr);
+  ds_fill(fl, org, refs, n_refs, jobs, n_per_ref * 16, 16, out, bit_depth, list_l, count_l, 0,
+          nullptr);
+  f2l.stamp = stamp_h;
+  fl.stamp = stamp_l;
+  f2l.stamp_v = fl.stamp_v = stamp_v;
+  hipStream_t s = rv_resolve_stream(stream);
+  if (org->hbd)
+    ds_la_pair_kernel<uint16_t><<<g_h + g_l, 256, 0, s>>>(f2l, fl, g_h);
+  else
+    ds_la_pair_kernel<uint8_t><<<g_h + g_l, 256, 0, s>>>(f2l, fl, g_h);
+  RV_HIP_CHECK_LAUNCH();
+  return RV_OK;
+}
+
 static int ds_dispatch(DsArgs &a, void *stream) {
   const int n = a.n, blk_w = a.w, blk_h = a.h, subpixel = a.subpel;
   const rv_plane *org = &a.org;
diff --git a/rav1e_amd/csrc/rv_replay.h b/rav1e_amd/csrc/rv_replay.h
--- a/rav1e_amd/csrc/rv_replay.h
+++ b/rav1e_amd/csrc/rv_replay.h
@@ -1,6 +1,7 @@
 #pragma once
 #include <string.h>
 
+#include <atomic>
 #include <chrono>
 #include <condition_variable>
 #include <algorithm>
@@ -195,6 +196,12 @@
   rv_fs_result *coarse = nullptr, *half_l = nullptr, *look = nullptr;
 };
 
+struct LaWork {
+  int32_t *list = nullptr;
+  uint32_t *stamp = nullptr;
+  unsigned long long *vcnt = nullptr;
+};
+
 constexpr int kEngineWaitS = 60;
 
 struct rv_la_hub {
@@ -214,7 +221,7 @@
   Owned own;
   hipStream_t las = nullptr;
   RoundRing rr;
-  int32_t *la_list = nullptr;
+  LaWork la_work;
   void *scratch = nullptr;
   size_t scratch_bytes = 0;
   struct Entry {
@@ -341,7 +348,8 @@
   rv_fs_result *half_l = nullptr;
   rv_ds_job *jobs_half[3] = {}, *jobs_full[3] = {}, *jobs_sub[3] = {}, *jobs_look[3] = {};
   rv_ds_job *jobs_half_l[3] = {nullptr, nullptr, nullptr};
-  int32_t *la_list = nullptr;
+  LaWork la_work;
+  std::atomic<int> la_verify{0};
   long la_round_sum = 0, la_reeval = 0;
   long la_frames = 0;
   RvLaEngine *eng = nullptr;
@@ -434,6 +442,7 @@
 
 inline bool groups_active(const rv_replay *r) { return r->n_groups >= 2 || r->comm; }
 
+LaWork la_work_alloc(rv_replay *r, size_t nr);
 hipError_t kp_harvest(rv_replay *r, int p, long upto);
 size_t plane_bytes(const rv_plane &p);
 void round_ring_alloc(Owned &dev, Owned &host, RoundRing &q, hipStream_t st);
@@ -447,7 +456,7 @@
 LaRefs la_refs_of(long m, int R);
 
 int lookahead_frame(rv_replay *r, RoundRing &rr, hipStream_t xs, const rv_replay_frame_info &fi,
-                    const LaRefs &lr, long frame, const LaOut &o, int32_t *la_list, bool pyramid,
+                    const LaRefs &lr, long frame, const LaOut &o, const LaWork &lw, bool pyramid,
                     long *nrounds, long *nre, hipEvent_t *e);
 void la_engine_destroy(rv_replay *r);
 int la_encode_exchange(rv_replay *r, long n, hipStream_t st);
diff --git a/rav1e_amd/csrc/rv_replay.hip b/rav1e_amd/csrc/rv_replay.hip
--- a/rav1e_amd/csrc/rv_replay.hip
+++ b/rav1e_amd/csrc/rv_replay.hip
@@ -789,6 +789,14 @@
   for (auto &in : r->inputs) alloc_input(r, in, true);
 }
 
+LaWork la_work_alloc(rv_replay *r, size_t nr) {
+  LaWork w;
+  w.list = r->dev<int32_t>(nr * 20);
+  w.stamp = r->dev<uint32_t>(nr * 20, Fill::Zero);
+  w.vcnt = r->dev<unsigned long long>(4, Fill::Zero);
+  return w;
+}
+
 static void alloc_superblocks(rv_replay *r) {
   const Geo &g = r->g;
   const size_t nsb = (size_t)g.nsb, nr = nsb * g.R, nc = nsb * g.C;
@@ -796,7 +804,7 @@
   r->half = r->dev<rv_fs_result>(nr * 4);
   r->look = r->dev<rv_fs_result>(nr * 16, Fill::Zero);
   r->half_l = r->dev<rv_fs_result>(nr * 4, Fill::Zero);
-  r->la_list = r->dev<int32_t>(nr * 20);
+  r->la_work = la_work_alloc(r, nr);
   r->full = r->dev<rv_fs_result>(nr);
   r->sub = r->dev<rv_fs_result>(nr);
   r->ds_evals = r->dev<uint32_t>((size_t)rv_replay::kRing * 2 * nr, Fill::Zero);
diff --git a/rav1e_amd/csrc/rv_replay_frame.hip b/rav1e_amd/csrc/rv_replay_frame.hip
--- a/rav1e_amd/csrc/rv_replay_frame.hip
+++ b/rav1e_amd/csrc/rv_replay_frame.hip
@@ -709,7 +709,7 @@
       memset(&er, 0, sizeof(er));
       er.n = g.R;
       for (int k = 0; k < g.R; k++) er.disp[k] = fi.ref_display[k], er.order[k] = k;
-      RV_R(lookahead_frame(r, r->rr, st, fi, er, ncoded, LaOut{r->coarse, r->half_l, r->look}, r->la_list,
+      RV_R(lookahead_frame(r, r->rr, st, fi, er, ncoded, LaOut{r->coarse, r->half_l, r->look}, r->la_work,
                            true, &r->la_round_sum, &r->la_reeval, tm ? e : nullptr));
       r->la_frames++;
     }
diff --git a/rav1e_amd/csrc/rv_replay_la.hip b/rav1e_amd/csrc/rv_replay_la.hip
--- a/rav1e_amd/csrc/rv_replay_la.hip
+++ b/rav1e_amd/csrc/rv_replay_la.hip
@@ -1,3 +1,5 @@
+#include <limits.h>
+
 #include "rv_replay.h"
 
 namespace rv {
@@ -13,6 +15,12 @@
   int what;
   int nref;
   RoundPub pub;
+  uint32_t *stamp_h, *stamp_l;
+  uint32_t seq;
+  int verify;
+  unsigned long long *vcnt;
+  const int32_t *prev_cnt;
+  int cap_h, cap_l;
 };
 
 __device__ inline rv_mv la_coarse4(const LaArgs &a, int k, int sb) {
@@ -26,6 +34,24 @@
   const int i = blockIdx.x * 256 + threadIdx.x;
   bool mh = false, ml = false;
   int job = 0;
+  auto ran = [&](const uint32_t *stamp, bool on, int s) {
+    const bool is = on && s >= 0;
+    const uint32_t t = stamp[is ? s : 0];
+    return is & (t == a.seq);
+  };
+  auto judge = [&](bool live, auto &&eval) -> bool {
+    if (a.init) {
+      eval();
+      return false;
+    }
+    if (!live && !a.verify) return false;
+    const bool changed = eval();
+    if (a.verify) {
+      atomicAdd(a.vcnt + (live ? 2 : 1), 1ull);
+      if (!live && changed) atomicAdd(a.vcnt, 1ull);
+    }
+    return changed;
+  };
   if (i < nh) {
     job = i;
     const int k = i / (g.nsb * 4), sb = (i / 4) % g.nsb, q = i % 4;
@@ -33,24 +59,35 @@
     int t0x, t0y, mi_w, mi_h;
     sb_tile(g, sx, sy, t0x, t0y, mi_w, mi_h);
     const int fsx = g.tx0 + sx, fsy = g.ty0 + sy, tsx = fsx - t0x, tsy = fsy - t0y;
-    const int tsw = (mi_w + 15) / 16, tsh = (mi_h + 15) / 16;
-    const bool hh = (q & 1) ? tsx < tsw - 1 : tsx > 0, hv = (q >> 1) ? tsy < tsh - 1 : tsy > 0;
-    const rv_mv ch = hh ? la_coarse4(a, k, (q & 1) ? sb + 1 : sb - 1) : rv_mv{0, 0};
-    const rv_mv cv = hv ? la_coarse4(a, k, (q >> 1) ? sb + g.tw : sb - g.tw) : rv_mv{0, 0};
-    const rv_mv cm[3] = {la_coarse4(a, k, sb), hh ? ch : cv, cv};
-    const int nc = 1 + (int)hh + (int)hv;
     int bx = tsx * 16 + (q & 1) * 8, by = tsy * 16 + (q >> 1) * 8;
     adjust_bo(mi_w, mi_h, bx, by, 32, 32);
-    auto rd = [&](int X4, int Y4) {
+    auto src = [&](int X4, int Y4) {
       const int SX = X4 >> 4, SY = Y4 >> 4;
-      if (SX == fsx && SY == fsy) return rv_mv{0, 0};
+      if (SX == fsx && SY == fsy) return -1;
       const int gsb = (SY - g.ty0) * g.tw + (SX - g.tx0);
-      const rv_mv h =
-          a.half_l[((size_t)k * g.nsb + gsb) * 4 + ((Y4 >> 3) & 1) * 2 + ((X4 >> 3) & 1)].best_mv;
-      return rv_mv{(int16_t)(h.row * 2), (int16_t)(h.col * 2)};
+      return (k * g.nsb + gsb) * 4 + ((Y4 >> 3) & 1) * 2 + ((X4 >> 3) & 1);
     };
-    mh = epzs_update(a.jh + i, 1, a.eg, t0x * 16, t0y * 16, mi_w, bx, by, cm, nc, rd, nullptr, 1) &&
-         !a.init;
+    if (a.init) a.stamp_h[i] = a.seq;
+    const EpzsUnits u = epzs_units(t0x * 16, t0y * 16, mi_w, bx, by);
+    const bool live = (a.init == 0) & (ran(a.stamp_h, u.hl, src(u.lx, u.ly)) |
+                                       ran(a.stamp_h, u.ht, src(u.tx, u.ty)) |
+                                       ran(a.stamp_h, u.htr, src(u.rx, u.ry)));
+    mh = judge(live, [&]() {
+      const int tsw = (mi_w + 15) / 16, tsh = (mi_h + 15) / 16;
+      const bool hh = (q & 1) ? tsx < tsw - 1 : tsx > 0, hv = (q >> 1) ? tsy < tsh - 1 : tsy > 0;
+      const rv_mv ch = hh ? la_coarse4(a, k, (q & 1) ? sb + 1 : sb - 1) : rv_mv{0, 0};
+      const rv_mv cv = hv ? la_coarse4(a, k, (q >> 1) ? sb + g.tw : sb - g.tw) : rv_mv{0, 0};
+      const rv_mv cm[3] = {la_coarse4(a, k, sb), hh ? ch : cv, cv};
+      const int nc = 1 + (int)hh + (int)hv;
+      auto rd = [&](int X4, int Y4) {
+        const int s = src(X4, Y4);
+        if (s < 0) return rv_mv{0, 0};
+        const rv_mv h = a.half_l[s].best_mv;
+        return rv_mv{(int16_t)(h.row * 2), (int16_t)(h.col * 2)};
+      };
+      return epzs_update(a.jh + i, 1, a.eg, t0x * 16, t0y * 16, mi_w, bx, by, cm, nc, rd, nullptr,
+                         1);
+    });
   } else if (i - nh < nl) {
     const int j = i - nh;
     job = j;
@@ -59,29 +96,45 @@
     int t0x, t0y, mi_w, mi_h;
     sb_tile(g, sx, sy, t0x, t0y, mi_w, mi_h);
     const int tsx = g.tx0 + sx - t0x, tsy = g.ty0 + sy - t0y;
-    rv_mv cm[6];
-    int nc = 0;
-    bool more = true;
-#pragma unroll
-    for (int p = 1; p < 7; p++) {
-      const int v = more ? a.sl[8 * j + p] : -1;
-      more = more && v >= 0;
-      const rv_mv m = !more ? rv_mv{0, 0}
-                            : (v & 1) ? a.half_l[v >> 1].best_mv : a.coarse[v >> 1].best_mv;
-      const int sc = (v & 1) ? 2 : 4;
-      cm[p - 1] = rv_mv{(int16_t)(m.row * sc), (int16_t)(m.col * sc)};
-      nc += more ? 1 : 0;
-    }
     int bx = tsx * 16 + (b % 4) * 4, by = tsy * 16 + (b / 4) * 4;
     adjust_bo(mi_w, mi_h, bx, by, 16, 16);
-    auto rd = [&](int X4, int Y4) {
+    auto src = [&](int X4, int Y4) {
       const int gsb = ((Y4 >> 4) - g.ty0) * g.tw + ((X4 >> 4) - g.tx0);
-      return a.look[((size_t)k * g.nsb + gsb) * 16 + ((Y4 & 15) >> 2) * 4 + ((X4 & 15) >> 2)]
-          .best_mv;
+      return (k * g.nsb + gsb) * 16 + ((Y4 & 15) >> 2) * 4 + ((X4 & 15) >> 2);
     };
-    ml = epzs_update(a.jl + j, 0, a.eg, t0x * 16, t0y * 16, mi_w, bx, by, cm, nc, rd, nullptr, 1) &&
-         !a.init;
-  }
+    if (a.init) a.stamp_l[j] = a.seq;
+    const int4 s0 = *(const int4 *)(a.sl + 8 * j), s1 = *(const int4 *)(a.sl + 8 * j + 4);
+    int v[6] = {s0.y, s0.z, s0.w, s1.x, s1.y, s1.z};
+    bool more = true, live = false;
+#pragma unroll
+    for (int p = 0; p < 6; p++) {
+      more = more && v[p] >= 0;
+      if (!more) v[p] = -1;
+    }
+#pragma unroll
+    for (int p = 0; p < 6; p++) live |= ran(a.stamp_h, v[p] >= 0 && (v[p] & 1), v[p] >> 1);
+    const EpzsUnits u = epzs_units(t0x * 16, t0y * 16, mi_w, bx, by);
+    live = (a.init == 0) & (live | ran(a.stamp_l, u.hl, src(u.lx, u.ly)) |
+                      ran(a.stamp_l, u.ht, src(u.tx, u.ty)) | ran(a.stamp_l, u.htr, src(u.rx, u.ry)));
+    ml = judge(live, [&]() {
+      rv_mv cm[6];
+      int nc = 0;
+#pragma unroll
+      for (int p = 0; p < 6; p++) {
+        const bool on = v[p] >= 0;
+        const rv_mv m = !on ? rv_mv{0, 0}
+                            : (v[p] & 1) ? a.half_l[v[p] >> 1].best_mv : a.coarse[v[p] >> 1].best_mv;
+        const int sc = (v[p] & 1) ? 2 : 4;
+        cm[p] = rv_mv{(int16_t)(m.row * sc), (int16_t)(m.col * sc)};
+        nc += on ? 1 : 0;
+      }
+      auto rd = [&](int X4, int Y4) { return a.look[src(X4, Y4)].best_mv; };
+      return epzs_update(a.jl + j, 0, a.eg, t0x * 16, t0y * 16, mi_w, bx, by, cm, nc, rd, nullptr,
+                         1);
+    });
+  }
+  if (a.verify && !a.init && i == 0 && (a.prev_cnt[0] > a.cap_h || a.prev_cnt[1] > a.cap_l))
+    atomicAdd(a.vcnt + 3, 1ull);
   const int lane = threadIdx.x & 63;
   const uint64_t below = (1ull << lane) - 1;
   const uint64_t bh = __ballot(mh), bl = __ballot(ml);
@@ -99,7 +152,7 @@
 
 int lookahead_frame(rv_replay *r, RoundRing &rr, hipStream_t xs,
                     const rv_replay_frame_info &fi, const LaRefs &lr, long frame,
-                    const LaOut &o, int32_t *la_list, bool pyramid, long *nrounds,
+                    const LaOut &o, const LaWork &lw, bool pyramid, long *nrounds,
                     long *nre, hipEvent_t *e) {
   const Geo &g = r->g;
   const int lv = fi.level, nr = g.nsb, RL = lr.n;
@@ -137,39 +190,62 @@
   la_a.look = o.look;
   const int nh = nr * RL * 4, nl = nr * RL * 16;
   la_a.nref = RL;
-  la_a.list_h = la_list;
-  la_a.list_l = la_list + nh;
+  int32_t *const list_h = lw.list, *const list_l = lw.list + nh;
+  uint32_t *const stamp_h = lw.stamp, *const stamp_l = lw.stamp + nh;
+  la_a.list_h = list_h;
+  la_a.list_l = list_l;
+  la_a.stamp_h = stamp_h;
+  la_a.stamp_l = stamp_l;
+  la_a.verify = r->la_verify.load() ? 1 : 0;
+  la_a.vcnt = lw.vcnt;
+  int cap_h = INT_MAX, cap_l = INT_MAX;
   auto la_launch = [&](int what, uint32_t q, bool init) -> int {
     la_a.what = what;
     la_a.init = init ? 1 : 0;
-    la_a.pub = rr.pub(q, !init);
+    la_a.pub = rr.pub(init ? 0 : q, !init);
+    la_a.seq = q;
+    la_a.prev_cnt = rr.slot(q - 1);
+    la_a.cap_h = cap_h;
+    la_a.cap_l = cap_l;
     const int n = ((what & 1) ? nh : 0) + ((what & 2) ? nl : 0);
     la_check_kernel<<<(n + 255) / 256, 256, 0, xs>>>(la_a);
     RV_H(hipGetLastError());
     return RV_OK;
   };
-  auto f2l = [&](const int32_t *list, const int32_t *cnt) {
+  constexpr int kLaPool = 512, kLaFloor = 10;
+  auto la_round = [&](uint32_t q) -> int {
+    int g2 = kLaPool, g3 = kLaPool;
+    if (rr.last_count >= 0) {
+      const int t = std::min(std::max((2 * rr.last_count + 15) / 16, kLaFloor), 2 * kLaPool);
+      g2 = (t + 4) / 5;
+      g3 = t - g2;
+    }
+    g2 = std::min(g2, (nh + 15) / 16);
+    g3 = std::min(g3, (nl + 15) / 16);
+    cap_h = g2 * 16;
+    cap_l = g3 * 16;
+    return rv_diamond_la_pair(&cur.hres, refs_h, r->jobs_half_l[lv], o.half_l, list_h, rr.slot(q),
+                              stamp_h, g2, &cur.y, refs_o, r->jobs_look[lv], o.look, list_l,
+                              rr.slot(q) + 1, stamp_l, g3, RL, nr, g.bd, q + 1, xs);
+  };
+  auto f2l = [&]() {
     return rv_diamond_search_multi(&cur.hres, refs_h, RL, r->jobs_half_l[lv], nr * 4, 16, 16, 0,
-                                   0, 0, g.bd, o.half_l, nullptr, nullptr, xs, nullptr, list, cnt,
-                                   0);
+                                   0, 0, g.bd, o.half_l, nullptr, nullptr, xs);
   };
-  auto fl = [&](const int32_t *list, const int32_t *cnt) {
+  auto fl = [&]() {
     return rv_diamond_search_multi(&cur.y, refs_o, RL, r->jobs_look[lv], nr * 16, 16, 16, 0, 0, 0,
-                                   g.bd, o.look, nullptr, nullptr, xs, nullptr, list, cnt, 0);
+                                   g.bd, o.look, nullptr, nullptr, xs);
   };
-  RV_R(la_launch(1, 0, true));
-  RV_R(f2l(nullptr, nullptr));
+  const uint32_t q0 = rr.seq;
+  RV_R(la_launch(1, q0, true));
+  RV_R(f2l());
   RV_R(ev(kEvF2));
   RV_R(ev(kEvLaBegin));
-  RV_R(la_launch(2, 0, true));
-  RV_R(fl(nullptr, nullptr));
+  RV_R(la_launch(2, q0, true));
+  RV_R(fl());
   (*nrounds)++;
   RV_R(run_rounds(
-      rr, xs, 5 * (g.tws + g.ths), [&](uint32_t q) { return la_launch(3, q, false); },
-      [&](uint32_t q) -> int {
-        RV_R(f2l(la_list, rr.slot(q)));
-        return fl(la_list + nh, rr.slot(q) + 1);
-      },
+      rr, xs, 5 * (g.tws + g.ths), [&](uint32_t q) { return la_launch(3, q, false); }, la_round,
       nrounds, nre, nullptr, "lookahead", frame, lv));
   RV_R(ev(kEvLaEnd));
   return RV_OK;
@@ -265,7 +341,7 @@
                         hipMemcpyDeviceToDevice, xs));
   }
   long la_rounds = 0, la_reeval = 0;
-  RV_R(lookahead_frame(r, E.rr, xs, fi, lr, m - 1, e.o, E.la_list, false, &la_rounds, &la_reeval,
+  RV_R(lookahead_frame(r, E.rr, xs, fi, lr, m - 1, e.o, E.la_work, false, &la_rounds, &la_reeval,
                        nullptr));
   {
     std::lock_guard<std::mutex> lk(E.mu);
@@ -484,7 +560,7 @@
   E->own.failed = hipGetDevice(&E->dev) != hipSuccess;
   round_ring_alloc(r->own, E->own, E->rr, r->stream);
   const int ni = g.w_imp * g.h_imp, nr = g.nsb * r->RA;
-  E->la_list = r->dev<int32_t>((size_t)nr * 20);
+  E->la_work = la_work_alloc(r, (size_t)nr);
   E->scratch_bytes = impwin_scratch_bytes(ni);
   E->scratch = r->dev<uint8_t>(E->scratch_bytes);
   E->ring.resize((size_t)E->RW);
@@ -509,6 +585,27 @@
   }
   E->th = std::thread(la_thread_main, r);
   return RV_OK;
+}
+
+int rv_replay_set_la_verify(rv_replay *r, int on) {
+  if (!r) return rv_set_error(RV_EINVAL, "rv_replay_set_la_verify: bad arguments");
+  if (r->coded > 0) return rv_set_error(RV_EINVAL, "rv_replay_set_la_verify: after the first frame");
+  r->la_verify.store(on ? 1 : 0);
+  return RV_OK;
+}
+int rv_replay_la_verify_counts(rv_replay *r, uint64_t *out, int cap) {
+  if (!r || !out || cap < 4) return rv_set_error(RV_EINVAL, "rv_replay_la_verify_counts: bad arguments");
+  RV_H(hipDeviceSynchronize());
+  for (int i = 0; i < 4; i++) out[i] = 0;
+  const unsigned long long *src[2] = {r->la_work.vcnt, r->eng && r->eng_owned ? r->eng->la_work.vcnt
+                                                                               : nullptr};
+  for (const unsigned long long *s : src) {
+    if (!s) continue;
+    unsigned long long h[4];
+    RV_H(hipMemcpy(h, s, sizeof(h), hipMemcpyDeviceToHost));
+    for (int i = 0; i < 4; i++) out[i] += h[i];
+  }
+  return 4;
 }
 
 rv_la_hub *rv_la_hub_create(int n_groups) {
diff --git a/rav1e_amd/replay.py b/rav1e_amd/replay.py
--- a/rav1e_amd/replay.py
+++ b/rav1e_amd/replay.py
@@ -294,6 +294,15 @@
     def set_inputs_ready(self, displays: int):
         _check(lib().rv_replay_set_inputs_ready(self.h, int(displays)),
                "rv_replay_set_inputs_ready")
+
+    def set_la_verify(self, on: bool = True):
+        _check(lib().rv_replay_set_la_verify(self.h, int(bool(on))), "rv_replay_set_la_verify")
+
+    def la_verify_counts(self) -> np.ndarray:
+        out = np.zeros(4, dtype=np.uint64)
+        _check(lib().rv_replay_la_verify_counts(self.h, out.ctypes.data, 4) - 4,
+               "rv_replay_la_verify_counts")
+        return out
 
     def set_importances(self, imp):
         if imp is None:
```
